# nuggy875/NeRF_pytorch_paeng

Measured on AMD Instinct MI355X. Metric: rays/sec (4096-ray batch, 64c+128f samples) + 800×800 frame render ms, higher is better.
Workload: dtype f32

## Files before the change

### nerf_pytorch_paeng_amd/csrc/api.hip

```cpp
#include <string>
#include "half_layout.h"

namespace minerf {

ABI_ERROR_STATE(, MI_NERF_EHIP)

int device_cus() {
    static std::atomic<int> cus[MN_MAX_DEVICES] = {};
    int dev = 0;
    if (hipGetDevice(&dev) != hipSuccess) return 256;
    std::atomic<int>& slot = cus[dev & (MN_MAX_DEVICES - 1)];
    int c = slot.load(std::memory_order_relaxed);
    if (c <= 0) {
        hipDeviceProp_t prop;
        c = (hipGetDeviceProperties(&prop, dev) == hipSuccess && prop.multiProcessorCount > 0) ? prop.multiProcessorCount : 256;
        slot.store(c, std::memory_order_relaxed);
    }
    return c;
}
int ensure_lds_opt_in(LdsOptIn& state, const void* kernel) {
    int dev = 0;
    MN_HIP(hipGetDevice(&dev));
    std::atomic<bool>& done = state.done[dev & (MN_MAX_DEVICES - 1)];
    if (!done.load(std::memory_order_acquire)) {
        MN_HIP(hipFuncSetAttribute(kernel, hipFuncAttributeMaxDynamicSharedMemorySize, 160 * 1024));
        done.store(true, std::memory_order_release);
    }
    return MI_NERF_OK;
}

int mlp_rays_fp32(const mi_nerf_net*, const void*, const float*, const float*, int64_t, int, float*, hipStream_t);
int mlp_embedded_fp32(const mi_nerf_net*, const void*, const float*, int64_t, float*, hipStream_t);
int mlp_rays_bf16(const mi_nerf_net*, const void*, const float*, const float*, int64_t, int, float*, hipStream_t, int points_per_wave, const StratDraw* strat,
                  FineDraw* fine = nullptr);
int mlp_rays_f16(const mi_nerf_net*, const void*, const float*, const float*, int64_t, int, float*, hipStream_t, int points_per_wave, const StratDraw* strat,
                 FineDraw* fine);
int mlp_rays_f16s(const mi_nerf_net*, const void*, const float*, const float*, int64_t, int, float*, hipStream_t);
int mlp_rays_f16s_stash(const mi_nerf_net*, const void*, const float*, const float*, int64_t, int, float*, float*, float*, float*, unsigned*, unsigned*,
                        hipStream_t);
int wgrad_products(int, const float* const*, const int*, const int*, const float* const*, const int*, const int*, int64_t, float* const*, const int*,
                   float* const*, void*, size_t, hipStream_t, bool);
int mlp_rays_fp32_stash(const mi_nerf_net*, const void*, const float*, const float*, int64_t, int, float*, float*, float*, float*, unsigned*,
                        unsigned*, hipStream_t);
int mlp_backward_fp32(const mi_nerf_net*, const void*, const void*, const float*, const float*, int64_t, int, const float*, const void*, void*,
                      size_t, float*, int, hipStream_t, const float*, int64_t, int);
int mlp_embedded_fp32_stash(const mi_nerf_net*, const void*, const float*, int64_t, float*, float*, float*, float*, unsigned*, unsigned*,
                            hipStream_t);
int train_layout(const mi_nerf_net*, int64_t, int, mi_nerf_train_layout*);
size_t wgrad_scratch_bytes();
int pack_apply(const int32_t*, const float*, size_t, void*, hipStream_t);
int frames_image_metrics(const float*, const float*, int64_t, float*, void*, size_t, hipStream_t);
int frames_nanmax(const float*, int64_t, float*, void*, size_t, hipStream_t);
int frames_to8b(const float*, int64_t, const float*, unsigned char*, hipStream_t);
int frames_rays_rgb(int, int, const float*, const float*, const float*, int64_t, float*, hipStream_t);
int frames_permute_rows(const float*, const int64_t*, int64_t, int, float*, hipStream_t);
int stage_make_o_d(int, int, const float*, const float*, int, int, float*, float*, hipStream_t);
int stage_make_o_d_pixels(int, int, const float*, const float*, const int64_t*, int64_t, float*, float*, hipStream_t);
int stage_ndc(int, int, float, float, const float*, int64_t, const float*, int64_t, int64_t, float*, float*, hipStream_t);
int stage_fill_uniform(uint32_t, uint32_t, int64_t, int64_t, int, float*, hipStream_t);
int stage_stratified(int64_t, int, float, float, const float*, uint32_t, int64_t, float*, hipStream_t);
int stage_embed(const float*, const float*, int64_t, int, int, int, float*, hipStream_t);
int stage_posenc(const float*, int64_t, int, float*, hipStream_t);
int stage_composite(const float*, const float*, const float*, int, int64_t, int, float*, float*, float*, float*, float*, hipStream_t);
int stage_composite_backward(const float*, const float*, const float*, int, int64_t, int, const float*, float*, hipStream_t);
int stage_sample_pdf(const float*, const float*, int64_t, int, int, int, const float*, float*, hipStream_t);
int stage_fine_z(const float*, const float*, int64_t, int, int, int, const float*, uint32_t, int64_t, float*, float*, hipStream_t);
int stage_composite_fine_z(const float*, const float*, const float*, int64_t, int, int, int, const float*, uint32_t, int64_t, float*, float*, float*,
                           float*, hipStream_t);

static int check_net_basic(const mi_nerf_net* net) {
    MN_CHECK_ARG(net != nullptr, "net is NULL");
    MN_CHECK_ARG(net->W >= 2 && net->W <= MAX_KERNEL_WIDTH, "unsupported width W=%d (the fp32 inference kernels run 2 <= W <= %d, padded to 128 / 256 / 384 / 512; "
                 "training, bf16 and split precision: 128 / 256 and 256)", net->W, MAX_KERNEL_WIDTH);
    MN_CHECK_ARG(net->D >= 2 && net->D <= 16, "unsupported depth D=%d", net->D);
    MN_CHECK_ARG(net->L_x >= 0 && net->L_x <= 10 && net->L_d >= 0 && net->L_d <= 4,
                 "unsupported encoding L_x=%d L_d=%d (the kernels evaluate up to 10 / 4 frequencies; fewer run with zero weights on the rest)", net->L_x, net->L_d);
    MN_CHECK_ARG(net->skip >= -1, "bad skip=%d", net->skip);
    return MI_NERF_OK;
}

enum class Family { FP32, F16S, BF16, F16 };
struct ModePlan { Family coarse, fine; int points_per_wave; };

static int mode_plan(int mode, ModePlan* p) {
    switch (mode) {
        case MI_NERF_MODE_F32:       *p = {Family::FP32, Family::FP32, 0}; return MI_NERF_OK;
        case MI_NERF_MODE_BF16:      *p = {Family::BF16, Family::BF16, 0}; return MI_NERF_OK;
        case MI_NERF_MODE_BF16_64:   *p = {Family::BF16, Family::BF16, 64}; return MI_NERF_OK;
        case MI_NERF_MODE_BF16_32:   *p = {Family::BF16, Family::BF16, 32}; return MI_NERF_OK;
        case MI_NERF_MODE_F16S:      *p = {Family::F16S, Family::F16S, 0}; return MI_NERF_OK;
        case MI_NERF_MODE_F16S_BF16: *p = {Family::F16S, Family::BF16, 0}; return MI_NERF_OK;
        case MI_NERF_MODE_F16:       *p = {Family::F16, Family::F16, 0}; return MI_NERF_OK;
        case MI_NERF_MODE_F16_BF16:  *p = {Family::F16, Family::BF16, 0}; return MI_NERF_OK;
    }
    set_error("mode must be one of MI_NERF_MODE_* (0..3, 5, 6, 8, 9; got %d)", mode);
    return MI_NERF_EINVAL;
}

static int mlp_rays_family(Family family, const mi_nerf_net* net, const void* packed, const float* rays, const float* z, int64_t n, int S, float* raw,
                           hipStream_t st, int points_per_wave, const StratDraw* strat = nullptr, FineDraw* fine = nullptr) {
    if (family == Family::FP32) return mlp_rays_fp32(net, packed, rays, z, n, S, raw, st);
    if (family == Family::F16S) return mlp_rays_f16s(net, packed, rays, z, n, S, raw, st);
    return (family == Family::F16 ? mlp_rays_f16 : mlp_rays_bf16)(net, packed, rays, z, n, S, raw, st, points_per_wave, strat, fine);
}

static int workspace_layout(const mi_nerf_render_cfg* cfg, int64_t n, mi_nerf_workspace_layout* L) {
    MN_CHECK_ARG(cfg && L, "NULL cfg/layout");
    MN_CHECK_ARG(n >= 0 && cfg->Sc >= 1 && cfg->Nf >= 0, "bad sizes n=%lld Sc=%d Nf=%d", (long long)n, cfg->Sc, cfg->Nf);
    MN_CHECK_ARG(cfg->Nf == 0 || cfg->Sc >= 3, "hierarchical sampling needs at least 3 coarse samples");
    size_t off = 0;
    const size_t nn = (size_t)n, Sc = (size_t)cfg->Sc, St = (size_t)(cfg->Sc + cfg->Nf);
    L->z_c = off;       off += align256(nn * Sc * 4);
    L->raw_c = off;     off += align256(nn * Sc * 16);
    L->weights_c = off; off += align256(nn * Sc * 4);
    L->z_f = off;       off += cfg->Nf > 0 ? align256(nn * St * 4) : 0;
    L->raw_f = off;     off += cfg->Nf > 0 ? align256(nn * St * 16) : 0;
    L->total = off;
    return MI_NERF_OK;
}

__global__ void mfma_selftest_kernel(const float* __restrict__ A, const float* __restrict__ B, float* __restrict__ D) {
    const int lane = threadIdx.x & 63;
    f32x16 acc;
#pragma unroll
    for (int r = 0; r < 16; ++r) acc[r] = 0.0f;
#pragma unroll
    for (int s = 0; s < 4; ++s) {
        const int k = 2 * s + (lane >> 5);
        const float a = A[(lane & 31) * 8 + k];
        const float b = B[k * 32 + (lane & 31)];
        acc = __builtin_amdgcn_mfma_f32_32x32x2f32(a, b, acc, 0, 0, 0);
    }
#pragma unroll
    for (int r = 0; r < 16; ++r) {
        const int i = (r & 3) + 8 * (r >> 2) + 4 * (lane >> 5);
        D[i * 32 + (lane & 31)] = acc[r];
    }
}

}

using namespace minerf;

extern "C" {

int mi_nerf_abi_version(void) { return MI_NERF_ABI_VERSION; }
const char* mi_nerf_last_error(void) { return g_err; }

size_t mi_nerf_packed_bytes(const mi_nerf_net* net) {
    if (check_net_basic(net)) return 0;
    return make_layout(net->D, net->W, net->skip, net->L_x, net->L_d).total_bytes;
}
int mi_nerf_pack_weights(const mi_nerf_net* net, const mi_nerf_params* params, void* blob, size_t bytes) {
    if (int rc = check_net_basic(net)) return rc;
    MN_CHECK_ARG(params && blob, "NULL params/blob");
    MN_CHECK_ARG(params->linear_x_w && params->linear_x_b && params->linear_density_w && params->linear_density_b &&
                 params->linear_feat_w && params->linear_feat_b && params->linear_d_w && params->linear_d_b &&
                 params->linear_color_w && params->linear_color_b, "NULL parameter pointer");
    for (int l = 0; l < net->D; ++l) MN_CHECK_ARG(params->linear_x_w[l] && params->linear_x_b[l], "NULL trunk layer %d", l);
    return pack_fp32(net, params, blob, bytes);
}
size_t mi_nerf_packed_bytes_bf16(const mi_nerf_net* net) {
    if (check_net_basic(net)) return 0;
    return packed_bytes_bf16(net);
}
size_t mi_nerf_packed_bytes_f16s(const mi_nerf_net* net) {
    return packed_bytes_f16s(net);
}
int mi_nerf_pack_weights_f16s(const mi_nerf_net* net, const mi_nerf_params* params, void* blob, size_t bytes) {
    MN_CHECK_ARG(net && params && blob, "NULL argument");
    return pack_f16s(net, params, blob, bytes);
}
int mi_nerf_pack_weights_bf16(const mi_nerf_net* net, const mi_nerf_params* params, void* blob, size_t bytes) {
    if (int rc = check_net_basic(net)) return rc;
    MN_CHECK_ARG(params && blob, "NULL params/blob");
    return pack_bf16(net, params, blob, bytes);
}

int mi_nerf_make_o_d(int W, int H, const float k4[4], const float pose12[12], int row0, int n_rows, float* o, float* d, void* st) {
    MN_CHECK_ARG(k4 && pose12, "NULL camera");
    return stage_make_o_d(W, H, k4, pose12, row0, n_rows, o, d, (hipStream_t)st);
}
int mi_nerf_make_o_d_pixels(int W, int H, const float k4[4], const float pose12[12], const int64_t* pix, int64_t n, float* o,
                            float* d, void* st) {
    MN_CHECK_ARG(k4 && pose12, "NULL camera");
    return stage_make_o_d_pixels(W, H, k4, pose12, pix, n, o, d, (hipStream_t)st);
}
int mi_nerf_ndc_rays(int H, int W, float focal, float near_, const float* o_in, int64_t os, const float* d_in, int64_t ds, int64_t n,
                     float* o_out, float* d_out, void* st) {
    return stage_ndc(H, W, focal, near_, o_in, os, d_in, ds, n, o_out, d_out, (hipStream_t)st);
}
int mi_nerf_fill_uniform(uint32_t seed, uint32_t stream_id, int64_t ray0, int64_t n_rays, int S, float* out, void* st) {
    return stage_fill_uniform(seed, stream_id, ray0, n_rays, S, out, (hipStream_t)st);
}
int mi_nerf_stratified_z(int64_t n_rays, int S, float near_, float far_, const float* t_rand, float* z, void* st) {
    MN_CHECK_ARG(t_rand != nullptr || n_rays == 0, "t_rand is NULL");
    return stage_stratified(n_rays, S, near_, far_, t_rand, 0, 0, z, (hipStream_t)st);
}
int mi_nerf_sample_pdf(const float* bins, const float* weights, int64_t n, int B, int N, int det, const float* u, float* out, void* st) {
    return stage_sample_pdf(bins, weights, n, B, N, det, u, out, (hipStream_t)st);
}
int mi_nerf_fine_z(const float* z_c, const float* w_c, int64_t n, int Sc, int Nf, int det, const float* u, float* z_f, float* z_s,
                   void* st) {
    MN_CHECK_ARG(det || u != nullptr || n == 0, "u is NULL (and det == 0)");
    return stage_fine_z(z_c, w_c, n, Sc, Nf, det, u, 0, 0, z_f, z_s, (hipStream_t)st);
}
int mi_nerf_embed(const float* rays, const float* z, int64_t n_rays, int S, int L_x, int L_d, float* out, void* st) {
    return stage_embed(rays, z, n_rays, S, L_x, L_d, out, (hipStream_t)st);
}
int mi_nerf_posenc(const float* x, int64_t n, int L, float* out, void* st) { return stage_posenc(x, n, L, out, (hipStream_t)st); }
int mi_nerf_mlp_embedded(const mi_nerf_net* net, const void* packed, const float* x, int64_t n, float* out, void* st) {
    return mlp_embedded_fp32(net, packed, x, n, out, (hipStream_t)st);
}
int mi_nerf_mlp_rays(const mi_nerf_net* net, const void* packed, const float* rays, const float* z, int64_t n_rays, int S, float* raw,
                     void* st) {
    return mlp_rays_fp32(net, packed, rays, z, n_rays, S, raw, (hipStream_t)st);
}
int mi_nerf_mlp_rays_bf16(const mi_nerf_net* net, const void* packed, const float* rays, const float* z, int64_t n_rays, int S,
                          float* raw, void* st) {
    MN_CHECK_ARG(z != nullptr || n_rays == 0, "z is NULL");
    return mlp_rays_bf16(net, packed, rays, z, n_rays, S, raw, (hipStream_t)st, 0, nullptr);
}
int mi_nerf_mlp_rays_f16s(const mi_nerf_net* net, const void* packed, const float* rays, const float* z, int64_t n_rays, int S, float* raw,
                          void* st) {
    return mlp_rays_f16s(net, packed, rays, z, n_rays, S, raw, (hipStream_t)st);
}
int mi_nerf_mlp_rays_bf16_shape(const mi_nerf_net* net, const void* packed, const float* rays, const float* z, int64_t n_rays, int S,
                                float* raw, int points_per_wave, void* st) {
    MN_CHECK_ARG(z != nullptr || n_rays == 0, "z is NULL");
    return mlp_rays_bf16(net, packed, rays, z, n_rays, S, raw, (hipStream_t)st, points_per_wave, nullptr);
}
int mi_nerf_composite(const float* raw, const float* z, const float* rays, int ray_stride, int64_t n, int S, float* rgb, float* disp,
                      float* acc, float* weights, float* depth, void* st) {
    return stage_composite(raw, z, rays, ray_stride, n, S, rgb, disp, acc, weights, depth, (hipStream_t)st);
}

int mi_nerf_composite_backward(const float* raw, const float* z, const float* rays, int ray_stride, int64_t n, int S,
                               const float* d_rgb, float* d_raw, void* st) {
    return stage_composite_backward(raw, z, rays, ray_stride, n, S, d_rgb, d_raw, (hipStream_t)st);
}

size_t mi_nerf_param_count(const mi_nerf_net* net) {
    if (check_net_basic(net)) return 0;
    return make_param_offsets(net->D, net->W, net->skip, net->L_x, net->L_d).total;
}
size_t mi_nerf_packed_bytes_bwd(const mi_nerf_net* net) {
    if (check_net_basic(net)) return 0;
    return packed_bytes_bwd(net);
}
int mi_nerf_pack_weights_bwd(const mi_nerf_net* net, const mi_nerf_params* params, void* host_blob, size_t blob_bytes) {
    if (int rc = check_net_basic(net)) return rc;
    MN_CHECK_ARG(params && host_blob, "NULL params/blob");
    return pack_bwd_fp32(net, params, host_blob, blob_bytes);
}
int mi_nerf_pack_map(const mi_nerf_net* net, int kind, int32_t* map_host, size_t map_len) {
    if (int rc = check_net_basic(net)) return rc;
    return pack_map(net, kind, map_host, map_len);
}
size_t mi_nerf_pack_map_bf16_len(const mi_nerf_net* net) {
    if (!net) return 0;
    return pack_map_bf16_len(net);
}
int mi_nerf_pack_map_bf16(const mi_nerf_net* net, int32_t* map_host, size_t map_len) {
    MN_CHECK_ARG(net && map_host, "NULL pointer");
    return pack_map_bf16(net, map_host, map_len);
}
int mi_nerf_pack_apply_bf16(const mi_nerf_net* net, const int32_t* map_dev, const float* flat_dev, void* blob_dev, size_t blob_bytes, void* st) {
    MN_CHECK_ARG(net, "net is NULL");
    return pack_apply_bf16(net, map_dev, flat_dev, blob_dev, blob_bytes, (hipStream_t)st);
}
int mi_nerf_pack_apply(const int32_t* map_dev, const float* flat_dev, size_t blob_bytes, void* blob_dev, void* st) {
    return pack_apply(map_dev, flat_dev, blob_bytes, blob_dev, (hipStream_t)st);
}
int mi_nerf_train_layout_query(const mi_nerf_net* net, int64_t n_rays, int S, mi_nerf_train_layout* out) {
    if (int rc = check_net_basic(net)) return rc;
    return train_layout(net, n_rays, S, out);
}
int mi_nerf_mlp_rays_train(const mi_nerf_net* net, const void* packed, const float* rays, const float* z, int64_t n_rays, int S,
                           float* raw, void* stash, size_t stash_bytes, void* st) {
    if (int rc = check_net_basic(net)) return rc;
    MN_CHECK_ARG(n_rays >= 0 && S >= 1, "bad sizes n_rays=%lld S=%d", (long long)n_rays, S);
    mi_nerf_train_layout L;
    if (int rc = train_layout(net, n_rays, S, &L)) return rc;
    if (n_rays == 0) return MI_NERF_OK;
    MN_CHECK_ARG(stash != nullptr && stash_bytes >= L.stash_bytes, "stash too small: %zu < %zu", stash_bytes, L.stash_bytes);
    return mlp_rays_fp32_stash(net, packed, rays, z, n_rays, S, raw, (float*)((char*)stash + L.stash_h), (float*)((char*)stash + L.stash_f),
                               (float*)((char*)stash + L.stash_g), (unsigned*)((char*)stash + L.mask_h), (unsigned*)((char*)stash + L.mask_g),
                               (hipStream_t)st);
}
int mi_nerf_mlp_rays_train_f16s(const mi_nerf_net* net, const void* packed_f16s, const float* rays, const float* z, int64_t n_rays, int S,
                                float* raw, void* stash, size_t stash_bytes, void* st) {
    if (int rc = check_net_basic(net)) return rc;
    MN_CHECK_ARG(n_rays >= 0 && S >= 1, "bad sizes n_rays=%lld S=%d", (long long)n_rays, S);
    mi_nerf_train_layout L;
    if (int rc = train_layout(net, n_rays, S, &L)) return rc;
    if (n_rays == 0) return MI_NERF_OK;
    MN_CHECK_ARG(stash != nullptr && stash_bytes >= L.stash_bytes, "stash too small: %zu < %zu", stash_bytes, L.stash_bytes);
    return mlp_rays_f16s_stash(net, packed_f16s, rays, z, n_rays, S, raw, (float*)((char*)stash + L.stash_h), (float*)((char*)stash + L.stash_f),
                               (float*)((char*)stash + L.stash_g), (unsigned*)((char*)stash + L.mask_h), (unsigned*)((char*)stash + L.mask_g),
                               (hipStream_t)st);
}
size_t mi_nerf_pack_map_f16s_len(const mi_nerf_net* net) {
    if (!net) return 0;
    return pack_map_f16s_len(net);
}
int mi_nerf_pack_map_f16s(const mi_nerf_net* net, int32_t* map_host, size_t map_len) {
    MN_CHECK_ARG(net && map_host, "NULL pointer");
    return pack_map_f16s(net, map_host, map_len);
}
size_t mi_nerf_packed_bytes_bwd_f16s(const mi_nerf_net* net) {
    if (!net) return 0;
    return packed_bytes_bwd_f16s(net);
}
int mi_nerf_pack_weights_bwd_f16s(const mi_nerf_net* net, const mi_nerf_params* params, void* host_blob, size_t blob_bytes) {
    MN_CHECK_ARG(net && params && host_blob, "NULL pointer");
    return pack_bwd_f16s(net, params, host_blob, blob_bytes);
}
size_t mi_nerf_pack_map_bwd_f16s_len(const mi_nerf_net* net) {
    if (!net) return 0;
    return pack_map_bwd_f16s_len(net);
}
int mi_nerf_pack_map_bwd_f16s(const mi_nerf_net* net, int32_t* map_host, size_t map_len) {
    MN_CHECK_ARG(net && map_host, "NULL pointer");
    return pack_map_bwd_f16s(net, map_host, map_len);
}
int mi_nerf_pack_apply_bwd_f16s(const mi_nerf_net* net, const int32_t* map_dev, const float* flat_dev, void* blob_dev, size_t blob_bytes,
                                uint32_t* out_of_range_dev, void* st) {
    MN_CHECK_ARG(net, "net is NULL");
    return pack_apply_bwd_f16s(net, map_dev, flat_dev, blob_dev, blob_bytes, out_of_range_dev, (hipStream_t)st);
}
int mi_nerf_pack_apply_f16s(const mi_nerf_net* net, const int32_t* map_dev, const float* flat_dev, void* blob_dev, size_t blob_bytes,
                            uint32_t* out_of_range_dev, void* st) {
    MN_CHECK_ARG(net, "net is NULL");
    return pack_apply_f16s(net, map_dev, flat_dev, blob_dev, blob_bytes, out_of_range_dev, (hipStream_t)st);
}
int mi_nerf_mlp_backward(const mi_nerf_net* net, const void* packed, const void* packed_bwd, const float* rays, const float* z,
                         int64_t n_rays, int S, const float* d_raw, const void* stash, void* work, size_t work_bytes, float* grads,
                         int stage, void* st) {
    if (int rc = check_net_basic(net)) return rc;
    return mlp_backward_fp32(net, packed, packed_bwd, rays, z, n_rays, S, d_raw, stash, work, work_bytes, grads, stage, (hipStream_t)st, nullptr, -1, 0);
}
int mi_nerf_mlp_backward_mode(const mi_nerf_net* net, const void* packed, const void* packed_bwd, const float* rays, const float* z,
                              int64_t n_rays, int S, const float* d_raw, const void* stash, void* work, size_t work_bytes, float* grads,
                              int stage, int mode, void* st) {
    if (int rc = check_net_basic(net)) return rc;
    MN_CHECK_ARG((mode & ~3) == 0, "unknown backward mode %d", mode);
    return mlp_backward_fp32(net, packed, packed_bwd, rays, z, n_rays, S, d_raw, stash, work, work_bytes, grads, stage, (hipStream_t)st, nullptr, -1, mode);
}
int mi_nerf_mlp_embedded_train(const mi_nerf_net* net, const void* packed, const float* x, int64_t n, float* out, void* stash, size_t stash_bytes,
                               void* st) {
    if (int rc = check_net_basic(net)) return rc;
    MN_CHECK_ARG(n >= 0, "bad n=%lld", (long long)n);
    mi_nerf_train_layout L;
    if (int rc = train_layout(net, (n + 31) / 32, 32, &L)) return rc;
    if (n == 0) return MI_NERF_OK;
    MN_CHECK_ARG(stash != nullptr && stash_bytes >= L.stash_bytes, "stash too small: %zu < %zu", stash_bytes, L.stash_bytes);
    return mlp_embedded_fp32_stash(net, packed, x, n, out, (float*)((char*)stash + L.stash_h), (float*)((char*)stash + L.stash_f),
                                   (float*)((char*)stash + L.stash_g), (unsigned*)((char*)stash + L.mask_h), (unsigned*)((char*)stash + L.mask_g),
                                   (hipStream_t)st);
}
int mi_nerf_mlp_embedded_backward(const mi_nerf_net* net, const void* packed, const void* packed_bwd, const float* x, int64_t n, const float* d_out,
                                  const void* stash, void* work, size_t work_bytes, float* grads, void* st) {
    if (int rc = check_net_basic(net)) return rc;
    MN_CHECK_ARG(n >= 0, "bad n=%lld", (long long)n);
    MN_CHECK_ARG(x != nullptr || n == 0, "NULL device pointer");
    static const float no_rows = 0.0f;
    return mlp_backward_fp32(net, packed, packed_bwd, nullptr, nullptr, (n + 31) / 32, 32, d_out, stash, work, work_bytes, grads, 0, (hipStream_t)st,
                             x ? x : &no_rows, n, 0);
}

int mi_nerf_image_metrics(const float* pred, const float* target, int64_t n, float* out2, void* scratch, size_t scratch_bytes, void* st) {
    return frames_image_metrics(pred, target, n, out2, scratch, scratch_bytes, (hipStream_t)st);
}
int mi_nerf_nanmax(const float* x, int64_t n, float* out, void* scratch, size_t scratch_bytes, void* st) {
    return frames_nanmax(x, n, out, scratch, scratch_bytes, (hipStream_t)st);
}
int mi_nerf_to8b(const float* x, int64_t n, const float* divisor, uint8_t* out, void* st) {
    return frames_to8b(x, n, divisor, out, (hipStream_t)st);
}
int mi_nerf_rays_rgb(int W, int H, const float k4[4], const float* poses, const float* images, int64_t n_img, float* out, void* st) {
    return frames_rays_rgb(W, H, k4, poses, images, n_img, out, (hipStream_t)st);
}
int mi_nerf_permute_rows(const float* src, const int64_t* perm, int64_t n, int row_floats, float* dst, void* st) {
    return frames_permute_rows(src, perm, n, row_floats, dst, (hipStream_t)st);
}

size_t mi_nerf_render_workspace_bytes(const mi_nerf_render_cfg* cfg, int64_t n_rays) {
    mi_nerf_workspace_layout L;
    if (workspace_layout(cfg, n_rays, &L)) return 0;
    return L.total;
}
int mi_nerf_render_workspace_layout(const mi_nerf_render_cfg* cfg, int64_t n_rays, mi_nerf_workspace_layout* out) {
    return workspace_layout(cfg, n_rays, out);
}

int mi_nerf_render_rays(const mi_nerf_net* net, const void* packed_c, const void* packed_f, const mi_nerf_render_cfg* cfg,
                        const float* rays, int64_t n, const float* t_rand, const float* u, void* ws, size_t ws_bytes,
                        float* rgb_c, float* disp_c, float* rgb_f, float* disp_f, void* stream) {
    hipStream_t st = (hipStream_t)stream;
    mi_nerf_workspace_layout L;
    if (int rc = workspace_layout(cfg, n, &L)) return rc;
    if (n == 0) return MI_NERF_OK;
    MN_CHECK_ARG(ws_bytes >= L.total, "workspace too small: %zu < %zu", ws_bytes, L.total);
    MN_CHECK_ARG(rays && rgb_c && disp_c && packed_c && (ws || L.total == 0), "NULL pointer");
    MN_CHECK_ARG(cfg->Nf == 0 || (packed_f && rgb_f && disp_f), "fine pass needs packed_fine and outputs");
    MN_CHECK_ARG(cfg->reserved == 0, "mi_nerf_render_cfg.reserved must be 0");
    char* w = (char*)ws;
    float* z_c = (float*)(w + L.z_c);
    float* raw_c = (float*)(w + L.raw_c);
    float* wts_c = (float*)(w + L.weights_c);
    const int Sc = cfg->Sc, St = cfg->Sc + cfg->Nf;
    ModePlan p;
    if (int rc = mode_plan(cfg->mode, &p)) return rc;
    if (p.coarse == Family::F16 || p.fine == Family::F16)
        if (int rc = check_net_half(net, "f16")) return rc;
    if (p.coarse == Family::F16S || p.fine == Family::F16S)
        if (int rc = check_net_f16s_forward(net)) return rc;
    FineDraw fd{};
    if (p.coarse == Family::BF16 || p.coarse == Family::F16) {
        const StratDraw sd{cfg->near_, cfg->far_, t_rand, cfg->seed, cfg->ray_offset, z_c};
        if (cfg->Nf > 0) fd = FineDraw{cfg->Nf, cfg->det, u, cfg->seed, cfg->ray_offset, rgb_c, disp_c, wts_c, (float*)(w + L.z_f), false};
        if (int rc = mlp_rays_family(p.coarse, net, packed_c, rays, nullptr, n, Sc, raw_c, st, p.points_per_wave, &sd,
                                     cfg->Nf > 0 && p.points_per_wave == 0 ? &fd : nullptr))
            return rc;
    } else {
        if (int rc = stage_stratified(n, Sc, cfg->near_, cfg->far_, t_rand, cfg->seed, cfg->ray_offset, z_c, st)) return rc;
        if (int rc = mlp_rays_family(p.coarse, net, packed_c, rays, z_c, n, Sc, raw_c, st, p.points_per_wave)) return rc;
    }
    if (cfg->Nf == 0) return stage_composite(raw_c, z_c, rays, 6, n, Sc, rgb_c, disp_c, nullptr, wts_c, nullptr, st);
    {
        float* z_f = (float*)(w + L.z_f);
        float* raw_f = (float*)(w + L.raw_f);
        if (!fd.taken)
            if (int rc = stage_composite_fine_z(raw_c, z_c, rays, n, Sc, cfg->Nf, cfg->det, u, cfg->seed, cfg->ray_offset, rgb_c, disp_c, wts_c, z_f, st))
                return rc;
        if (int rc = mlp_rays_family(p.fine, net, packed_f, rays, z_f, n, St, raw_f, st, p.points_per_wave)) return rc;
        if (int rc = stage_composite(raw_f, z_f, rays, 6, n, St, rgb_f, disp_f, nullptr, nullptr, nullptr, st)) return rc;
    }
    return MI_NERF_OK;
}

int mi_nerf_time_mlp_rays(const mi_nerf_net* net, const void* packed, const float* rays, const float* z, int64_t n_rays, int S,
                          float* raw, int iters, int mode, float* avg_ms, void* stream) {
    hipStream_t st = (hipStream_t)stream;
    MN_CHECK_ARG(iters >= 1 && avg_ms, "bad iters / NULL output");
    ModePlan p;
    if (int rc = mode_plan(mode, &p)) return rc;
    MN_CHECK_ARG(p.coarse == p.fine, "MI_NERF_MODE_* %d is two kernel families (mi_nerf_render_rays only): one network, one kernel family", mode);
    if (p.fine == Family::F16)
        if (int rc = check_net_half(net, "f16")) return rc;
    if (p.fine == Family::F16S)
        if (int rc = check_net_f16s_forward(net)) return rc;
    hipEvent_t e0, e1;
    MN_HIP(hipEventCreate(&e0));
    MN_HIP(hipEventCreate(&e1));
    int rc = MI_NERF_OK;
    MN_HIP(hipEventRecord(e0, st));
    for (int i = 0; i < iters && rc == MI_NERF_OK; ++i)
        rc = mlp_rays_family(p.fine, net, packed, rays, z, n_rays, S, raw, st, p.points_per_wave);
    MN_HIP(hipEventRecord(e1, st));
    MN_HIP(hipEventSynchronize(e1));
    float ms = 0.f;
    MN_HIP(hipEventElapsedTime(&ms, e0, e1));
    (void)hipEventDestroy(e0);
    (void)hipEventDestroy(e1);
    *avg_ms = ms / (float)iters;
    return rc;
}

size_t mi_nerf_wgrad_scratch_bytes(void) { return wgrad_scratch_bytes(); }
extern "C++" template <typename F>
static int timed_launches(int iters, float* avg_ms, hipStream_t st, F body) {
    MN_CHECK_ARG(iters >= 1, "bad iters");
    hipEvent_t e0 = nullptr, e1 = nullptr;
    if (avg_ms) {
        MN_HIP(hipEventCreate(&e0));
        MN_HIP(hipEventCreate(&e1));
        MN_HIP(hipEventRecord(e0, st));
    }
    int rc = MI_NERF_OK;
    for (int i = 0; i < iters && rc == MI_NERF_OK; ++i) rc = body();
    if (avg_ms) {
        MN_HIP(hipEventRecord(e1, st));
        MN_HIP(hipEventSynchronize(e1));
        float ms = 0.f;
        MN_HIP(hipEventElapsedTime(&ms, e0, e1));
        (void)hipEventDestroy(e0);
        (void)hipEventDestroy(e1);
        *avg_ms = ms / (float)iters;
    }
    return rc;
}
int mi_nerf_wgrad_products(int n, const float* const* delta, const int* ldd, const int* M, const float* const* x, const int* ldx, const int* N,
                           int64_t P, float* const* out, const int* ldo, float* const* bias, void* scratch, size_t scratch_bytes, int iters,
                           float* avg_ms, void* stream) {
    hipStream_t st = (hipStream_t)stream;
    return timed_launches(iters, avg_ms, st, [&] { return wgrad_products(n, delta, ldd, M, x, ldx, N, P, out, ldo, bias, scratch, scratch_bytes, st, false); });
}
int mi_nerf_wgrad_products_f16s(int n, const float* const* delta, const int* ldd, const int* M, const float* const* x, const int* ldx, const int* N,
                                int64_t P, float* const* out, const int* ldo, float* const* bias, void* scratch, size_t scratch_bytes, int iters,
                                float* avg_ms, void* stream) {
    hipStream_t st = (hipStream_t)stream;
    return timed_launches(iters, avg_ms, st, [&] { return wgrad_products(n, delta, ldd, M, x, ldx, N, P, out, ldo, bias, scratch, scratch_bytes, st, true); });
}

int mi_nerf_selftest_mfma(void* stream) {
    hipStream_t st = (hipStream_t)stream;
    float hA[32 * 8], hB[8 * 32], hD[32 * 32], ref[32 * 32];
    for (int i = 0; i < 32; ++i) for (int k = 0; k < 8; ++k) hA[i * 8 + k] = (float)((i * 3 + k * 7) % 11 - 5);
    for (int k = 0; k < 8; ++k) for (int j = 0; j < 32; ++j) hB[k * 32 + j] = (float)((k * 5 + j * 2 + (j > 9)) % 13 - 6);
    for (int i = 0; i < 32; ++i) for (int j = 0; j < 32; ++j) {
        float s = 0.f;
        for (int k = 0; k < 8; ++k) s += hA[i * 8 + k] * hB[k * 32 + j];
        ref[i * 32 + j] = s;
    }
    float *dA, *dB, *dD;
    MN_HIP(hipMalloc(&dA, sizeof(hA)));
    MN_HIP(hipMalloc(&dB, sizeof(hB)));
    MN_HIP(hipMalloc(&dD, sizeof(hD)));
    MN_HIP(hipMemcpyAsync(dA, hA, sizeof(hA), hipMemcpyHostToDevice, st));
    MN_HIP(hipMemcpyAsync(dB, hB, sizeof(hB), hipMemcpyHostToDevice, st));
    hipLaunchKernelGGL(mfma_selftest_kernel, dim3(1), dim3(64), 0, st, dA, dB, dD);
    MN_LAUNCH_CHECK("mfma_selftest_kernel");
    MN_HIP(hipMemcpyAsync(hD, dD, sizeof(hD), hipMemcpyDeviceToHost, st));
    MN_HIP(hipStreamSynchronize(st));
    (void)hipFree(dA); (void)hipFree(dB); (void)hipFree(dD);
    for (int i = 0; i < 32 * 32; ++i)
        if (hD[i] != ref[i]) {
            set_error("MFMA layout mismatch at D[%d][%d]: got %g want %g", i / 32, i % 32, hD[i], ref[i]);
            return MI_NERF_EINVAL;
        }
    return MI_NERF_OK;
}

}
```

### nerf_pytorch_paeng_amd/csrc/layout.h

```cpp
#pragma once
#include <stdint.h>
#include <stddef.h>

namespace minerf {

constexpr int QUAD_BYTES = 1024;
constexpr int SLOT_QUADS = 16;
constexpr int SLOT_BYTES = QUAD_BYTES * SLOT_QUADS;
constexpr int HEADER_BYTES = 1024;
constexpr uint32_t BLOB_MAGIC = 0x4D494E46u;

__host__ __device__ constexpr int pe_ksteps(int L) { return ((3 * L + 2 + 3) / 4) * 4; }

constexpr int KERNEL_LX = 10, KERNEL_LD = 4;

constexpr int MAX_KERNEL_WIDTH = 512;
__host__ __device__ constexpr int kernel_width(int W) { return W <= 128 ? 128 : (W <= 256 ? 256 : (W <= 384 ? 384 : 512)); }
__host__ __device__ constexpr bool wide_kernel_width(int Wk) { return Wk > 256; }
__host__ __device__ constexpr int pe_ksteps16(int L) { return (((3 * L + 1) / 2 + 1 + 3) / 4) * 4; }
__host__ __device__ constexpr bool native_width(int W) { return W == 128 || W == 256; }

struct BlobLayout {
    uint32_t stream_off;
    uint32_t stream_bytes_hoist;
    uint32_t stream_bytes_full;
    uint32_t side_off;
    uint32_t side_floats;
    uint32_t bias_trunk;
    uint32_t bias_feat;
    uint32_t bias_d;
    uint32_t dens_w;
    uint32_t dens_b;
    uint32_t color_w;
    uint32_t color_b;
    uint32_t wdir_t;
    uint32_t total_bytes;
};

__host__ __device__ inline uint32_t round_up_u32(uint32_t v, uint32_t m) { return (v + m - 1) / m * m; }

inline BlobLayout make_layout(int D, int W_net, int skip, int , int ) {
    constexpr int L_x = KERNEL_LX, L_d = KERNEL_LD;
    const int W = kernel_width(W_net);
    BlobLayout b{};
    const int NT = W / 32;
    const int in_d = 3 + 6 * L_d;
    const uint32_t pe_quads = (uint32_t)(pe_ksteps(L_x) / 4) * NT;
    const uint32_t h_quads = (uint32_t)(W / 2 / 4) * NT;
    uint32_t quads = pe_quads;
    for (int l = 1; l < D; ++l) quads += h_quads + ((skip >= 0 && l == skip + 1) ? pe_quads : 0);
    quads += h_quads;
    quads += (uint32_t)(W / 2 / 4) * (NT / 2);
    b.stream_off = HEADER_BYTES;
    b.stream_bytes_hoist = round_up_u32(quads, SLOT_QUADS) * QUAD_BYTES;
    uint32_t full = round_up_u32(quads, SLOT_QUADS) + round_up_u32((uint32_t)(pe_ksteps(L_d) / 4) * (NT / 2), SLOT_QUADS);
    b.stream_bytes_full = full * QUAD_BYTES;
    b.side_off = b.stream_off + b.stream_bytes_full;
    uint32_t f = 0;
    b.bias_trunk = f; f += (uint32_t)D * W;
    b.bias_feat = f;  f += W;
    b.bias_d = f;     f += W / 2;
    b.dens_w = f;     f += W;
    b.dens_b = f;     f += 4;
    b.color_w = f;    f += 3 * (W / 2);
    b.color_b = f;    f += 4;
    b.wdir_t = f;     f += (uint32_t)in_d * (W / 2);
    b.side_floats = round_up_u32(f, 4);
    b.total_bytes = b.side_off + b.side_floats * 4;
    return b;
}

struct SideTables {
    const char* stream;
    const float* side;
    int D;
    int skip_layer;
    unsigned stream_bytes;
    unsigned side_floats;
    unsigned o_bias_trunk, o_bias_feat, o_bias_d, o_wdir_t;
    unsigned o_dens_w, o_dens_b, o_color_w, o_color_b;
    unsigned o_head_b;
};
inline int skip_layer_of(int D, int skip) { return (skip >= 0 && skip + 1 < D) ? skip + 1 : -1; }

inline SideTables side_tables(const BlobLayout& L, const void* packed_dev, int D, int skip, bool full_stream) {
    SideTables t{};
    t.stream = (const char*)packed_dev + L.stream_off;
    t.side = (const float*)((const char*)packed_dev + L.side_off);
    t.D = D;
    t.skip_layer = skip_layer_of(D, skip);
    t.stream_bytes = full_stream ? L.stream_bytes_full : L.stream_bytes_hoist;
    t.side_floats = L.side_floats;
    t.o_bias_trunk = L.bias_trunk; t.o_bias_feat = L.bias_feat; t.o_bias_d = L.bias_d; t.o_wdir_t = L.wdir_t;
    t.o_dens_w = L.dens_w; t.o_dens_b = L.dens_b; t.o_color_w = L.color_w; t.o_color_b = L.color_b;
    return t;
}

struct ParamOffsets {
    uint32_t w_x[16], b_x[16];
    int in_l[16];
    uint32_t w_d, b_d, w_feat, b_feat, w_dens, b_dens, w_color, b_color;
    uint32_t total;
};

inline ParamOffsets make_param_offsets(int D, int W, int skip, int L_x, int L_d) {
    ParamOffsets p{};
    const int in_x = 3 + 6 * L_x, in_d = 3 + 6 * L_d;
    uint32_t f = 0;
    for (int l = 0; l < D; ++l) {
        p.in_l[l] = (l == 0) ? in_x : ((skip >= 0 && l == skip + 1) ? W + in_x : W);
        p.w_x[l] = f; f += (uint32_t)W * p.in_l[l];
        p.b_x[l] = f; f += W;
    }
    p.w_d = f;     f += (uint32_t)(W / 2) * (W + in_d);
    p.b_d = f;     f += W / 2;
    p.w_feat = f;  f += (uint32_t)W * W;
    p.b_feat = f;  f += W;
    p.w_dens = f;  f += W;
    p.b_dens = f;  f += 1;
    p.w_color = f; f += 3 * (W / 2);
    p.b_color = f; f += 3;
    p.total = f;
    return p;
}

inline uint32_t bwd_stream_bytes(int D, int W) {
    const uint32_t NT = W / 32;
    const uint32_t quads = (uint32_t)(W / 16) * NT + (uint32_t)D * (uint32_t)(W / 8) * NT;
    return round_up_u32(quads, SLOT_QUADS) * QUAD_BYTES;
}

}
```

### nerf_pytorch_paeng_amd/csrc/mlp_fp32.hip

```cpp
#include <stdlib.h>
#include <vector>
#include "common.h"
#include "layout.h"
#include "mlp_core.h"


namespace minerf {


template <int L, bool SLOW, int NPE>
__device__ __forceinline__ void encode_regs(float (&pe)[NPE], const float (&p)[3], int hh) {
#pragma unroll
    for (int s = 0; s < 3 * L; ++s) {
        const float y = p[s % 3] * (float)(1 << (s / 3));
        pe[s] = SLOW ? sin_cos_slow(y, hh) : sin_cos_fast(y, hh);
    }
    pe[3 * L] = hh ? p[1] : p[0];
    pe[3 * L + 1] = hh ? 0.0f : p[2];
#pragma unroll
    for (int s = 3 * L + 2; s < NPE; ++s) pe[s] = 0.0f;
}

template <int L, int NPE>
__device__ __forceinline__ void gather_regs(float (&pe)[NPE], const float* row, int hh, bool valid, int L_net) {
#pragma unroll
    for (int s = 0; s < 3 * L; ++s) {
        const int ch = 3 + 6 * (s / 3) + (s % 3) + 3 * hh;
        const bool have = valid && (s / 3) < L_net;
        pe[s] = have ? row[have ? ch : 0] : 0.0f;
    }
    pe[3 * L] = valid ? row[hh] : 0.0f;
    pe[3 * L + 1] = (valid && !hh) ? row[2] : 0.0f;
#pragma unroll
    for (int s = 3 * L + 2; s < NPE; ++s) pe[s] = 0.0f;
}

template <int W, bool STASH, int NEXT, int AL, int HN>
__device__ __forceinline__ void hidden_gemm(const MlpArgs& a, int layer, long long out_idx, long long wt, bool wave_active, f32x16 (&acc)[8],
                                            const float (&h)[HN], f32x4 (&aq)[8], const char* smem, WRing& ring, int lane, int hh) {
    constexpr int NT = W / 32;
    constexpr int HK_B = NT - 3, HK_M = NT - 2, HK_S = NT - 1;
    if constexpr (STASH) {
        float* row = a.stash_h + ((long long)layer * a.stash_rows + out_idx) * W + 4 * hh;
        unsigned mw[4] = {0u, 0u, 0u, 0u};
        unsigned mb[4];
        auto hook = [&](int kq, int t) __attribute__((always_inline)) {
            if (t == HK_B) mask_bits_chunk(h, kq, mb);
            if (t == HK_M) mask_merge_chunk(mb, kq, mw);
            if (t == HK_S) store_chunk(h, kq, row);
        };
        gemm_part<NT, HN, NEXT, AL>(acc, h, aq, smem, ring, lane, hook);
        if (wave_active) {
            u32x4 m; m[0] = mw[0]; m[1] = mw[1]; m[2] = mw[2]; m[3] = mw[3];
            *(u32x4*)(a.mask_h + (((long long)layer * a.n_wtiles + wt) * 64 + lane) * 4) = m;
        }
    } else {
        gemm_part<NT, HN, NEXT, AL>(acc, h, aq, smem, ring, lane);
    }
}

template <int W, int MODE, int LX, int LD, bool STASH>
__global__ __launch_bounds__(256) __attribute__((amdgpu_waves_per_eu(1, 1)))
void mlp_fp32_kernel(const MlpArgs a) {
    constexpr int NT = W / 32;
    constexpr int HN = W / 2;
    constexpr int KPE = pe_ksteps(LX);
    constexpr int KDE = pe_ksteps(LD);
    constexpr int AL = STASH ? 8 : 4;
    extern __shared__ __attribute__((aligned(16))) char smem[];
    float* side = (float*)(smem + RING_BYTES);
    const int tid = threadIdx.x;
    const int lane = tid & 63;
    const int wave = __builtin_amdgcn_readfirstlane(tid >> 6);
    const int col = lane & 31, hh = lane >> 5;
    float* scratch = side + a.side_floats + wave * (W / 2);

    for (unsigned i = tid * 4; i < a.side_floats; i += 256 * 4) *(f32x4*)(side + i) = *(const f32x4*)(a.side + i);

    const long long n_wg_tiles = (a.n_wtiles + 3) >> 2;
    if ((long long)blockIdx.x >= n_wg_tiles) return;

    WRing ring = ring_start(a.stream, a.stream_bytes, smem, wave, lane);

    f32x16 acc[8];
    f32x4 aq[8];
    float h[HN];
    float pe[KPE];
    ring_advance(ring);
#pragma unroll
    for (int t = 0; t < NT; ++t) aq[t] = ring_read(smem, ring, lane, t);

#ifdef MN_DIAG
    unsigned long long seg[8] = {0, 0, 0, 0, 0, 0, 0, 0};
    unsigned long long tprev = mn_stamp();
#endif
    RayTileWalk<32> walk = {};
    long long bias_ray = -1;
    const long long wid = (long long)blockIdx.x * 4 + wave;
    if constexpr (MODE == 0) walk.start(a, wid, col);
    for (long long it = 0; it < a.n_iter; ++it) {
#ifdef MN_DIAG
        ring.dlog = (a.diag && it == 2 && blockIdx.x < 4) ? a.diag + (size_t)gridDim.x * 32 + ((size_t)blockIdx.x * 4 + wave) * 512 : nullptr;
        ring.dcnt = 0;
#endif
        bool wave_active;
        long long wt;
        bool valid;
        long long out_idx;
        float de[KDE];
        if constexpr (MODE == 0) {
            wave_active = walk.active(a);
            const long long ray = walk.ray(a);
            const int chunk = walk.chunk(a);
            wt = ray * a.tpr + chunk;
            const int sample = chunk * 32 + col;
            valid = wave_active && sample < a.S;
            const int sc = sample < a.S ? sample : a.S - 1;
            out_idx = ray * a.S + sc;
            const float o[3] = {walk.o[0], walk.o[1], walk.o[2]}, d[3] = {walk.d[0], walk.d[1], walk.d[2]};
            const float zv = walk.z;
            walk.advance(a, col);
            float p[3];
            sample_point(p, o, d, zv);
            if (__builtin_expect(point_is_fast<LX>(p), 1)) encode_regs<LX, false>(pe, p, hh);
            else encode_regs<LX, true>(pe, p, hh);
            if (ray != bias_ray) {
                bias_ray = ray;
                hoisted_dir_bias<W, LD>(scratch, d[0], d[1], d[2], side + a.o_wdir_t, side + a.o_bias_d, lane);
            }
        } else {
            wt = it * ((long long)gridDim.x * 4) + wid;
            wave_active = wt < a.n_wtiles;
            if (!wave_active) wt = a.n_wtiles - 1;
            const long long p0 = wt * 32 + col;
            valid = wave_active && p0 < a.n_pts;
            out_idx = p0 < a.n_pts ? p0 : a.n_pts - 1;
            const int in_x_net = 3 + 6 * a.Lx_net;
            const float* row = a.x + out_idx * (in_x_net + 3 + 6 * a.Ld_net);
            gather_regs<LX>(pe, row, hh, true, a.Lx_net);
            gather_regs<LD>(de, row + in_x_net, hh, true, a.Ld_net);
        }

        MN_STAMP(0);
        acc_init<NT>(acc, side + a.o_bias_trunk, hh);
        gemm_part<NT, KPE, NT, AL>(acc, pe, aq, smem, ring, lane);
        MN_STAMP(1);
#pragma unroll 1
        for (int l = 1; l < a.D; ++l) {
            acc_to_b<NT, true>(acc, h);
            acc_init<NT>(acc, side + a.o_bias_trunk + l * W, hh);
            if (l == a.skip_layer) gemm_part<NT, KPE, NT, AL>(acc, pe, aq, smem, ring, lane);
            hidden_gemm<W, STASH, NT, AL>(a, l - 1, out_idx, wt, wave_active, acc, h, aq, smem, ring, lane, hh);
        }
        acc_to_b<NT, true>(acc, h);
        MN_STAMP(2);
        const float dens = xhalf_sum(dot_half<HN>(h, side + a.o_dens_w, hh)) + side[a.o_dens_b];
        acc_init<NT>(acc, side + a.o_bias_feat, hh);
        hidden_gemm<W, STASH, NT / 2, AL>(a, a.D - 1, out_idx, wt, wave_active, acc, h, aq, smem, ring, lane, hh);
        acc_to_b<NT, false>(acc, h);
        MN_STAMP(3);
        float* const row_f = STASH ? a.stash_f + out_idx * W + 4 * hh : nullptr;
        auto feat_hook = [&](int kq, int t) __attribute__((always_inline)) {
            if (STASH && t == NT / 2 - 1) store_chunk(h, kq, row_f);
        };
        if constexpr (MODE == 0) {
            acc_init<NT / 2>(acc, scratch, hh);
            gemm_part<NT / 2, HN, NT, AL>(acc, h, aq, smem, ring, lane, feat_hook);
        } else {
            acc_init<NT / 2>(acc, side + a.o_bias_d, hh);
            gemm_part<NT / 2, HN, NT / 2, AL>(acc, h, aq, smem, ring, lane, feat_hook);
            gemm_part<NT / 2, KDE, NT, AL>(acc, de, aq, smem, ring, lane);
        }
        float h2[HN / 2];
        acc_to_b<NT / 2, true>(acc, h2);
        if constexpr (STASH) {
            store_rows<NT / 2>(h2, a.stash_g + out_idx * (W / 2) + 4 * hh, valid);
            unsigned mg[2] = {0u, 0u};
#pragma unroll
            for (int q = 0; q < HN / 8; ++q) mask_pack_chunk(h2, q, mg);
            if (wave_active) {
                u32x2 m; m[0] = mg[0]; m[1] = mg[1];
                *(u32x2*)(a.mask_g + (wt * 64 + lane) * 2) = m;
            }
        }
        MN_STAMP(4);
        const float* cw = side + a.o_color_w;
        const float r0 = xhalf_sum(dot_half<HN / 2>(h2, cw, hh)) + side[a.o_color_b + 0];
        const float r1 = xhalf_sum(dot_half<HN / 2>(h2, cw + W / 2, hh)) + side[a.o_color_b + 1];
        const float r2 = xhalf_sum(dot_half<HN / 2>(h2, cw + W, hh)) + side[a.o_color_b + 2];
        if (valid && hh == 0) {
            f32x4 o; o[0] = r0; o[1] = r1; o[2] = r2; o[3] = dens;
            *(f32x4*)(a.out + out_idx * 4) = o;
        }
        MN_STAMP(5);
    }
#ifdef MN_DIAG
    if (a.diag && lane == 0) {
        unsigned long long* d = a.diag + ((size_t)blockIdx.x * 4 + wave) * 8;
        for (int i = 0; i < 8; ++i) d[i] = seg[i];
    }
#endif
    asm volatile("s_waitcnt vmcnt(0)" ::: "memory");
    __syncthreads();
}

static int check_net(const mi_nerf_net* net) {
    MN_CHECK_ARG(net != nullptr, "net is NULL");
    MN_CHECK_ARG(net->W >= 2 && net->W <= MAX_KERNEL_WIDTH, "unsupported width W=%d (the fp32 inference kernels run 2 <= W <= %d, padded to 128 / 256 / 384 / 512)", net->W, MAX_KERNEL_WIDTH);
    MN_CHECK_ARG(net->D >= 2 && net->D <= 16, "unsupported depth D=%d", net->D);
    MN_CHECK_ARG(net->L_x >= 0 && net->L_x <= KERNEL_LX && net->L_d >= 0 && net->L_d <= KERNEL_LD,
                 "unsupported encoding L_x=%d L_d=%d (the kernels evaluate up to %d / %d frequencies)", net->L_x, net->L_d, KERNEL_LX, KERNEL_LD);
    MN_CHECK_ARG(net->skip >= -1, "bad skip=%d", net->skip);
    return MI_NERF_OK;
}

int mlp_rays_fp32_wide(const mi_nerf_net*, const void*, const float*, const float*, int64_t, int, float*, hipStream_t);
int mlp_embedded_fp32_wide(const mi_nerf_net*, const void*, const float*, int64_t, float*, hipStream_t);

template <int W, int MODE, bool STASH = false>
static int launch(const MlpArgs& args_in, hipStream_t st) {
    MlpArgs args = args_in;
    auto kern = mlp_fp32_kernel<W, MODE, 10, 4, STASH>;
    static LdsOptIn opt_in = {};
    size_t lds;
    int grid;
    if (int rc = plan_launch<W, MODE>(args, (const void*)kern, opt_in, lds, grid)) return rc;
#ifdef MN_DIAG
    {
        MlpArgs da = args;
        unsigned long long* dbuf = nullptr;
        const size_t n = (size_t)grid * 4 * 8 + 16 * 512;
        MN_HIP(hipMalloc(&dbuf, n * 8));
        MN_HIP(hipMemsetAsync(dbuf, 0, n * 8, st));
        da.diag = dbuf;
        hipLaunchKernelGGL(kern, dim3(grid), dim3(256), lds, st, da);
        MN_HIP(hipStreamSynchronize(st));
        std::vector<unsigned long long> hbuf(n);
        MN_HIP(hipMemcpy(hbuf.data(), dbuf, n * 8, hipMemcpyDeviceToHost));
        (void)hipFree(dbuf);
        const double tiles = (double)((args.n_wtiles + 4 * grid - 1) / (4 * grid));
        static const char* names[6] = {"prologue", "layer0", "trunk", "dens+feature", "viewdir", "colour+store"};
        double tot = 0;
        fprintf(stderr, "[mn_diag] W=%d MODE=%d grid=%d tiles/wg=%.1f  cycles per tile (mean over waves):\n", W, MODE, grid, tiles);
        for (int sgi = 0; sgi < 6; ++sgi) {
            double sum = 0;
            for (size_t w = 0; w < (size_t)grid * 4; ++w) sum += (double)hbuf[w * 8 + sgi];
            const double per = sum / ((double)grid * 4) / tiles;
            tot += per;
            fprintf(stderr, "[mn_diag]   %-14s %10.0f\n", names[sgi], per);
        }
        fprintf(stderr, "[mn_diag]   %-14s %10.0f\n", "total", tot);
        if (const char* e = getenv("MN_DIAG_KQ")) {
            const int wsel = atoi(e);
            const unsigned long long* lg = hbuf.data() + (size_t)grid * 32 + (size_t)wsel * 512;
            fprintf(stderr, "[mn_diag] k-quad deltas (cycles; ideal %d) of wave %d, tile 2:", 4 * 64 * (W / 32), wsel);
            for (int i = 1; i < 500 && lg[i]; ++i) fprintf(stderr, "%s%llu", (i % 16 == 1) ? "\n[mn_diag]   " : " ", lg[i] - lg[i - 1]);
            fprintf(stderr, "\n");
        }
        return MI_NERF_OK;
    }
#endif
    hipLaunchKernelGGL(kern, dim3(grid), dim3(256), lds, st, args);
    MN_LAUNCH_CHECK("mlp_fp32_kernel");
    return MI_NERF_OK;
}

int mlp_rays_fp32(const mi_nerf_net* net, const void* packed_dev, const float* rays_dev, const float* z_dev,
                  int64_t n_rays, int S, float* raw_dev, hipStream_t st) {
    if (int rc = check_net(net)) return rc;
    MN_CHECK_ARG(n_rays >= 0 && S >= 1, "bad sizes n_rays=%lld S=%d", (long long)n_rays, S);
    if (n_rays == 0) return MI_NERF_OK;
    MN_CHECK_ARG(packed_dev && rays_dev && z_dev && raw_dev, "NULL device pointer");
    if (wide_kernel_width(kernel_width(net->W))) return mlp_rays_fp32_wide(net, packed_dev, rays_dev, z_dev, n_rays, S, raw_dev, st);
    MlpArgs a{};
    fill_common(a, net, packed_dev, false);
    fill_rays<32>(a, rays_dev, z_dev, n_rays, S, raw_dev);
    return kernel_width(net->W) == 256 ? launch<256, 0>(a, st) : launch<128, 0>(a, st);
}

int mlp_rays_fp32_stash(const mi_nerf_net* net, const void* packed_dev, const float* rays_dev, const float* z_dev,
                        int64_t n_rays, int S, float* raw_dev, float* stash_h, float* stash_f, float* stash_g, unsigned* mask_h,
                        unsigned* mask_g, hipStream_t st) {
    if (int rc = check_net(net)) return rc;
    MN_CHECK_ARG(native_width(net->W), "the training kernels exist for W = 128 and 256 (got %d)", net->W);
    MN_CHECK_ARG(n_rays >= 0 && S >= 1, "bad sizes n_rays=%lld S=%d", (long long)n_rays, S);
    if (n_rays == 0) return MI_NERF_OK;
    MN_CHECK_ARG(packed_dev && rays_dev && z_dev && raw_dev && stash_h && stash_f && stash_g && mask_h && mask_g, "NULL device pointer");
    MlpArgs a{};
    fill_common(a, net, packed_dev, false);
    fill_rays<32>(a, rays_dev, z_dev, n_rays, S, raw_dev);
    a.stash_h = stash_h; a.stash_f = stash_f; a.stash_g = stash_g; a.stash_rows = (long long)n_rays * S;
    a.mask_h = mask_h; a.mask_g = mask_g;
    return net->W == 256 ? launch<256, 0, true>(a, st) : launch<128, 0, true>(a, st);
}

int mlp_embedded_fp32_stash(const mi_nerf_net* net, const void* packed_dev, const float* x_dev, int64_t n, float* out_dev, float* stash_h,
                            float* stash_f, float* stash_g, unsigned* mask_h, unsigned* mask_g, hipStream_t st) {
    if (int rc = check_net(net)) return rc;
    MN_CHECK_ARG(native_width(net->W), "the training kernels exist for W = 128 and 256 (got %d)", net->W);
    MN_CHECK_ARG(n >= 0, "bad n=%lld", (long long)n);
    if (n == 0) return MI_NERF_OK;
    MN_CHECK_ARG(packed_dev && x_dev && out_dev && stash_h && stash_f && stash_g && mask_h && mask_g, "NULL device pointer");
    MlpArgs a{};
    fill_common(a, net, packed_dev, true);
    a.x = x_dev; a.out = out_dev; a.n_pts = n;
    a.n_wtiles = (n + 31) / 32;
    a.stash_h = stash_h; a.stash_f = stash_f; a.stash_g = stash_g; a.stash_rows = a.n_wtiles * 32;
    a.mask_h = mask_h; a.mask_g = mask_g;
    return net->W == 256 ? launch<256, 1, true>(a, st) : launch<128, 1, true>(a, st);
}

int mlp_embedded_fp32(const mi_nerf_net* net, const void* packed_dev, const float* x_dev, int64_t n, float* out_dev,
                      hipStream_t st) {
    if (int rc = check_net(net)) return rc;
    MN_CHECK_ARG(n >= 0, "bad n=%lld", (long long)n);
    if (n == 0) return MI_NERF_OK;
    MN_CHECK_ARG(packed_dev && x_dev && out_dev, "NULL device pointer");
    if (wide_kernel_width(kernel_width(net->W))) return mlp_embedded_fp32_wide(net, packed_dev, x_dev, n, out_dev, st);
    MlpArgs a{};
    fill_common(a, net, packed_dev, true);
    a.x = x_dev; a.out = out_dev; a.n_pts = n;
    a.n_wtiles = (n + 31) / 32;
    return kernel_width(net->W) == 256 ? launch<256, 1>(a, st) : launch<128, 1>(a, st);
}

}
```

### nerf_pytorch_paeng_amd/csrc/stage_dev.h

```cpp
#pragma once
#include "common.h"

namespace minerf {

__device__ __forceinline__ float wave_sum(float v) {
#pragma unroll
    for (int m = 32; m >= 1; m >>= 1) v += __shfl_xor(v, m, 64);
    return v;
}
__device__ __forceinline__ float wave_excl_prod(float v, int lane) {
    float inc = v;
#pragma unroll
    for (int d = 1; d < 64; d <<= 1) {
        const float o = __shfl_up(inc, d, 64);
        if (lane >= d) inc *= o;
    }
    const float e = __shfl_up(inc, 1, 64);
    return lane == 0 ? 1.0f : e;
}
__device__ __forceinline__ float wave_excl_sum(float v, int lane) {
    float inc = v;
#pragma unroll
    for (int d = 1; d < 64; d <<= 1) {
        const float o = __shfl_up(inc, d, 64);
        if (lane >= d) inc += o;
    }
    const float e = __shfl_up(inc, 1, 64);
    return lane == 0 ? 0.0f : e;
}
__device__ __forceinline__ float wave_excl_suffix_sum(float v, int lane) {
    float inc = v;
#pragma unroll
    for (int d = 1; d < 64; d <<= 1) {
        const float o = __shfl_down(inc, d, 64);
        if (lane + d < 64) inc += o;
    }
    const float e = __shfl_down(inc, 1, 64);
    return lane == 63 ? 0.0f : e;
}

template <int C>
__device__ __forceinline__ void composite_ray(const float* __restrict__ raw, const float* __restrict__ z, const float* __restrict__ rays,
                                              int ray_stride, long long ray, int S, int lane, float* __restrict__ rgb_o,
                                              float* __restrict__ disp_o, float* __restrict__ acc_o, float* __restrict__ w_o,
                                              float* __restrict__ depth_o, float* w_lds) {
    const float* dp = rays + ray * ray_stride + (ray_stride == 6 ? 3 : 0);
    const float dx = dp[0], dy = dp[1], dz = dp[2];
    const float dnorm = __builtin_sqrtf(dx * dx + dy * dy + dz * dz);
    const float* zr = z + ray * S;
    const f32x4* rr = (const f32x4*)(raw + ray * S * 4);

    float alpha[C], zv[C], cr[C], cg[C], cb[C];
    float local = 1.0f;
#pragma unroll
    for (int c = 0; c < C; ++c) {
        const int s = lane * C + c;
        const bool in = s < S;
        const int sc = in ? s : S - 1;
        const f32x4 v = rr[sc];
        zv[c] = zr[sc];
        float dist = (s + 1 < S) ? (zr[s + 1] - zv[c]) : 1e10f;
        dist = dist * dnorm;
        const float sig = __builtin_fmaxf(v[3], 0.0f);
        float a = 1.0f - expf(-sig * dist);
        if (!in || S == 1) a = 0.0f;
        alpha[c] = a;
        cr[c] = 1.0f / (1.0f + expf(-v[0]));
        cg[c] = 1.0f / (1.0f + expf(-v[1]));
        cb[c] = 1.0f / (1.0f + expf(-v[2]));
        local *= in ? (1.0f - a + 1e-10f) : 1.0f;
    }
    float T = wave_excl_prod(local, lane);
    float sw = 0.f, sr = 0.f, sg = 0.f, sb = 0.f, sd = 0.f;
#pragma unroll
    for (int c = 0; c < C; ++c) {
        const int s = lane * C + c;
        const float w = alpha[c] * T;
        if (s < S) {
            if (w_o) w_o[ray * S + s] = w;
            if (w_lds) w_lds[s] = w;
            sw += w; sr += w * cr[c]; sg += w * cg[c]; sb += w * cb[c]; sd += w * zv[c];
        }
        T *= (1.0f - alpha[c] + 1e-10f);
    }
    sw = wave_sum(sw); sr = wave_sum(sr); sg = wave_sum(sg); sb = wave_sum(sb); sd = wave_sum(sd);
    if (lane == 0) {
        const float q = sd / sw;
        const float m = (q != q) ? q : __builtin_fmaxf(1e-10f, q);
        float disp = 1.0f / m;
        if (disp != disp) disp = 0.0f;
        if (disp > 5.0f) disp = 5.0f;
        const float bg = 1.0f - sw;
        rgb_o[ray * 3 + 0] = sr + bg; rgb_o[ray * 3 + 1] = sg + bg; rgb_o[ray * 3 + 2] = sb + bg;
        disp_o[ray] = disp;
        if (acc_o) acc_o[ray] = sw;
        if (depth_o) depth_o[ray] = sd;
    }
}

__device__ __forceinline__ void build_cdf(const float* __restrict__ w, int nw, float* cdf, int lane) {
    const int C = (nw + 63) / 64;
    float part = 0.f;
    for (int c = 0; c < C; ++c) {
        const int k = lane * C + c;
        if (k < nw) part += w[k] + 1e-5f;
    }
    const float total = wave_sum(part);
    float run = 0.f, lsum = 0.f;
    for (int c = 0; c < C; ++c) {
        const int k = lane * C + c;
        if (k < nw) lsum += (w[k] + 1e-5f) / total;
    }
    run = wave_excl_sum(lsum, lane);
    if (lane == 0) cdf[0] = 0.0f;
    for (int c = 0; c < C; ++c) {
        const int k = lane * C + c;
        if (k < nw) { run += (w[k] + 1e-5f) / total; cdf[k + 1] = run; }
    }
}

__device__ __forceinline__ float invert_cdf(const float* cdf, const float* bins, int B, float u) {
    int lo = 0, len = B;
    while (len > 0) {
        const int half = len >> 1;
        const bool go = cdf[lo + half] <= u;
        lo = go ? lo + half + 1 : lo;
        len = go ? len - half - 1 : half;
    }
    const int below = lo - 1 > 0 ? lo - 1 : 0;
    const int above = lo < B - 1 ? lo : B - 1;
    const float c0 = cdf[below], c1 = cdf[above];
    float denom = c1 - c0;
    if (denom < 1e-5f) denom = 1.0f;
    const float t = (u - c0) / denom;
    const float b0 = bins[below], b1 = bins[above];
    return b0 + t * (b1 - b0);
}

__device__ __forceinline__ float det_u(int j, int N) {
    if (N == 1) return 0.0f;
    const float step = 1.0f / (float)(N - 1);
    return (j < N / 2) ? step * (float)j : 1.0f - step * (float)(N - 1 - j);
}

template <int R>
__device__ __forceinline__ void bitonic_sort_regs(float (&v)[R], int lane) {
    constexpr int n2 = 64 * R;
#pragma unroll
    for (int k = 2; k <= n2; k <<= 1) {
#pragma unroll
        for (int j = k >> 1; j > 0; j >>= 1) {
            if (j >= R) {
                const int m = j / R;
                const bool lower = (lane & m) == 0;
#pragma unroll
                for (int r = 0; r < R; ++r) {
                    const bool up = (((R * lane + r) & k) == 0);
                    const float x = v[r], y = __shfl_xor(x, m, 64);
                    const bool lt = x < y;
                    const float lo = lt ? x : y, hi = lt ? y : x;
                    v[r] = (lower == up) ? lo : hi;
                }
            } else {
#pragma unroll
                for (int r = 0; r < R; ++r)
                    if ((r & j) == 0) {
                        const bool up = (((R * lane + r) & k) == 0);
                        const float x = v[r], y = v[r | j];
                        const bool lt = x < y;
                        const float lo = lt ? x : y, hi = lt ? y : x;
                        v[r] = up ? lo : hi;
                        v[r | j] = up ? hi : lo;
                    }
            }
        }
    }
}
template <int R>
__device__ __forceinline__ void sort_row_regs(const float* all, int St, float* __restrict__ zrow, int lane) {
    float v[R];
    int nan_here = 0;
#pragma unroll
    for (int r = 0; r < R; ++r) {
        const int e = R * lane + r;
        const float x = e < St ? all[e] : __builtin_inff();
        const bool isn = x != x;
        nan_here += isn ? 1 : 0;
        v[r] = isn ? __builtin_inff() : x;
    }
    int n_nan = nan_here;
#pragma unroll
    for (int o = 32; o > 0; o >>= 1) n_nan += __shfl_xor(n_nan, o, 64);
    bitonic_sort_regs<R>(v, lane);
#pragma unroll
    for (int r = 0; r < R; ++r) {
        const int e = R * lane + r;
        if (e < St) zrow[e] = e < St - n_nan ? v[r] : __builtin_nanf("");
    }
}

__device__ __forceinline__ void fine_z_ray(const float* __restrict__ z_c, const float* wr, long long ray, int Sc, int Nf, int n2, int det,
                                           const Jitter& u, float* __restrict__ z_f, float* __restrict__ z_samp, float* lds,
                                           int lane) {
    const int B = Sc - 1, St = Sc + Nf;
    float* cdf = lds;
    float* bn = cdf + B;
    float* all = bn + B;
    const float* zr = z_c + ray * Sc;
    for (int k = lane; k < Sc; k += 64) all[k] = zr[k];
    for (int k = lane; k < B; k += 64) bn[k] = 0.5f * (zr[k + 1] + zr[k]);
    build_cdf(wr + 1, Sc - 2, cdf, lane);
    __builtin_amdgcn_wave_barrier();
    __builtin_amdgcn_fence(__ATOMIC_ACQ_REL, "wavefront");
    for (int j = lane; j < Nf; j += 64) {
        const float uu = det ? det_u(j, Nf) : jitter_at(u, ray, j, Nf);
        const float s = invert_cdf(cdf, bn, B, uu);
        all[Sc + j] = s;
        if (z_samp) z_samp[ray * Nf + j] = s;
    }
    __builtin_amdgcn_wave_barrier();
    __builtin_amdgcn_fence(__ATOMIC_ACQ_REL, "wavefront");
    if (n2 == 256) return sort_row_regs<4>(all, St, z_f + ray * St, lane);
    if (n2 == 128) return sort_row_regs<2>(all, St, z_f + ray * St, lane);
    if (n2 == 64) return sort_row_regs<1>(all, St, z_f + ray * St, lane);
    if (n2 == 512) return sort_row_regs<8>(all, St, z_f + ray * St, lane);
    int nan_here = 0;
    for (int e = lane; e < n2; e += 64) {
        const float v = e < St ? all[e] : __builtin_inff();
        const bool isn = v != v;
        nan_here += isn ? 1 : 0;
        if (isn || e >= St) all[e] = __builtin_inff();
    }
    int n_nan = nan_here;
#pragma unroll
    for (int o = 32; o > 0; o >>= 1) n_nan += __shfl_xor(n_nan, o, 64);
    __builtin_amdgcn_wave_barrier();
    __builtin_amdgcn_fence(__ATOMIC_ACQ_REL, "wavefront");
    for (int k = 2; k <= n2; k <<= 1)
        for (int j = k >> 1; j > 0; j >>= 1) {
            for (int t = lane; t < (n2 >> 1); t += 64) {
                const int i = ((t & ~(j - 1)) << 1) | (t & (j - 1));
                const int l = i | j;
                const float x = all[i], y = all[l];
                const bool lt = x < y;
                const float lo = lt ? x : y, hi = lt ? y : x;
                const bool up = (i & k) == 0;
                all[i] = up ? lo : hi;
                all[l] = up ? hi : lo;
            }
            __builtin_amdgcn_wave_barrier();
            __builtin_amdgcn_fence(__ATOMIC_ACQ_REL, "wavefront");
        }
    for (int e = lane; e < St; e += 64) z_f[ray * St + e] = e < St - n_nan ? all[e] : __builtin_nanf("");
}

}
```

### nerf_pytorch_paeng_amd/csrc/stages.hip

```cpp
#include "common.h"
#include "stage_dev.h"

namespace minerf {

struct CamArgs {
    float fx, fy, cx, cy;
    float r[9];
    float t[3];
};

__device__ __forceinline__ void pixel_ray(const CamArgs& c, int x, int y, float (&d)[3]) {
    const float dx = ((float)x - c.cx) / c.fx;
    const float dy = -((float)y - c.cy) / c.fy;
    const float dz = -1.0f;
#pragma unroll
    for (int i = 0; i < 3; ++i)
        d[i] = __builtin_fmaf(dz, c.r[3 * i + 2], __builtin_fmaf(dy, c.r[3 * i + 1], dx * c.r[3 * i + 0]));
}

__global__ __launch_bounds__(256) void make_o_d_kernel(CamArgs c, int W, int row0, long long n, float* __restrict__ o,
                                                        float* __restrict__ dout) {
    const long long i = (long long)blockIdx.x * 256 + threadIdx.x;
    if (i >= n) return;
    const int y = (int)(i / W) + row0, x = (int)(i % W);
    float d[3];
    pixel_ray(c, x, y, d);
    dout[3 * i + 0] = d[0]; dout[3 * i + 1] = d[1]; dout[3 * i + 2] = d[2];
    if (o) { o[3 * i + 0] = c.t[0]; o[3 * i + 1] = c.t[1]; o[3 * i + 2] = c.t[2]; }
}

__global__ __launch_bounds__(256) void make_o_d_pixels_kernel(CamArgs c, int W, const long long* __restrict__ pix,
                                                               long long n, float* __restrict__ o, float* __restrict__ dout) {
    const long long i = (long long)blockIdx.x * 256 + threadIdx.x;
    if (i >= n) return;
    const long long p = pix[i];
    float d[3];
    pixel_ray(c, (int)(p % W), (int)(p / W), d);
    dout[3 * i + 0] = d[0]; dout[3 * i + 1] = d[1]; dout[3 * i + 2] = d[2];
    if (o) { o[3 * i + 0] = c.t[0]; o[3 * i + 1] = c.t[1]; o[3 * i + 2] = c.t[2]; }
}

static CamArgs cam_args(const float k4[4], const float pose12[12]) {
    CamArgs c;
    c.fx = k4[0]; c.fy = k4[1]; c.cx = k4[2]; c.cy = k4[3];
    for (int i = 0; i < 3; ++i) {
        for (int j = 0; j < 3; ++j) c.r[3 * i + j] = pose12[4 * i + j];
        c.t[i] = pose12[4 * i + 3];
    }
    return c;
}

__global__ __launch_bounds__(256) void ndc_kernel(float sx, float sy, float near_, float two_near, const float* __restrict__ oin,
                                                   long long os, const float* __restrict__ din, long long ds, long long n,
                                                   float* __restrict__ oo, float* __restrict__ dd) {
    const long long i = (long long)blockIdx.x * 256 + threadIdx.x;
    if (i >= n) return;
    float ox = oin[i * os + 0], oy = oin[i * os + 1], oz = oin[i * os + 2];
    const float dx = din[i * ds + 0], dy = din[i * ds + 1], dz = din[i * ds + 2];
    const float t = -(near_ + oz) / dz;
    ox = ox + t * dx; oy = oy + t * dy; oz = oz + t * dz;
    const float ox_oz = ox / oz, oy_oz = oy / oz;
    oo[3 * i + 0] = sx * ox / oz;
    oo[3 * i + 1] = sy * oy / oz;
    oo[3 * i + 2] = 1.0f + two_near / oz;
    dd[3 * i + 0] = sx * (dx / dz - ox_oz);
    dd[3 * i + 1] = sy * (dy / dz - oy_oz);
    dd[3 * i + 2] = -two_near / oz;
}

__global__ __launch_bounds__(256) void fill_uniform_kernel(uint32_t seed, uint32_t stream_id, long long ray0, long long total,
                                                            int S, float* __restrict__ out) {
    const long long i = (long long)blockIdx.x * 256 + threadIdx.x;
    if (i >= total) return;
    const long long r = i / S;
    out[i] = counter_uniform(seed, stream_id, (uint32_t)(ray0 + r), (uint32_t)(i - r * S));
}

__global__ __launch_bounds__(256) void stratified_kernel(long long total, int S, float near_, float far_, float step,
                                                          Jitter t_rand, float* __restrict__ z) {
    const long long idx = (long long)blockIdx.x * 256 + threadIdx.x;
    if (idx >= total) return;
    const long long ray = idx / S;
    const int i = (int)(idx - ray * S);
    z[idx] = stratified_depth(ray, i, S, step, near_, far_, t_rand);
}

constexpr int EMB_PTS = 64;
__global__ __launch_bounds__(256) void embed_kernel(const float* __restrict__ rays, const float* __restrict__ z, long long n_pts,
                                                     int S, int L_x, int L_d, float* __restrict__ out) {
    extern __shared__ __attribute__((aligned(16))) float emb_tile[];
    const int in_x = 3 + 6 * L_x, ch_total = in_x + 3 + 6 * L_d;
    const int items = L_x + L_d + 2;
    const long long p0 = (long long)blockIdx.x * EMB_PTS;
    const int npt = (int)((n_pts - p0 < EMB_PTS) ? n_pts - p0 : EMB_PTS);
    for (int w = threadIdx.x; w < npt * items; w += 256) {
        const int lp = w / items, it = w - lp * items;
        const long long pt = p0 + lp;
        const float* rp = rays + (pt / S) * 6;
        const bool is_d = it > L_x;
        float b[3];
        if (!is_d) {
            const float zz = z[pt];
#pragma unroll
            for (int c = 0; c < 3; ++c) b[c] = rp[c] + rp[3 + c] * zz;
        } else {
            const float dx = rp[3], dy = rp[4], dz = rp[5];
            const float nrm = __builtin_sqrtf(dx * dx + dy * dy + dz * dz);
#pragma unroll
            for (int c = 0; c < 3; ++c) b[c] = rp[3 + c] / nrm;
        }
        float* row = emb_tile + lp * ch_total + (is_d ? in_x : 0);
        const int k = (is_d ? it - L_x - 1 : it) - 1;
        if (k < 0) {
#pragma unroll
            for (int c = 0; c < 3; ++c) row[c] = b[c];
        } else {
#pragma unroll
            for (int c = 0; c < 3; ++c) {
                const float y = b[c] * (float)(1 << k);
                const bool fast = __builtin_fabsf(y) < SINCOS_FAST_LIMIT;
                row[3 + 6 * k + c] = sin_cos_any(y, fast, 0);
                row[3 + 6 * k + 3 + c] = sin_cos_any(y, fast, 1);
            }
        }
    }
    __syncthreads();
    float* o = out + p0 * ch_total;
    const int n = npt * ch_total;
    if (((uintptr_t)o & 15) == 0) {
        const int n4 = n >> 2;
        for (int i = threadIdx.x; i < n4; i += 256) ((f32x4*)o)[i] = ((const f32x4*)emb_tile)[i];
        for (int i = 4 * n4 + threadIdx.x; i < n; i += 256) o[i] = emb_tile[i];
    } else {
        for (int i = threadIdx.x; i < n; i += 256) o[i] = emb_tile[i];
    }
}

__global__ __launch_bounds__(256) void posenc_kernel(const float* __restrict__ x, long long n, int L, float* __restrict__ out) {
    const int ch_total = 3 + 6 * L;
    const long long idx = (long long)blockIdx.x * 256 + threadIdx.x;
    if (idx >= n * ch_total) return;
    const long long pt = idx / ch_total;
    const int ch = (int)(idx - pt * ch_total);
    const int c = (ch < 3) ? ch : (ch - 3) % 3;
    const float base = x[pt * 3 + c];
    float v = base;
    if (ch >= 3) {
        const int k = (ch - 3) / 6, is_cos = ((ch - 3) % 6) >= 3;
        const float y = base * (float)(1 << k);
        v = sin_cos_any(y, __builtin_fabsf(y) < SINCOS_FAST_LIMIT, is_cos);
    }
    out[idx] = v;
}

template <int C>
__global__ __launch_bounds__(256) void composite_kernel(const float* __restrict__ raw, const float* __restrict__ z,
                                                         const float* __restrict__ rays, int ray_stride, long long n, int S,
                                                         float* __restrict__ rgb_o, float* __restrict__ disp_o,
                                                         float* __restrict__ acc_o, float* __restrict__ w_o,
                                                         float* __restrict__ depth_o) {
    const int lane = threadIdx.x & 63;
    const long long ray = (long long)blockIdx.x * 4 + (threadIdx.x >> 6);
    if (ray >= n) return;
    composite_ray<C>(raw, z, rays, ray_stride, ray, S, lane, rgb_o, disp_o, acc_o, w_o, depth_o, nullptr);
}

template <int C>
__global__ __launch_bounds__(256) void composite_bwd_kernel(const float* __restrict__ raw, const float* __restrict__ z,
                                                             const float* __restrict__ rays, int ray_stride, long long n, int S,
                                                             const float* __restrict__ d_rgb, float* __restrict__ d_raw) {
    const int lane = threadIdx.x & 63;
    const long long ray = (long long)blockIdx.x * 4 + (threadIdx.x >> 6);
    if (ray >= n) return;
    const float* dp = rays + ray * ray_stride + (ray_stride == 6 ? 3 : 0);
    const float dx = dp[0], dy = dp[1], dz = dp[2];
    const float dnorm = __builtin_sqrtf(dx * dx + dy * dy + dz * dz);
    const float* zr = z + ray * S;
    const f32x4* rr = (const f32x4*)(raw + ray * S * 4);
    f32x4* out = (f32x4*)(d_raw + ray * S * 4);
    const float Gr = d_rgb[ray * 3 + 0], Gg = d_rgb[ray * 3 + 1], Gb = d_rgb[ray * 3 + 2];

    float alpha[C], dads[C], cr[C], cg[C], cb[C];
    float local = 1.0f;
#pragma unroll
    for (int c = 0; c < C; ++c) {
        const int s = lane * C + c;
        const bool in = s < S;
        const int sc = in ? s : S - 1;
        const f32x4 v = rr[sc];
        float dist = (s + 1 < S) ? (zr[s + 1] - zr[sc]) : 1e10f;
        dist = dist * dnorm;
        const float sig = __builtin_fmaxf(v[3], 0.0f);
        const float e = expf(-sig * dist);
        float a = 1.0f - e;
        float ds = (v[3] > 0.0f) ? dist * e : 0.0f;
        if (!in || S == 1) { a = 0.0f; ds = 0.0f; }
        alpha[c] = a;
        dads[c] = ds;
        cr[c] = 1.0f / (1.0f + expf(-v[0]));
        cg[c] = 1.0f / (1.0f + expf(-v[1]));
        cb[c] = 1.0f / (1.0f + expf(-v[2]));
        local *= in ? (1.0f - a + 1e-10f) : 1.0f;
    }
    float T = wave_excl_prod(local, lane);
    float Tc[C], q[C], w[C];
    float lsum = 0.0f;
#pragma unroll
    for (int c = 0; c < C; ++c) {
        Tc[c] = T;
        w[c] = alpha[c] * T;
        q[c] = Gr * (cr[c] - 1.0f) + Gg * (cg[c] - 1.0f) + Gb * (cb[c] - 1.0f);
        lsum += q[c] * w[c];
        T *= (1.0f - alpha[c] + 1e-10f);
    }
    float R = wave_excl_suffix_sum(lsum, lane);
#pragma unroll
    for (int c = C - 1; c >= 0; --c) {
        const int s = lane * C + c;
        const float u = 1.0f - alpha[c] + 1e-10f;
        const float dLda = q[c] * Tc[c] - R / u;
        R += q[c] * w[c];
        if (s < S) {
            f32x4 o;
            o[0] = Gr * w[c] * cr[c] * (1.0f - cr[c]);
            o[1] = Gg * w[c] * cg[c] * (1.0f - cg[c]);
            o[2] = Gb * w[c] * cb[c] * (1.0f - cb[c]);
            o[3] = dLda * dads[c];
            out[s] = o;
        }
    }
}

__global__ __launch_bounds__(256) void sample_pdf_kernel(const float* __restrict__ bins, const float* __restrict__ weights,
                                                          long long n, int B, int N, int det, const float* __restrict__ u,
                                                          float* __restrict__ out) {
    extern __shared__ __attribute__((aligned(16))) float lds[];
    const int lane = threadIdx.x & 63, wv = threadIdx.x >> 6;
    const long long ray = (long long)blockIdx.x * 4 + wv;
    if (ray >= n) return;
    float* cdf = lds + wv * 2 * B;
    float* bn = cdf + B;
    for (int k = lane; k < B; k += 64) bn[k] = bins[ray * B + k];
    build_cdf(weights + ray * (B - 1), B - 1, cdf, lane);
    __builtin_amdgcn_wave_barrier();
    __builtin_amdgcn_fence(__ATOMIC_ACQ_REL, "wavefront");
    for (int j = lane; j < N; j += 64) {
        const float uu = det ? det_u(j, N) : u[ray * N + j];
        out[ray * N + j] = invert_cdf(cdf, bn, B, uu);
    }
}

__global__ __launch_bounds__(256) void fine_z_kernel(const float* __restrict__ z_c, const float* __restrict__ w_c, long long n,
                                                      int Sc, int Nf, int n2, int det, Jitter u,
                                                      float* __restrict__ z_f, float* __restrict__ z_samp) {
    extern __shared__ __attribute__((aligned(16))) float lds[];
    const int lane = threadIdx.x & 63, wv = threadIdx.x >> 6;
    const long long ray = (long long)blockIdx.x * 4 + wv;
    if (ray >= n) return;
    fine_z_ray(z_c, w_c + ray * Sc, ray, Sc, Nf, n2, det, u, z_f, z_samp, lds + wv * (2 * (Sc - 1) + n2), lane);
}

template <int C>
__global__ __launch_bounds__(256) void composite_fine_z_kernel(const float* __restrict__ raw, const float* __restrict__ z_c,
                                                                const float* __restrict__ rays, long long n, int Sc, int Nf, int n2, int det,
                                                                Jitter u, float* __restrict__ rgb_o, float* __restrict__ disp_o,
                                                                float* __restrict__ w_o, float* __restrict__ z_f) {
    extern __shared__ __attribute__((aligned(16))) float lds[];
    const int lane = threadIdx.x & 63, wv = threadIdx.x >> 6;
    const long long ray = (long long)blockIdx.x * 4 + wv;
    if (ray >= n) return;
    float* mine = lds + wv * (Sc + 2 * (Sc - 1) + n2);
    composite_ray<C>(raw, z_c, rays, 6, ray, Sc, lane, rgb_o, disp_o, nullptr, w_o, nullptr, mine);
    __builtin_amdgcn_wave_barrier();
    __builtin_amdgcn_fence(__ATOMIC_ACQ_REL, "wavefront");
    fine_z_ray(z_c, mine, ray, Sc, Nf, n2, det, u, z_f, nullptr, mine + Sc, lane);
}

constexpr int MAX_LDS_FLOATS_PER_RAY = 64 * 1024 / 4 / 4;

int stage_make_o_d(int W, int H, const float k4[4], const float pose12[12], int row0, int n_rows, float* o, float* d,
                   hipStream_t st) {
    MN_CHECK_ARG(W > 0 && H > 0 && row0 >= 0 && n_rows >= 0 && row0 + n_rows <= H, "bad image window W=%d H=%d rows [%d,+%d)", W, H, row0, n_rows);
    MN_CHECK_ARG(d != nullptr, "rays_d output is NULL");
    const long long n = (long long)n_rows * W;
    if (n == 0) return MI_NERF_OK;
    hipLaunchKernelGGL(make_o_d_kernel, dim3(blocks_for(n, 256)), dim3(256), 0, st, cam_args(k4, pose12), W, row0, n, o, d);
    MN_LAUNCH_CHECK("make_o_d_kernel");
    return MI_NERF_OK;
}

int stage_make_o_d_pixels(int W, int H, const float k4[4], const float pose12[12], const int64_t* pix, int64_t n, float* o,
                          float* d, hipStream_t st) {
    MN_CHECK_ARG(W > 0 && H > 0 && n >= 0 && d != nullptr && (pix != nullptr || n == 0), "bad arguments");
    if (n == 0) return MI_NERF_OK;
    hipLaunchKernelGGL(make_o_d_pixels_kernel, dim3(blocks_for(n, 256)), dim3(256), 0, st, cam_args(k4, pose12), W,
                       (const long long*)pix, (long long)n, o, d);
    MN_LAUNCH_CHECK("make_o_d_pixels_kernel");
    return MI_NERF_OK;
}

int stage_ndc(int H, int W, float focal, float near_, const float* o_in, int64_t os, const float* d_in, int64_t ds, int64_t n,
              float* o_out, float* d_out, hipStream_t st) {
    MN_CHECK_ARG(H > 0 && W > 0 && n >= 0, "bad sizes");
    if (n == 0) return MI_NERF_OK;
    MN_CHECK_ARG(o_in && d_in && o_out && d_out, "NULL pointer");
    const float sx = (float)(-1.0 / ((double)W / (2.0 * (double)focal)));
    const float sy = (float)(-1.0 / ((double)H / (2.0 * (double)focal)));
    const float two_near = (float)(2.0 * (double)near_);
    hipLaunchKernelGGL(ndc_kernel, dim3(blocks_for(n, 256)), dim3(256), 0, st, sx, sy, near_, two_near, o_in, (long long)os, d_in,
                       (long long)ds, (long long)n, o_out, d_out);
    MN_LAUNCH_CHECK("ndc_kernel");
    return MI_NERF_OK;
}

int stage_fill_uniform(uint32_t seed, uint32_t stream_id, int64_t ray0, int64_t n_rays, int S, float* out, hipStream_t st) {
    MN_CHECK_ARG(n_rays >= 0 && S >= 0 && (out || n_rays * S == 0), "bad arguments");
    const long long total = (long long)n_rays * S;
    if (total == 0) return MI_NERF_OK;
    hipLaunchKernelGGL(fill_uniform_kernel, dim3(blocks_for(total, 256)), dim3(256), 0, st, seed, stream_id, (long long)ray0, total, S, out);
    MN_LAUNCH_CHECK("fill_uniform_kernel");
    return MI_NERF_OK;
}

int stage_stratified(int64_t n_rays, int S, float near_, float far_, const float* t_rand, uint32_t seed, int64_t ray0, float* z, hipStream_t st) {
    MN_CHECK_ARG(n_rays >= 0 && S >= 1, "bad sizes");
    const long long total = (long long)n_rays * S;
    if (total == 0) return MI_NERF_OK;
    MN_CHECK_ARG(z, "NULL pointer");
    const float step = S > 1 ? 1.0f / (float)(S - 1) : 0.0f;
    hipLaunchKernelGGL(stratified_kernel, dim3(blocks_for(total, 256)), dim3(256), 0, st, total, S, near_, far_, step,
                       Jitter{t_rand, seed, 0u, (long long)ray0}, z);
    MN_LAUNCH_CHECK("stratified_kernel");
    return MI_NERF_OK;
}

int stage_embed(const float* rays, const float* z, int64_t n_rays, int S, int L_x, int L_d, float* out, hipStream_t st) {
    MN_CHECK_ARG(n_rays >= 0 && S >= 1 && L_x >= 0 && L_x <= 20 && L_d >= 0 && L_d <= 20, "bad sizes");
    const long long n_pts = (long long)n_rays * S;
    const long long total = n_pts * (6 + 6 * L_x + 6 * L_d);
    if (total == 0) return MI_NERF_OK;
    MN_CHECK_ARG(rays && z && out, "NULL pointer");
    hipLaunchKernelGGL(embed_kernel, dim3(blocks_for(n_pts, EMB_PTS)), dim3(256), (size_t)EMB_PTS * (6 + 6 * L_x + 6 * L_d) * sizeof(float), st,
                       rays, z, n_pts, S, L_x, L_d, out);
    MN_LAUNCH_CHECK("embed_kernel");
    return MI_NERF_OK;
}

int stage_posenc(const float* x, int64_t n, int L, float* out, hipStream_t st) {
    MN_CHECK_ARG(n >= 0 && L >= 0 && L <= 20, "bad sizes");
    const long long total = (long long)n * (3 + 6 * L);
    if (total == 0) return MI_NERF_OK;
    MN_CHECK_ARG(x && out, "NULL pointer");
    hipLaunchKernelGGL(posenc_kernel, dim3(blocks_for(total, 256)), dim3(256), 0, st, x, (long long)n, L, out);
    MN_LAUNCH_CHECK("posenc_kernel");
    return MI_NERF_OK;
}

int stage_composite(const float* raw, const float* z, const float* rays, int ray_stride, int64_t n, int S, float* rgb, float* disp,
                    float* acc, float* weights, float* depth, hipStream_t st) {
    MN_CHECK_ARG(n >= 0 && S >= 1 && S <= 1024, "bad sizes (n=%lld S=%d)", (long long)n, S);
    MN_CHECK_ARG(ray_stride == 3 || ray_stride == 6, "ray_stride must be 3 or 6");
    if (n == 0) return MI_NERF_OK;
    MN_CHECK_ARG(raw && z && rays && rgb && disp, "NULL pointer");
    const dim3 grid(blocks_for(n, 4)), block(256);
    const int C = (S + 63) / 64;
#define MN_COMP(CC) hipLaunchKernelGGL(composite_kernel<CC>, grid, block, 0, st, raw, z, rays, ray_stride, (long long)n, S, rgb, disp, acc, weights, depth)
    if (C == 1) MN_COMP(1); else if (C == 2) MN_COMP(2); else if (C == 3) MN_COMP(3); else if (C == 4) MN_COMP(4);
    else if (C <= 8) MN_COMP(8); else MN_COMP(16);
#undef MN_COMP
    MN_LAUNCH_CHECK("composite_kernel");
    return MI_NERF_OK;
}

int stage_composite_backward(const float* raw, const float* z, const float* rays, int ray_stride, int64_t n, int S,
                             const float* d_rgb, float* d_raw, hipStream_t st) {
    MN_CHECK_ARG(n >= 0 && S >= 1 && S <= 1024, "bad sizes (n=%lld S=%d)", (long long)n, S);
    MN_CHECK_ARG(ray_stride == 3 || ray_stride == 6, "ray_stride must be 3 or 6");
    if (n == 0) return MI_NERF_OK;
    MN_CHECK_ARG(raw && z && rays && d_rgb && d_raw, "NULL pointer");
    const dim3 grid(blocks_for(n, 4)), block(256);
    const int C = (S + 63) / 64;
#define MN_COMPB(CC) hipLaunchKernelGGL(composite_bwd_kernel<CC>, grid, block, 0, st, raw, z, rays, ray_stride, (long long)n, S, d_rgb, d_raw)
    if (C == 1) MN_COMPB(1); else if (C == 2) MN_COMPB(2); else if (C == 3) MN_COMPB(3); else if (C == 4) MN_COMPB(4);
    else if (C <= 8) MN_COMPB(8); else MN_COMPB(16);
#undef MN_COMPB
    MN_LAUNCH_CHECK("composite_bwd_kernel");
    return MI_NERF_OK;
}

int stage_sample_pdf(const float* bins, const float* weights, int64_t n, int B, int N, int det, const float* u, float* out,
                     hipStream_t st) {
    MN_CHECK_ARG(n >= 0 && B >= 2 && B <= MAX_LDS_FLOATS_PER_RAY / 2 && N >= 1, "bad sizes (B=%d N=%d; at most %d bins)", B, N, MAX_LDS_FLOATS_PER_RAY / 2);
    if (n == 0) return MI_NERF_OK;
    MN_CHECK_ARG(bins && weights && out && (det || u), "NULL pointer");
    hipLaunchKernelGGL(sample_pdf_kernel, dim3(blocks_for(n, 4)), dim3(256), (size_t)4 * 2 * B * sizeof(float), st, bins, weights,
                       (long long)n, B, N, det, u, out);
    MN_LAUNCH_CHECK("sample_pdf_kernel");
    return MI_NERF_OK;
}

int stage_fine_z(const float* z_c, const float* w_c, int64_t n, int Sc, int Nf, int det, const float* u, uint32_t seed, int64_t ray0,
                 float* z_f, float* z_samp, hipStream_t st) {
    MN_CHECK_ARG(n >= 0 && Sc >= 3 && Nf >= 1 && Sc + Nf <= MAX_LDS_FLOATS_PER_RAY, "bad sizes (Sc=%d Nf=%d)", Sc, Nf);
    int n2 = 2;
    while (n2 < Sc + Nf) n2 <<= 1;
    MN_CHECK_ARG(2 * (Sc - 1) + n2 <= MAX_LDS_FLOATS_PER_RAY, "bad sizes (Sc=%d Nf=%d: 2*(Sc-1) + %d (Sc+Nf rounded up to a power of two) must not exceed %d)",
                 Sc, Nf, n2, MAX_LDS_FLOATS_PER_RAY);
    if (n == 0) return MI_NERF_OK;
    MN_CHECK_ARG(z_c && w_c && z_f, "NULL pointer");
    const size_t lds = (size_t)4 * (2 * (Sc - 1) + n2) * sizeof(float);
    hipLaunchKernelGGL(fine_z_kernel, dim3(blocks_for(n, 4)), dim3(256), lds, st, z_c, w_c, (long long)n, Sc, Nf, n2, det,
                       Jitter{u, seed, 1u, (long long)ray0}, z_f, z_samp);
    MN_LAUNCH_CHECK("fine_z_kernel");
    return MI_NERF_OK;
}

int stage_composite_fine_z(const float* raw_c, const float* z_c, const float* rays, int64_t n, int Sc, int Nf, int det, const float* u,
                           uint32_t seed, int64_t ray0, float* rgb_c, float* disp_c, float* w_c, float* z_f, hipStream_t st) {
    MN_CHECK_ARG(n >= 0 && Sc >= 3 && Sc <= 1024 && Nf >= 1 && Sc + Nf <= MAX_LDS_FLOATS_PER_RAY, "bad sizes (Sc=%d Nf=%d)", Sc, Nf);
    int n2 = 2;
    while (n2 < Sc + Nf) n2 <<= 1;
    MN_CHECK_ARG(Sc + 2 * (Sc - 1) + n2 <= MAX_LDS_FLOATS_PER_RAY, "bad sizes (Sc=%d Nf=%d: 3 Sc - 2 + %d must not exceed %d)", Sc, Nf, n2,
                 MAX_LDS_FLOATS_PER_RAY);
    if (n == 0) return MI_NERF_OK;
    MN_CHECK_ARG(raw_c && z_c && rays && rgb_c && disp_c && w_c && z_f, "NULL pointer");
    const size_t lds = (size_t)4 * (Sc + 2 * (Sc - 1) + n2) * sizeof(float);
    const dim3 grid(blocks_for(n, 4)), block(256);
    const Jitter j{u, seed, 1u, (long long)ray0};
    const int C = (Sc + 63) / 64;
#define MN_CFZ(CC) hipLaunchKernelGGL(composite_fine_z_kernel<CC>, grid, block, lds, st, raw_c, z_c, rays, (long long)n, Sc, Nf, n2, det, j, rgb_c, disp_c, w_c, z_f)
    if (C == 1) MN_CFZ(1); else if (C == 2) MN_CFZ(2); else if (C == 3) MN_CFZ(3); else if (C == 4) MN_CFZ(4);
    else if (C <= 8) MN_CFZ(8); else MN_CFZ(16);
#undef MN_CFZ
    MN_LAUNCH_CHECK("composite_fine_z_kernel");
    return MI_NERF_OK;
}

}
```

### nerf_pytorch_paeng_amd/dist.py

```python
from __future__ import annotations

import ctypes as C
from typing import Callable, Dict, Optional, Sequence, Tuple

import torch
import torch.distributed as dist

from ._lib import MiNerfError, check, dev_ptr, lib, stream_ptr

COMM_ID_BYTES = 128


def shard_rows(H: int, world: int, rank: int) -> Tuple[int, int]:
    base, extra = divmod(H, world)
    n = base + (1 if rank < extra else 0)
    row0 = rank * base + min(rank, extra)
    return row0, n


def shard_range(n: int, world: int, rank: int) -> Tuple[int, int]:
    return shard_rows(n, world, rank)


class TileComm:

    def __init__(self, id_bytes: bytes, world: int, rank: int, device):
        self.device = torch.device(device)
        if self.device.type != "cuda":
            raise MiNerfError(f"TileComm lives on a HIP device, got {self.device}")
        if len(id_bytes) != COMM_ID_BYTES:
            raise MiNerfError(f"the unique id has {COMM_ID_BYTES} bytes, got {len(id_bytes)}")
        self.world, self.rank = int(world), int(rank)
        self._staging: Optional[torch.Tensor] = None
        handle = C.c_void_p()
        with torch.cuda.device(self.device):
            check(lib().mi_nerf_comm_init_rank(C.c_char_p(bytes(id_bytes)), self.world, self.rank, C.byref(handle)), "mi_nerf_comm_init_rank")
        self._handle = handle

    @staticmethod
    def available() -> None:
        check(lib().mi_nerf_rccl_available(), "mi_nerf_rccl_available")

    @staticmethod
    def unique_id() -> bytes:
        buf = C.create_string_buffer(COMM_ID_BYTES)
        check(lib().mi_nerf_comm_unique_id(buf), "mi_nerf_comm_unique_id")
        return buf.raw

    @classmethod
    def from_group(cls, device, group=None) -> "TileComm":
        device = torch.device(device)
        world, rank = dist.get_world_size(group), dist.get_rank(group)
        carrier = device if dist.get_backend(group) == "nccl" else torch.device("cpu")
        ident, why = bytes(COMM_ID_BYTES), None
        try:
            cls.available()
            if rank == 0:
                ident = cls.unique_id()
        except MiNerfError as e:
            why = e
        ok = torch.tensor([0 if why is not None else 1], dtype=torch.int32, device=carrier)
        dist.all_reduce(ok, op=dist.ReduceOp.MIN, group=group)
        if int(ok.item()) == 0:
            raise MiNerfError(f"TileComm.from_group: RCCL is not usable on every rank of the group (rank {rank}: {why if why is not None else 'ok here'})")
        t = torch.frombuffer(bytearray(ident), dtype=torch.uint8).to(carrier)
        dist.broadcast(t, src=dist.get_global_rank(group, 0) if group is not None else 0, group=group)
        return cls(bytes(t.cpu().numpy().tobytes()), world, rank, device)

    def all_gather_tiles(self, local: torch.Tensor, H: int, W: int, out: Optional[torch.Tensor] = None) -> torch.Tensor:
        if self._handle is None:
            raise MiNerfError("the communicator is closed")
        if local.dim() != 2 or local.shape[0] % W:
            raise MiNerfError(f"tile must be [rows_local * {W}, C], got {tuple(local.shape)}")
        Cc = int(local.shape[1])
        rows = local.shape[0] // W
        frame = torch.empty(H * W, Cc, dtype=torch.float32, device=local.device) if out is None else out
        if tuple(frame.shape) != (H * W, Cc) or frame.device != local.device:
            raise MiNerfError(f"out must be [{H * W}, {Cc}] on {local.device}, got {tuple(frame.shape)} on {frame.device}")
        need = int(lib().mi_nerf_all_gather_staging_bytes(self.world, H, W, Cc))
        if need and (self._staging is None or self._staging.numel() < need):
            self._staging = torch.empty(need, dtype=torch.uint8, device=local.device)
        with torch.cuda.device(local.device):
            check(lib().mi_nerf_all_gather_tiles(self._handle, dev_ptr(local, "tile"), rows, H, W, Cc, dev_ptr(frame, "frame"),
                                                 dev_ptr(self._staging, "staging", torch.uint8, 16) if need else None, need,
                                                 stream_ptr(local.device)), "mi_nerf_all_gather_tiles")
        return frame

    def close(self) -> None:
        if self._handle is not None:
            h, self._handle = self._handle, None
            with torch.cuda.device(self.device):
                check(lib().mi_nerf_comm_destroy(h), "mi_nerf_comm_destroy")


def unpad_tiles(staging: torch.Tensor, world: int, H: int, W: int, C_: int) -> torch.Tensor:
    frame = torch.empty(H * W, C_, dtype=torch.float32, device=staging.device)
    with torch.cuda.device(staging.device):
        check(lib().mi_nerf_unpad_tiles(dev_ptr(staging, "staging"), int(world), int(H), int(W), int(C_), dev_ptr(frame), stream_ptr(staging.device)),
              "mi_nerf_unpad_tiles")
    return frame


_tile_comms: Dict[Tuple[int, int], TileComm] = {}


def tile_comm(device, group=None) -> TileComm:
    device = torch.device(device)
    key = (id(group) if group is not None else 0, device.index if device.index is not None else torch.cuda.current_device())
    if key not in _tile_comms:
        _tile_comms[key] = TileComm.from_group(device, group)
    return _tile_comms[key]


def close_tile_comms() -> None:
    while _tile_comms:
        _tile_comms.popitem()[1].close()


def gather_tiles(local: torch.Tensor, H: int, W: int, group=None, force_collective: bool = False, via: str = "torch") -> torch.Tensor:
    if via not in ("torch", "c_abi"):
        raise ValueError(f"via must be 'torch' or 'c_abi', got {via!r}")
    if not (dist.is_available() and dist.is_initialized()) or (dist.get_world_size(group) == 1 and not force_collective):
        return local
    world, rank = dist.get_world_size(group), dist.get_rank(group)
    if via == "c_abi":
        if not local.is_cuda:
            raise MiNerfError(f"via='c_abi' gathers through the library's RCCL communicator and needs tiles on a HIP device (got {local.device}); there is no host fallback")
        _, n_rows = shard_rows(H, world, rank)
        if local.shape[0] != n_rows * W:
            raise ValueError(f"rank {rank}: tile has {local.shape[0]} rays, expected {n_rows * W}")
        return tile_comm(local.device, group).all_gather_tiles(local.contiguous(), H, W)
    C = local.shape[1]
    max_rows = (H + world - 1) // world
    _, n_rows = shard_rows(H, world, rank)
    if local.shape[0] != n_rows * W:
        raise ValueError(f"rank {rank}: tile has {local.shape[0]} rays, expected {n_rows * W}")
    padded = local
    if n_rows < max_rows:
        padded = torch.zeros(max_rows * W, C, dtype=local.dtype, device=local.device)
        padded[:n_rows * W] = local
    dev = local.device
    if dev.type == "cuda" and dist.get_backend(group) == "gloo":
        padded = padded.cpu()
    out = torch.empty(world * max_rows * W, C, dtype=local.dtype, device=padded.device)
    dist.all_gather_into_tensor(out, padded.contiguous(), group=group)
    out = out.to(dev)
    if H % world == 0:
        return out
    parts = []
    for r in range(world):
        _, nr = shard_rows(H, world, r)
        parts.append(out[r * max_rows * W:r * max_rows * W + nr * W])
    return torch.cat(parts, 0)


def assemble_tiles(tiles: Sequence[torch.Tensor], H: int, W: int) -> torch.Tensor:
    world = len(tiles)
    for r, t in enumerate(tiles):
        _, nr = shard_rows(H, world, r)
        if t.shape[0] != nr * W:
            raise ValueError(f"tile {r} of {world} has {t.shape[0]} rays, expected {nr * W}")
    return tiles[0] if world == 1 else torch.cat(list(tiles), 0)


def render_shard(H: int, W: int, K, pose, model, opts, world: int, rank: int, *, seed: int = 0, bf16: bool = False,
                 f16s: bool = False, coarse_f16s: bool = False) -> torch.Tensor:
    from . import nerf_process as NP
    from . import ops
    from .weights import packed_for
    packed = packed_for(model)
    r0, nr = shard_rows(H, world, rank)
    _, d = ops.make_o_d(W, H, K, pose, packed.device, row0=r0, n_rows=nr, want_origins=False)
    p = pose if isinstance(pose, torch.Tensor) else torch.as_tensor(pose)
    o = p[:3, -1].to(packed.device, torch.float32).expand(d.shape)
    rc, dc, rf, df = NP.batchify_rays_and_render_by_chunk(o, d, packed, None, H, W, K, opts, seed=seed, ray_offset=r0 * W, bf16=bf16, f16s=f16s,
                                                          coarse_f16s=coarse_f16s)
    rgb, disp = (rc, dc) if int(opts.N_samples_f) == 0 else (rf, df)
    return torch.cat([rgb, disp[:, None]], -1)


def render_frame(H: int, W: int, K, pose, model, opts, *, seed: int = 0, group=None, bf16: bool = False, f16s: bool = False,
                 render_rows_fn: Optional[Callable[[int, int], torch.Tensor]] = None, via: str = "torch",
                 force_collective: bool = False, coarse_f16s: bool = False) -> Tuple[torch.Tensor, torch.Tensor]:
    if dist.is_available() and dist.is_initialized():
        world, rank = dist.get_world_size(group), dist.get_rank(group)
    else:
        world, rank = 1, 0
    if render_rows_fn is None:
        local = render_shard(H, W, K, pose, model, opts, world, rank, seed=seed, bf16=bf16, f16s=f16s, coarse_f16s=coarse_f16s)
    else:
        local = render_rows_fn(*shard_rows(H, world, rank))
    full = gather_tiles(local, H, W, group, force_collective=force_collective, via=via)
    return full[:, :3].reshape(H, W, 3), full[:, 3].reshape(H, W)
```

### nerf_pytorch_paeng_amd/harness.py

```python
from __future__ import annotations

import os
import struct
import zlib
from typing import Dict, List, Optional, Sequence

import numpy as np
import torch

from . import nerf_process as NP
from . import ops
from ._lib import MiNerfError, as_f32_dev
from .rays import make_o_d


def write_png(path: str, img: np.ndarray) -> None:
    a = np.ascontiguousarray(img)
    if a.dtype != np.uint8:
        raise MiNerfError(f"write_png wants uint8, got {a.dtype}")
    if a.ndim == 3 and a.shape[2] == 1:
        a = a[:, :, 0]
    if a.ndim == 2:
        color, raw = 0, a
    elif a.ndim == 3 and a.shape[2] == 3:
        color, raw = 2, a.reshape(a.shape[0], -1)
    else:
        raise MiNerfError(f"write_png: unsupported shape {a.shape}")
    h, w = a.shape[0], a.shape[1]
    rows = np.concatenate([np.zeros((h, 1), np.uint8), raw], axis=1).tobytes()

    def chunk(tag: bytes, data: bytes) -> bytes:
        return struct.pack(">I", len(data)) + tag + data + struct.pack(">I", zlib.crc32(tag + data) & 0xFFFFFFFF)

    with open(path, "wb") as f:
        f.write(b"\x89PNG\r\n\x1a\n" + chunk(b"IHDR", struct.pack(">IIBBBBB", w, h, 8, color, 0, 0, 0))
                + chunk(b"IDAT", zlib.compress(rows, 6)) + chunk(b"IEND", b""))


def load_checkpoint(path: str, model: Optional[torch.nn.Module] = None, *, allow_pickle: bool = False) -> Dict:
    ck = torch.load(path, map_location="cpu", weights_only=not allow_pickle)
    if "model_state_dict" not in ck:
        raise MiNerfError(f"{path}: no 'model_state_dict' (keys: {sorted(ck)[:8]})")
    if model is not None:
        model.load_state_dict(ck["model_state_dict"])
    return ck


def _ckpt_path(log_dir: str, exp_name: str, idx) -> str:
    return os.path.join(log_dir, exp_name, f"{exp_name}_{idx}.pth.tar")


def spherical_poses(theta_deg, phi_deg: float, radius: float) -> np.ndarray:
    th = np.atleast_1d(np.asarray(theta_deg, dtype=np.float64)) / 180.0 * np.pi
    ph = float(phi_deg) / 180.0 * np.pi
    ct, st = np.cos(th).astype(np.float32), np.sin(th).astype(np.float32)
    cp, sp, r = np.float32(np.cos(ph)), np.float32(np.sin(ph)), np.float32(radius)
    zero, one = np.zeros_like(ct), np.ones_like(ct)
    fwd = np.stack([st * cp, ct * cp, -sp * one], -1)
    rows = np.stack([np.stack([-ct, st * sp, fwd[:, 0], fwd[:, 0] * r], -1),
                     np.stack([st, ct * sp, fwd[:, 1], fwd[:, 1] * r], -1),
                     np.stack([zero, cp * one, fwd[:, 2], fwd[:, 2] * r], -1),
                     np.stack([zero, zero, zero, one], -1)], 1)
    return rows.astype(np.float32)


def pose_spherical(theta: float, phi: float, radius: float) -> torch.Tensor:
    return torch.from_numpy(spherical_poses([theta], phi, radius)[0])


def get_render_pose(n_angle: int = 1, single_angle: float = -1, phi: float = -30.0, nf: float = 4.0, device=None) -> torch.Tensor:
    circle = n_angle != 1 and single_angle == -1
    azimuths = np.linspace(-180, 180, n_angle + 1)[:-1] if circle else [single_angle]
    poses = torch.from_numpy(spherical_poses(azimuths, phi, nf))
    return poses.to(device) if device is not None else poses


def _unit(v: np.ndarray) -> np.ndarray:
    if v.ndim == 1:
        return v / np.linalg.norm(v)
    return v / np.sqrt(np.square(v).sum(-1, keepdims=True))


def look_frames(back: np.ndarray, up: np.ndarray, eye: np.ndarray) -> np.ndarray:
    z = _unit(np.asarray(back))
    x = _unit(np.cross(np.broadcast_to(up, z.shape), z))
    y = _unit(np.cross(z, x))
    return np.stack([x, y, z, np.broadcast_to(eye, z.shape)], -1)


def rig_average(poses: np.ndarray) -> np.ndarray:
    frame = look_frames(_unit(poses[:, :3, 2].sum(0)), poses[:, :3, 1].sum(0), poses[:, :3, 3].mean(0))
    return np.concatenate([frame, poses[0, :3, -1:]], 1)


def spiral_path(c2w: np.ndarray, up: np.ndarray, radii, focus: float, zrate: float, rots: float, n: int) -> np.ndarray:
    t = np.linspace(0.0, 2.0 * np.pi * rots, int(n) + 1)[:-1]
    frame = c2w[:3, :4]
    local = np.stack([np.cos(t), -np.sin(t), -np.sin(t * zrate), np.ones_like(t)], -1) * np.append(np.asarray(radii, dtype=np.float64), 1.0)
    eyes = (local[:, None, :] * frame[None]).sum(-1)
    target = (frame * np.array([0.0, 0.0, -focus, 1.0])).sum(-1)
    cams = look_frames(eyes - target, up, eyes)
    return np.concatenate([cams, np.broadcast_to(c2w[:, 4:5], (len(t), 3, 1))], -1)


def recenter_rig(poses: np.ndarray) -> np.ndarray:
    last_row = np.array([0.0, 0.0, 0.0, 1.0])
    world_from_avg = np.vstack([rig_average(poses)[:3, :4], last_row])
    homog = np.concatenate([poses[:, :3, :4], np.broadcast_to(last_row, (poses.shape[0], 1, 4))], 1)
    out = poses + 0
    out[:, :3, :4] = (np.linalg.inv(world_from_avg) @ homog)[:, :3, :4]
    return out


def llff_render_poses(poses, bds, path_zflat: bool = False, n_views: int = 120, n_rots: int = 2) -> np.ndarray:
    centre = rig_average(poses)
    up = _unit(poses[:, :3, 1].sum(0))
    nearest, farthest = bds.min() * .9, bds.max() * 5.
    focus = 1. / (.25 / nearest + .75 / farthest)
    radii = np.percentile(np.abs(poses[:, :3, 3]), 90, 0)
    if path_zflat:
        centre[:3, 3] = centre[:3, 3] - nearest * .1 * centre[:3, 2]
        radii[2] = 0.
        n_rots, n_views = 1, n_views // 2
    return spiral_path(centre, up, radii, focus, zrate=.5, rots=n_rots, n=n_views).astype(np.float32)


def llff_cameras(raw_poses, raw_bds, bd_factor=.75, path_zflat: bool = False) -> Dict:
    poses = np.moveaxis(np.concatenate([raw_poses[:, 1:2, :], -raw_poses[:, 0:1, :], raw_poses[:, 2:, :]], 1), -1, 0).astype(np.float32)
    bds = np.moveaxis(raw_bds, -1, 0).astype(np.float32)
    scale = 1. if bd_factor is None else 1. / (bds.min() * bd_factor)
    poses[:, :3, 3] *= scale
    bds *= scale
    poses = recenter_rig(poses)
    render_poses = llff_render_poses(poses, bds, path_zflat)
    poses = poses.astype(np.float32)
    H, W, focal = poses[0, :3, -1]
    H, W = int(H), int(W)
    K = np.array([[focal, 0, 0.5 * W], [0, focal, 0.5 * H], [0, 0, 1]])
    return {"poses": poses, "bds": bds, "render_poses": render_poses, "gt_extrinsic": poses[:, :3, :4], "gt_intrinsic": K, "hw": [H, W]}


_PRECISIONS = {"fp32": (), "f16s": ("f16s",), "bf16": ("bf16",), "f16s+bf16": ("bf16", "coarse_f16s"), "f16": ("f16",), "f16+bf16": ("bf16", "coarse_f16")}


def _precision(opts) -> Dict[str, bool]:
    mode = str(getattr(opts, "precision", "fp32")).lower()
    if mode not in _PRECISIONS:
        raise ValueError(f"opts.precision must be one of {', '.join(repr(k) for k in _PRECISIONS)}, got {mode!r}")
    return {k: k in _PRECISIONS[mode] for k in ops.PRECISION_FLAGS}


def _frozen(model, opts):
    from .weights import packed_for
    if getattr(opts, "baked", None) is not None and getattr(opts, "mesh_view", None) is not None:
        raise MiNerfError("opts.baked and opts.mesh_view are both set: each renders every frame without the network; set one")
    if getattr(opts, "baked", None) is not None or getattr(opts, "mesh_view", None) is not None:
        return None
    packed = packed_for(model)
    if ops.precision(**_precision(opts)).reads_f16s:
        packed.f16s()
        packed.check_f16s_range()
    return packed


def _device_of(model, opts):
    grid = getattr(opts, "baked", None)
    if grid is not None:
        return grid.device
    view = getattr(opts, "mesh_view", None)
    if view is not None:
        return view.verts.device
    return next(model.parameters()).device if isinstance(model, torch.nn.Module) else model.device


def _render_pose(model, posenc, K, pose, hw, opts):
    img_h, img_w = hw
    view = getattr(opts, "mesh_view", None)
    if view is not None:
        from .mesh import Camera
        frame = view.render(Camera(img_h, img_w, K, pose[:3, :4]), near=float(getattr(opts, "mesh_view_near", 1e-3)),
                            cull=int(getattr(opts, "mesh_view_cull", 0)), bg=getattr(opts, "mesh_view_bg", (1.0, 1.0, 1.0)))
        return frame.rgb.reshape(-1, 3), frame.disp.reshape(-1)
    rays_o, rays_d = make_o_d(img_w, img_h, K, pose[:3, :4])
    grid = getattr(opts, "baked", None)
    if grid is not None:
        rays = torch.cat([rays_o.reshape(-1, 3), rays_d.reshape(-1, 3)], -1)
        rgb, disp, _, _ = grid.render(rays, step=getattr(opts, "baked_step", None), T_min=float(getattr(opts, "baked_T_min", 0.0) or 0.0))
        return rgb, disp
    rgb_c, disp_c, rgb_f, disp_f = NP.batchify_rays_and_render_by_chunk(rays_o, rays_d, model, posenc, img_h, img_w, K, opts, **_precision(opts),
                                                                        occupancy=getattr(opts, "occupancy", None))
    return (rgb_c, disp_c) if int(opts.N_samples_f) == 0 else (rgb_f, disp_f)


def test(idx, i_test, posenc, model, test_imgs, gt_intrinsic, gt_extrinsic, hw, opts, *, log_dir: Optional[str] = None,
         save_dir: Optional[str] = None, keep_frames: bool = False, ssim: bool = False, lpips=None) -> Dict:
    want_ssim = bool(ssim) or bool(getattr(opts, "ssim", False))
    lpips_model = lpips if lpips is not None else getattr(opts, "lpips", None)
    want_lpips = lpips_model is not None
    col_lpips = 3 if want_ssim else 2
    if isinstance(model, torch.nn.Module):
        model.eval()
        if log_dir is not None:
            load_checkpoint(_ckpt_path(log_dir, opts.exp_name, idx), model)
    if save_dir is not None:
        os.makedirs(save_dir, exist_ok=True)
    img_h, img_w = hw
    dev = _device_of(model, opts)
    n_pose = len(gt_extrinsic)
    want_frames = save_dir is not None or keep_frames
    metrics = torch.empty(n_pose, col_lpips + int(want_lpips), dtype=torch.float32, device=dev)
    rgbs8 = torch.empty(n_pose, img_h, img_w, 3, dtype=torch.uint8, device=dev) if want_frames else None
    disps8 = torch.empty(n_pose, img_h, img_w, 1, dtype=torch.uint8, device=dev) if want_frames else None
    with torch.no_grad():
        frozen = _frozen(model, opts)
        for i, pose in enumerate(gt_extrinsic):
            pose = as_f32_dev(pose, dev)
            pred_rgb, pred_disp = _render_pose(frozen, posenc, gt_intrinsic, pose, hw, opts)
            target = as_f32_dev(test_imgs[i], pred_rgb.device).reshape(-1, 3)
            metrics[i, :2] = ops.image_metrics(pred_rgb, target)
            if want_ssim:
                metrics[i, 2:3] = ops.ssim(pred_rgb.reshape(-1, 3), target, hw=(img_h, img_w))
            if want_lpips:
                metrics[i, col_lpips:] = ops.lpips(pred_rgb.reshape(-1, 3), target, hw=(img_h, img_w), model=lpips_model)
            if want_frames:
                rgbs8[i] = ops.to8b(pred_rgb).reshape(img_h, img_w, 3)
                disps8[i] = ops.to8b(pred_disp, ops.nanmax(pred_disp)).reshape(img_h, img_w, 1)
    m_host = metrics.cpu().numpy()
    losses: List[float] = [float(v) for v in m_host[:, 0]]
    psnrs: List[float] = [float(v) for v in m_host[:, 1]]
    frames = []
    if want_frames:
        rgbs_np, disps_np = rgbs8.cpu().numpy(), disps8.cpu().numpy()
        for i in range(n_pose):
            if save_dir is not None:
                write_png(os.path.join(save_dir, f"{i:03d}.png"), rgbs_np[i])
                write_png(os.path.join(save_dir, f"{i:03d}_disp.png"), disps_np[i])
            if keep_frames:
                frames.append((rgbs_np[i], disps_np[i]))
    ssims: Optional[List[float]] = [float(v) for v in m_host[:, 2]] if want_ssim else None
    lpipss: Optional[List[float]] = [float(v) for v in m_host[:, col_lpips]] if want_lpips else None
    best = int(np.argmax(psnrs)) if psnrs else -1
    res = {"loss": losses, "psnr": psnrs, "ssim": ssims, "lpips": lpipss, "best_idx": best,
           "best_psnr": psnrs[best] if psnrs else None, "mean_psnr": float(np.mean(psnrs)) if psnrs else None}
    if want_ssim:
        res["best_ssim"] = max(ssims) if ssims else None
        res["mean_ssim"] = float(np.mean(ssims)) if ssims else None
    if want_lpips:
        res["best_lpips"] = min(lpipss) if lpipss else None
        res["mean_lpips"] = float(np.mean(lpipss)) if lpipss else None
    if keep_frames:
        res["frames"] = frames
    if save_dir is not None:
        with open(os.path.join(save_dir, "_result.txt"), "w") as f:
            for i in range(len(losses)):
                f.write(f"idx:{i}\tloss:{losses[i]}\tpsnr:{psnrs[i]}\tssim:{ssims[i] if want_ssim else 'n/a'}\tlpips:{lpipss[i] if want_lpips else 'n/a'}\n")
            f.write(f"\nBest Value ) PSNR : {res['best_psnr']}\tSSIM : {res['best_ssim'] if want_ssim else 'n/a'}\tLPIPS : {res['best_lpips'] if want_lpips else 'n/a'}\n")
            f.write(f"Mean Value ) PSNR : {res['mean_psnr']}\tSSIM : {res['mean_ssim'] if want_ssim else 'n/a'}\tLPIPS : {res['mean_lpips'] if want_lpips else 'n/a'}")
    return res


def render(idx, posenc, model, gt_intrinsic, render_pose, hw, opts, *, log_dir: Optional[str] = None, save_dir: Optional[str] = None):
    dev = _device_of(model, opts)
    if getattr(opts, "data_type", None) in ("blender", "custom"):
        render_pose = get_render_pose(n_angle=opts.n_angle, single_angle=opts.single_angle, phi=opts.phi, nf=opts.nf)
    elif render_pose is None:
        raise MiNerfError("render(): llff data needs the loader's render poses (harness.llff_render_poses); got None")
    poses = torch.as_tensor(np.asarray(render_pose) if not isinstance(render_pose, torch.Tensor) else render_pose, dtype=torch.float32).to(dev)
    if isinstance(model, torch.nn.Module):
        model.eval()
        if log_dir is not None:
            load_checkpoint(_ckpt_path(log_dir, opts.exp_name, idx), model)
    if save_dir is not None:
        os.makedirs(save_dir, exist_ok=True)
    img_h, img_w = hw
    n = poses.shape[0]
    rgbs = torch.empty(n, img_h, img_w, 3, dtype=torch.uint8, device=dev)
    disps = torch.empty(n, img_h, img_w, dtype=torch.uint8, device=dev)
    with torch.no_grad():
        frozen = _frozen(model, opts)
        for i in range(n):
            rgb, disp = _render_pose(frozen, posenc, gt_intrinsic, poses[i], hw, opts)
            rgbs[i] = ops.to8b(rgb).reshape(img_h, img_w, 3)
            disps[i] = ops.to8b(disp, ops.nanmax(disp)).reshape(img_h, img_w)
    rgbs_np, disps_np = rgbs.cpu().numpy(), disps.cpu().numpy()
    if save_dir is not None:
        for i in range(n):
            write_png(os.path.join(save_dir, f"{i}_rgb.png"), rgbs_np[i])
            write_png(os.path.join(save_dir, f"{i}_disp.png"), disps_np[i])
    return rgbs_np, disps_np


class ShuffledRows:

    def __init__(self, table: torch.Tensor, perm: torch.Tensor):
        self.table, self.perm = table, perm

    @property
    def shape(self):
        return self.table.shape

    @property
    def device(self):
        return self.table.device

    def __len__(self) -> int:
        return int(self.table.shape[0])

    def __getitem__(self, key) -> torch.Tensor:
        if not isinstance(key, slice):
            raise MiNerfError("a shuffled global batch is read in slices of consecutive rows (train.py:29); materialize() gives the whole array")
        return ops.gather_rows(self.table, self.perm[key].contiguous())

    def materialize(self) -> torch.Tensor:
        return ops.permute_rows(self.table, self.perm)


class GetterRayBatchIdx:

    def __init__(self, rays_rgb: torch.Tensor, generator: Optional[torch.Generator] = None, shuffle: bool = False):
        self.table = rays_rgb
        self.perm: Optional[torch.Tensor] = None
        self.epoch = 0
        self.i_batch = 0
        self._gen = generator
        if shuffle:
            self._draw()

    def _draw(self) -> None:
        self.perm = torch.randperm(self.table.shape[0], device=self.table.device, generator=self._gen)

    @property
    def rays_rgb(self):
        return self.table if self.perm is None else ShuffledRows(self.table, self.perm)

    def shuffle_ray_idx(self, batch_size: int) -> None:
        self._draw()
        self.i_batch = batch_size
        self.epoch += 1

    def __call__(self, batch_size: int):
        self.i_batch += batch_size
        if self.i_batch >= self.table.shape[0]:
            self.shuffle_ray_idx(batch_size)
        return self.i_batch, self.rays_rgb, self.epoch


def global_batch(images, gt_intrinsic, gt_extrinsic, i_train: Sequence[int], hw, device, generator: Optional[torch.Generator] = None,
                 shuffle: bool = True) -> GetterRayBatchIdx:
    img_h, img_w = hw
    idx = torch.as_tensor(np.asarray(list(i_train)), dtype=torch.long)
    imgs = torch.as_tensor(np.asarray(images) if not isinstance(images, torch.Tensor) else images)
    poses = torch.as_tensor(np.asarray(gt_extrinsic) if not isinstance(gt_extrinsic, torch.Tensor) else gt_extrinsic)
    imgs = imgs[idx.to(imgs.device)].to(device=device, dtype=torch.float32).contiguous()
    poses = poses[idx.to(poses.device)][:, :3, :4].to(device=device, dtype=torch.float32).contiguous()
    rr = ops.rays_rgb(img_w, img_h, gt_intrinsic, poses, imgs)
    return GetterRayBatchIdx(rr, generator, shuffle=shuffle)


def sample_rays_and_pixel(i, img_w, img_h, K, pose, target_img, opts, generator: Optional[torch.Generator] = None, *, pose_grad: bool = False):
    target_img = as_f32_dev(target_img)
    dev = target_img.device
    if i < int(getattr(opts, "precrop_iters", 0)):
        dH = int(img_h // 2 * opts.precrop_frac)
        dW = int(img_w // 2 * opts.precrop_frac)
        ys = torch.arange(img_h // 2 - dH, img_h // 2 + dH, device=dev)
        xs = torch.arange(img_w // 2 - dW, img_w // 2 + dW, device=dev)
    else:
        ys = torch.arange(img_h, device=dev)
        xs = torch.arange(img_w, device=dev)
    n_coords = ys.numel() * xs.numel()
    n = int(opts.N_rays)
    if n > n_coords:
        raise MiNerfError(f"cannot draw {n} pixels without replacement from {n_coords}")
    sel = torch.randperm(n_coords, device=dev, generator=generator)[:n]
    py, px = ys[sel // xs.numel()], xs[sel % xs.numel()]
    pix = (py * img_w + px).contiguous()
    if pose_grad:
        from . import pose as pose_mod
        rays_o, rays_d = pose_mod.make_o_d(int(img_w), int(img_h), K, pose, pixels=pix)
    else:
        rays_o, rays_d = ops.make_o_d_pixels(int(img_w), int(img_h), K, pose, pix)
    target = target_img.reshape(-1, 3)[pix]
    return rays_o, rays_d, target


def train(idx, i_train, images, gt_cam_param, hw, model, criterion, posenc, optimizer, global_batch_idx, vis, opts, *,
          log_dir: Optional[str] = None, generator: Optional[torch.Generator] = None) -> Dict:
    from . import geometry as geo
    geom = geo.parse_options(getattr(opts, "geometry", None), float(opts.near), float(opts.far))
    refiner = getattr(opts, "pose_refine", None)
    if refiner is not None:
        from .pose import CameraRefiner
        if not isinstance(refiner, CameraRefiner):
            raise MiNerfError(f"opts.pose_refine must be a pose.CameraRefiner, got {type(refiner).__name__}")
        if global_batch_idx is not None and getattr(opts, "global_batch", True):
            raise MiNerfError("opts.pose_refine needs the per-image branch: the global batch holds rays precomputed from fixed poses "
                              "(pass global_batch_idx=None or opts.global_batch=False)")
    model.train()
    img_h, img_w = hw
    gt_intrinsic, gt_extrinsic = gt_cam_param
    dev = next(model.parameters()).device
    if global_batch_idx is not None and getattr(opts, "global_batch", True):
        i_batch, rays_rgb, _ = global_batch_idx(int(opts.N_rays))
        batch = rays_rgb[i_batch - int(opts.N_rays):i_batch]
        rays_o, rays_d, target_img = batch[:, 0], batch[:, 1], batch[:, 2]
    else:
        i_img = int(np.random.choice(i_train))
        target_full = as_f32_dev(torch.as_tensor(images[i_img]), dev)
        pose = torch.as_tensor(np.asarray(gt_extrinsic[i_img]) if not isinstance(gt_extrinsic, torch.Tensor) else gt_extrinsic[i_img])
        if refiner is not None:
            rays_o, rays_d, target_img = sample_rays_and_pixel(idx, img_w, img_h, gt_intrinsic, refiner(i_img, pose[:3, :4]), target_full, opts,
                                                               generator, pose_grad=True)
        else:
            rays_o, rays_d, target_img = sample_rays_and_pixel(idx, img_w, img_h, gt_intrinsic, pose[:3, :4], target_full, opts, generator)
    train_grid = getattr(opts, "train_occupancy", None)
    rebake = int(getattr(opts, "occupancy_rebake_every", 0) or 0)
    if train_grid is not None and rebake > 0 and idx % rebake == 0:
        with torch.no_grad():
            train_grid.bake(model, **getattr(opts, "occupancy_bake_args", {}))
    rgb_c, _, rgb_f, _, *extras = NP.batchify_rays_and_render_by_chunk(rays_o.contiguous(), rays_d.contiguous(), model, posenc, img_h, img_w,
                                                                       gt_intrinsic, opts, **_precision(opts), train_occupancy=train_grid,
                                                                       **({} if geom is None else {"geometry": True}),
                                                                       **({} if refiner is None else {"ray_grad": True}))
    optimizer.zero_grad()
    target_img = target_img.contiguous()
    loss = criterion(rgb_c, target_img)
    out = {"loss_c": loss.detach(), "psnr_c": -10.0 * torch.log10(loss.detach())}
    if int(opts.N_samples_f) > 0:
        loss_f = criterion(rgb_f, target_img)
        out.update(loss_f=loss_f.detach(), psnr_f=-10.0 * torch.log10(loss_f.detach()))
        loss = loss + loss_f
    if geom is not None:
        acc_t = depth_t = None
        if geom["targets"] is not None:
            with torch.no_grad():
                acc_t, depth_t = geom["targets"](torch.cat([rays_o, rays_d], -1).detach().contiguous())
        for key in ("c", "f") if int(opts.N_samples_f) > 0 else ("c",):
            for name, term in geo.loss_terms(geom, extras[0], key, acc_t, depth_t).items():
                loss = loss + geom[name + "_weight"] * term
                out["loss_" + name] = out.get("loss_" + name, 0.0) + term.detach()
    out["loss"] = loss.detach()
    loss.backward()
    optimizer.step()
    if _precision(opts)["f16s"] and idx % int(getattr(opts, "idx_print", 0) or 100) == 0:
        from . import train_path
        out["f16s"] = train_path.f16s_status(model, reset=False)
    if log_dir is not None and idx % int(getattr(opts, "idx_save", 0) or (1 << 62)) == 0 and idx > 0:
        save_path = os.path.join(log_dir, opts.exp_name)
        os.makedirs(save_path, exist_ok=True)
        torch.save({"idx": idx, "model_state_dict": model.state_dict(), "optimizer_state_dict": optimizer.state_dict()},
                   _ckpt_path(log_dir, opts.exp_name, idx))
    return out
```

### nerf_pytorch_paeng_amd/nerf_process.py

```python
from __future__ import annotations

from typing import Dict, Optional

import torch

from . import ops
from ._lib import MiNerfError, as_f32_dev
from .weights import PackedNeRF, packed_for
from . import train_path
from . import occupancy as occ
from . import occupancy_train
from . import geometry as geo

MAX_RAYS_PER_LAUNCH = 1 << 20

_rng = {"seed": 0, "calls": 0}


def manual_seed(seed: int) -> None:
    _rng["seed"], _rng["calls"] = int(seed), 0


def _next_seed(seed: Optional[int]) -> int:
    if seed is not None:
        return int(seed)
    s = (_rng["seed"] * 0x9E3779B1 + _rng["calls"]) & 0xFFFFFFFF
    _rng["calls"] += 1
    return s


_det = ops.deterministic


def ndc_rays(H, W, focal, near, rays_o, rays_d):
    lead = rays_d.shape[:-1]
    d = as_f32_dev(rays_d).reshape(-1, 3)
    o = rays_o.to(torch.float32) if rays_o.dtype != torch.float32 else rays_o
    o = o.expand(rays_d.shape).reshape(-1, 3) if o.shape != rays_d.shape else o.reshape(-1, 3)
    if isinstance(focal, torch.Tensor):
        focal = float(focal.item())
    oo, dd = ops.ndc_rays(int(H), int(W), float(focal), float(near), o, d)
    return oo.reshape(*lead, 3), dd.reshape(*lead, 3)


def sample_pdf(bins, weights, N_samples, det=False, opts=None, *, u=None):
    assert opts is not None
    bins, weights = as_f32_dev(bins), as_f32_dev(weights, bins.device)
    lead = bins.shape[:-1]
    b2, w2 = bins.reshape(-1, bins.shape[-1]), weights.reshape(-1, weights.shape[-1])
    if not det:
        u = (ops.fill_uniform(_next_seed(None), 1, 0, b2.shape[0], int(N_samples), bins.device) if u is None
             else as_f32_dev(u, bins.device).reshape(-1, int(N_samples)))
    out = ops.sample_pdf(b2, w2, int(N_samples), bool(det), u)
    return out.reshape(*lead, int(N_samples))


def pre_process(rays, posenc, opts, z_vals=None, weights=None, isFine=False, *, t_rand=None, u=None):
    rays = as_f32_dev(rays)
    n = rays.shape[0]
    L_x, L_d = int(getattr(posenc[0], "L", 10)), int(getattr(posenc[1], "L", 4))
    if not isFine:
        if t_rand is None:
            t_rand = ops.fill_uniform(_next_seed(None), 0, 0, n, int(opts.N_samples_c), rays.device)
        z = ops.stratified_z(float(opts.near), float(opts.far), as_f32_dev(t_rand, rays.device))
    else:
        det = _det(opts)
        if not det and u is None:
            u = ops.fill_uniform(_next_seed(None), 1, 0, n, int(opts.N_samples_f), rays.device)
        z = ops.fine_z(as_f32_dev(z_vals, rays.device), as_f32_dev(weights, rays.device), int(opts.N_samples_f), det,
                       None if det else as_f32_dev(u, rays.device))
    embedded = ops.embed(rays, z, L_x, L_d)
    return embedded, z, rays[:, 3:]


class _Composite(torch.autograd.Function):

    @staticmethod
    def forward(ctx, raw, z, d, weights_grad=False):
        rgb, disp, acc, wts, depth = ops.composite(raw, z, d, want_all=True)
        ctx.save_for_backward(raw, z, d)
        ctx.mark_non_differentiable(*((disp,) if weights_grad else (disp, wts)))
        ctx.set_materialize_grads(False)
        return rgb, disp, acc, wts, depth

    @staticmethod
    def backward(ctx, g_rgb, g_disp, g_acc, g_wts, g_depth):
        if g_rgb is None and g_acc is None and g_wts is None and g_depth is None:
            return None, None, None, None
        raw, z, d = ctx.saved_tensors
        if g_acc is None and g_wts is None and g_depth is None:
            return ops.composite_backward(raw, z, d, g_rgb.contiguous().float()), None, None, None
        g_rgb, g_acc, g_wts, g_depth = (None if g is None else g.contiguous().float() for g in (g_rgb, g_acc, g_wts, g_depth))
        return geo.composite_geo_backward(raw, z, d, 0.0, 1.0, g_rgb, g_acc, g_depth, None, g_wts), None, None, None


def post_process(outputs, z_vals, rays_d, *, weights_grad: bool = False):
    z = as_f32_dev(z_vals)
    raw = as_f32_dev(outputs, z.device)
    d = as_f32_dev(rays_d, z.device)
    if torch.is_grad_enabled() and raw.requires_grad:
        return _Composite.apply(raw, z.detach(), d.detach(), bool(weights_grad))
    return ops.composite(raw, z, d, want_all=True)


raw2outputs = post_process


def run_network(model, embedded, is_fine: bool = False):
    if train_path.wants_grad(model):
        return model(embedded, is_fine)
    packed = packed_for(model)
    return ops.mlp_embedded(packed.net, packed.blob(is_fine), as_f32_dev(embedded, packed.device))


def _render(rays: torch.Tensor, packed: PackedNeRF, opts, t_rand, u, seed: int, ray_offset: int, prec: ops.Precision,
            intermediates: bool, occupancy=None, geometry: bool = False) -> Dict[str, torch.Tensor]:
    n = rays.shape[0]
    dev = rays.device
    Sc, Nf = int(opts.N_samples_c), int(opts.N_samples_f)
    det = _det(opts)
    cfg = ops.render_cfg(float(opts.near), float(opts.far), Sc, Nf, det, seed=seed, ray_offset=ray_offset)
    cfg.mode = prec.mode
    if t_rand is not None:
        t_rand = as_f32_dev(t_rand, dev)
    elif intermediates:
        t_rand = ops.fill_uniform(seed, 0, ray_offset, n, Sc, dev)
    if Nf > 0 and not det:
        if u is not None:
            u = as_f32_dev(u, dev)
        elif intermediates:
            u = ops.fill_uniform(seed, 1, ray_offset, n, Nf, dev)
    else:
        u = None
    net, blob_c, blob_f = packed.kernel_blobs(prec)
    stats = None
    if occupancy is None:
        rgb_c, disp_c, rgb_f, disp_f, ws = ops.render_rays(net, blob_c, blob_f if Nf > 0 else None, cfg, rays, t_rand, u)
        views = ops.workspace_views
    else:
        rgb_c, disp_c, rgb_f, disp_f, ws, stats = occ.render_rays(net, blob_c, blob_f if Nf > 0 else None, cfg, occupancy, rays, t_rand, u)
        occupancy.last_stats = occ.add_stats(occupancy.last_stats, stats)
        views = occ.workspace_views
    out = {"rgb_c": rgb_c, "disp_c": disp_c}
    if Nf > 0:
        out["rgb_f"], out["disp_f"] = rgb_f, disp_f
    if geometry:
        v = views(cfg, n, ws)
        for key in ("c", "f") if Nf > 0 else ("c",):
            extra = geo.composite_geo(v["raw_" + key], v["z_" + key], rays, float(opts.near), float(opts.far))
            out.update({name + "_" + key: t for name, t in zip(geo.EXTRA_KEYS, (extra[2], extra[4], extra[5]))})
    if intermediates:
        for k, v in views(cfg, n, ws).items():
            out["_" + k] = v
        out["_t_rand"], out["_u"] = t_rand, u
        if stats is not None:
            out["_occ_stats"] = stats
    return out


def _occupancy_arg(occupancy, training: bool, prec: ops.Precision):
    if occupancy is None:
        return None
    if training:
        raise MiNerfError("occupancy= is an inference feature (call under torch.no_grad(), or freeze the model); to train with a grid pass it as "
                          "train_occupancy=")
    if not isinstance(occupancy, occ.OccupancyGrid):
        raise MiNerfError(f"occupancy must be an occupancy.OccupancyGrid, got {type(occupancy).__name__}")
    occ.check_precision(prec)
    occupancy.last_stats = None
    return occupancy


def _train_occupancy_arg(grid, training: bool, prec: ops.Precision):
    if grid is None:
        return None
    occupancy_train.check_grid(grid)
    if not training:
        raise MiNerfError("train_occupancy= is a training feature: gradients are disabled or no parameter of the model requires them "
                          "(under torch.no_grad() render with occupancy=)")
    if prec.coarse != prec.fine or prec.fine not in ("fp32", "f16s"):
        raise MiNerfError(f"training with a grid runs fp32 or f16s for both networks (got coarse {prec.coarse}, fine {prec.fine})")
    grid.last_stats = None
    return grid


def _train_f16s(prec: ops.Precision, intermediates: bool = False) -> bool:
    if prec.fine not in ("fp32", "f16s") or intermediates:
        raise MiNerfError("the training path has no bf16 / f16 mode (fp32, or f16s=True: split-precision forward, fp32 backward) and returns no intermediates")
    return prec.fine == "f16s"


def _geometry_kw(geometry, ray_grad=False) -> Dict[str, bool]:
    return {**({"geometry": True} if geometry else {}), **({"ray_grad": True} if ray_grad else {})}


def _render_train(rays, model, opts, train_occupancy, t_rand, u, seed: int, ray_offset: int, f16s: bool, geometry, ray_grad):
    grid = {} if train_occupancy is None else {"grid": train_occupancy}
    return train_path.render_train(rays, model, opts, t_rand=t_rand, u=u, seed=seed, ray_offset=ray_offset, f16s=f16s,
                                   **_geometry_kw(geometry, ray_grad), **grid)


def _ray_grad_arg(ray_grad, train_occupancy) -> bool:
    if ray_grad and train_occupancy is not None:
        raise MiNerfError(train_path.RAY_GRAD_WITH_GRID)
    return bool(ray_grad)


def render_rays(rays, model, posenc, opts, *, t_rand=None, u=None, seed=None, ray_offset: int = 0, bf16: bool = False,
                return_intermediates: bool = False, f16s: bool = False, coarse_f16s: bool = False, f16: bool = False, coarse_f16: bool = False,
                occupancy=None, train_occupancy=None, geometry: bool = False, ray_grad: bool = False):
    prec = ops.precision(bf16, f16s, coarse_f16s, f16, coarse_f16)
    ray_grad = _ray_grad_arg(ray_grad, train_occupancy)
    training = train_path.wants_grad(model) or train_path.wants_ray_grad(model, ray_grad, rays)
    occupancy = _occupancy_arg(occupancy, training, prec)
    train_occupancy = _train_occupancy_arg(train_occupancy, training, prec)
    if training:
        train_f16s = _train_f16s(prec, return_intermediates)
        if rays.dim() != 2 or rays.shape[1] != 6:
            raise MiNerfError(f"rays must be [n, 6] (o, d), got {tuple(rays.shape)}")
        return _render_train(rays, model, opts, train_occupancy, t_rand, u, _next_seed(seed), int(ray_offset), train_f16s, geometry, ray_grad)
    packed = packed_for(model)
    rays = as_f32_dev(rays, packed.device)
    if rays.dim() != 2 or rays.shape[1] != 6:
        raise MiNerfError(f"rays must be [n, 6] (o, d), got {tuple(rays.shape)}")
    if occupancy is not None and rays.shape[0] > occ.MAX_RAYS_PER_LAUNCH:
        raise MiNerfError(f"render_rays with a grid takes at most {occ.MAX_RAYS_PER_LAUNCH} rays per call (batchify_rays_and_render_by_chunk slabs them)")
    return _render(rays, packed, opts, t_rand, u, _next_seed(seed), int(ray_offset), prec, return_intermediates, occupancy, **_geometry_kw(geometry))


def batchify_rays_and_render_by_chunk(ray_o, ray_d, model, posenc, H, W, K, opts, *, t_rand=None, u=None, seed=None,
                                      ray_offset: int = 0, bf16: bool = False, f16s: bool = False, coarse_f16s: bool = False, f16: bool = False,
                                      coarse_f16: bool = False, occupancy=None, train_occupancy=None, geometry: bool = False,
                                      ray_grad: bool = False):
    prec = ops.precision(bf16, f16s, coarse_f16s, f16, coarse_f16)
    ray_grad = _ray_grad_arg(ray_grad, train_occupancy)
    training = train_path.wants_grad(model) or train_path.wants_ray_grad(model, ray_grad, ray_o, ray_d)
    occupancy = _occupancy_arg(occupancy, training, prec)
    train_occupancy = _train_occupancy_arg(train_occupancy, training, prec)
    train_f16s = _train_f16s(prec) if training else False
    packed = None if training else packed_for(model)
    dev = next(model.parameters()).device if training else packed.device
    ray_d = as_f32_dev(ray_d, dev)
    flat_d = ray_d.reshape(-1, 3)
    ray_o = ray_o.to(dev) if ray_o.device != dev else ray_o
    flat_o = ray_o.to(torch.float32).expand(ray_d.shape).reshape(-1, 3)
    if getattr(opts, "data_type", None) == "llff":
        k00 = K[0][0]
        focal = float(k00.item()) if isinstance(k00, torch.Tensor) else float(k00)
        if ray_grad:
            from . import pose
            flat_o, flat_d = pose.ndc_rays(H, W, focal, 1.0, flat_o, flat_d)
        else:
            flat_o, flat_d = ndc_rays(H, W, focal, 1.0, flat_o, flat_d)
    rays = torch.cat((flat_o, flat_d), dim=-1)
    N = rays.shape[0]
    seed = _next_seed(seed)
    Nf = int(opts.N_samples_f)
    parts = []
    train_stats = None
    slab = train_path.MAX_TRAIN_RAYS if training else (MAX_RAYS_PER_LAUNCH if occupancy is None else occ.MAX_RAYS_PER_LAUNCH)
    for i in range(0, N, slab):
        j = min(N, i + slab)
        tr, uu = (None if t_rand is None else t_rand[i:j]), (None if u is None else u[i:j])
        if training:
            parts.append(_render_train(rays[i:j].contiguous(), model, opts, train_occupancy, tr, uu, seed, int(ray_offset) + i, train_f16s, geometry,
                                       ray_grad))
            if train_occupancy is not None:
                train_stats = occ.add_stats(train_stats, train_occupancy.last_stats)
        else:
            parts.append(_render(rays[i:j], packed, opts, tr, uu, seed, int(ray_offset) + i, prec, False, occupancy, **_geometry_kw(geometry)))
    if train_occupancy is not None:
        train_occupancy.last_stats = train_stats
    def cat(key):
        return parts[0][key] if len(parts) == 1 else torch.cat([p[key] for p in parts], dim=0)
    res = (cat("rgb_c"), cat("disp_c"), cat("rgb_f"), cat("disp_f")) if Nf > 0 else (cat("rgb_c"), cat("disp_c"), None, None)
    if geometry:
        return (*res, {name + "_" + key: cat(name + "_" + key) for key in (("c", "f") if Nf > 0 else ("c",)) for name in geo.EXTRA_KEYS})
    return res
```

### nerf_pytorch_paeng_amd/ops.py

```python
from __future__ import annotations

import ctypes as C
from typing import Dict, NamedTuple, Optional, Sequence, Tuple

import numpy as np
import torch

from . import _lib as L
from ._lib import MiNerfError, Net, RenderCfg, TrainLayout, WorkspaceLayout, check, dev_ptr, lib, stream_ptr


def _guard(device):
    device = torch.device(device)
    if device.type != "cuda":
        raise MiNerfError(f"tensors must live on a HIP device (got {device}); this path has no CPU fallback")
    return torch.cuda.device(device)


def make_net(D: int, W: int, skip: int = 4, L_x: int = 10, L_d: int = 4) -> Net:
    return Net(D, W, skip, L_x, L_d)


F16S_FWD_MAX_D = 14
F16S_DGRAD_MAX_D = 15
HALF_64PT_MAX_D = 12


def check_f16s_forward_depth(net: Net) -> None:
    if net.D > F16S_FWD_MAX_D:
        raise MiNerfError(f"the split-precision forward kernel keeps every layer's biases and its waves' encoding buffers beside the weight ring in LDS: "
                          f"D = {net.D} does not fit (D <= {F16S_FWD_MAX_D}); a deeper network runs in fp32, bf16 or f16")


def f16s_dgrad_fits(net: Net) -> bool:
    return net.D <= F16S_DGRAD_MAX_D


def pack_module(sd: Dict[str, "np.ndarray | torch.Tensor"], prefix: str, net: Net, bf16: bool = False, backward: bool = False,
                f16s: bool = False) -> torch.Tensor:
    def arr(key):
        v = sd[prefix + key]
        if isinstance(v, torch.Tensor):
            v = v.detach().cpu().numpy()
        return np.ascontiguousarray(v, dtype=np.float32)

    in_x, in_d, W, D = 3 + 6 * net.L_x, 3 + 6 * net.L_d, net.W, net.D
    keep = []
    def ptr(a, shape):
        if tuple(a.shape) != tuple(shape):
            raise MiNerfError(f"parameter shape {a.shape} != expected {shape}")
        keep.append(a)
        return a.ctypes.data_as(C.c_void_p)

    wx = (C.c_void_p * D)()
    bx = (C.c_void_p * D)()
    for l in range(D):
        fan_in = in_x if l == 0 else (W + in_x if (net.skip >= 0 and l == net.skip + 1) else W)
        wx[l] = ptr(arr(f"linear_x.{l}.weight"), (W, fan_in))
        bx[l] = ptr(arr(f"linear_x.{l}.bias"), (W,))
    p = L.Params(wx, bx,
                 ptr(arr("linear_density.weight"), (1, W)), ptr(arr("linear_density.bias"), (1,)),
                 ptr(arr("linear_feat.weight"), (W, W)), ptr(arr("linear_feat.bias"), (W,)),
                 ptr(arr("linear_d.weight"), (W // 2, W + in_d)), ptr(arr("linear_d.bias"), (W // 2,)),
                 ptr(arr("linear_color.weight"), (3, W // 2)), ptr(arr("linear_color.bias"), (3,)))
    if backward and f16s:
        size_fn, pack_fn = lib().mi_nerf_packed_bytes_bwd_f16s, lib().mi_nerf_pack_weights_bwd_f16s
    elif backward:
        size_fn, pack_fn = lib().mi_nerf_packed_bytes_bwd, lib().mi_nerf_pack_weights_bwd
    elif f16s:
        size_fn, pack_fn = lib().mi_nerf_packed_bytes_f16s, lib().mi_nerf_pack_weights_f16s
    elif bf16:
        size_fn, pack_fn = lib().mi_nerf_packed_bytes_bf16, lib().mi_nerf_pack_weights_bf16
    else:
        size_fn, pack_fn = lib().mi_nerf_packed_bytes, lib().mi_nerf_pack_weights
    nbytes = size_fn(C.byref(net))
    if nbytes == 0:
        check(1, "mi_nerf_packed_bytes")
    blob = torch.empty(nbytes, dtype=torch.uint8)
    check(pack_fn(C.byref(net), C.byref(p), blob.data_ptr(), nbytes), "mi_nerf_pack_weights")
    return blob


def _cam(K, pose) -> Tuple[C.Array, C.Array]:
    k = K.detach().cpu().numpy() if isinstance(K, torch.Tensor) else np.asarray(K)
    k4 = (C.c_float * 4)(float(np.float32(k[0][0])), float(np.float32(k[1][1])), float(np.float32(k[0][2])), float(np.float32(k[1][2])))
    p = pose.detach().cpu().numpy() if isinstance(pose, torch.Tensor) else np.asarray(pose)
    p = np.asarray(p, dtype=np.float32)[:3, :4]
    return k4, (C.c_float * 12)(*p.reshape(-1).tolist())


def make_o_d(W: int, H: int, K, pose, device, row0: int = 0, n_rows: Optional[int] = None, want_origins: bool = True):
    n_rows = H - row0 if n_rows is None else n_rows
    device = torch.device(device)
    k4, p12 = _cam(K, pose)
    d = torch.empty(n_rows, W, 3, dtype=torch.float32, device=device)
    o = torch.empty(n_rows, W, 3, dtype=torch.float32, device=device) if want_origins else None
    with _guard(device):
        check(lib().mi_nerf_make_o_d(W, H, k4, p12, row0, n_rows, dev_ptr(o), dev_ptr(d), stream_ptr(device)), "mi_nerf_make_o_d")
    return o, d


def make_o_d_pixels(W: int, H: int, K, pose, pix: torch.Tensor):
    device = pix.device
    k4, p12 = _cam(K, pose)
    n = pix.numel()
    o = torch.empty(n, 3, dtype=torch.float32, device=device)
    d = torch.empty(n, 3, dtype=torch.float32, device=device)
    with _guard(device):
        check(lib().mi_nerf_make_o_d_pixels(W, H, k4, p12, dev_ptr(pix, "pix", torch.int64, 8), n, dev_ptr(o), dev_ptr(d),
                                            stream_ptr(device)), "mi_nerf_make_o_d_pixels")
    return o, d


def ndc_rays(H: int, W: int, focal: float, near: float, rays_o: torch.Tensor, rays_d: torch.Tensor):
    device = rays_d.device
    n = rays_d.shape[0]
    def strided(t, name):
        if t.dim() != 2 or t.shape[1] != 3 or t.dtype != torch.float32 or not t.is_cuda:
            raise MiNerfError(f"{name} must be a [n,3] fp32 device tensor")
        if t.stride(1) != 1 or (t.stride(0) not in (0, 3) and n > 1):
            t = t.contiguous()
        return t, (t.stride(0) if n > 1 else 3)
    o, os_ = strided(rays_o, "rays_o")
    d, ds_ = strided(rays_d, "rays_d")
    oo = torch.empty(n, 3, dtype=torch.float32, device=device)
    dd = torch.empty(n, 3, dtype=torch.float32, device=device)
    with _guard(device):
        check(lib().mi_nerf_ndc_rays(H, W, float(focal), float(near), o.data_ptr(), os_, d.data_ptr(), ds_, n, dev_ptr(oo),
                                     dev_ptr(dd), stream_ptr(device)), "mi_nerf_ndc_rays")
    return oo, dd


def deterministic(opts) -> bool:
    p = getattr(opts, "perturb", 1.0)
    return isinstance(p, (int, float)) and p == 0.0


def fill_uniform(seed: int, stream_id: int, ray0: int, n_rays: int, n_samples: int, device, out: Optional[torch.Tensor] = None) -> torch.Tensor:
    device = torch.device(device)
    if out is None:
        out = torch.empty(n_rays, n_samples, dtype=torch.float32, device=device)
    else:
        if tuple(out.shape) != (n_rays, n_samples):
            raise MiNerfError(f"out must be [{n_rays}, {n_samples}], got {tuple(out.shape)}")
        device = out.device
    with _guard(device):
        check(lib().mi_nerf_fill_uniform(seed & 0xFFFFFFFF, stream_id, ray0, n_rays, n_samples, dev_ptr(out), stream_ptr(device)),
              "mi_nerf_fill_uniform")
    return out


def stratified_z(near: float, far: float, t_rand: torch.Tensor) -> torch.Tensor:
    n, S = t_rand.shape
    z = torch.empty_like(t_rand)
    with _guard(t_rand.device):
        check(lib().mi_nerf_stratified_z(n, S, float(near), float(far), dev_ptr(t_rand, "t_rand"), dev_ptr(z),
                                         stream_ptr(t_rand.device)), "mi_nerf_stratified_z")
    return z


def sample_pdf(bins: torch.Tensor, weights: torch.Tensor, N: int, det: bool, u: Optional[torch.Tensor]) -> torch.Tensor:
    n, B = bins.shape
    if tuple(weights.shape) != (n, B - 1):
        raise MiNerfError(f"weights must be [n, B-1] = {(n, B - 1)}, got {tuple(weights.shape)}")
    if not det and (u is None or tuple(u.shape) != (n, N)):
        raise MiNerfError("u [n, N] is required unless det")
    out = torch.empty(n, N, dtype=torch.float32, device=bins.device)
    with _guard(bins.device):
        check(lib().mi_nerf_sample_pdf(dev_ptr(bins, "bins"), dev_ptr(weights, "weights"), n, B, N, int(det),
                                       None if det else dev_ptr(u, "u"), dev_ptr(out), stream_ptr(bins.device)), "mi_nerf_sample_pdf")
    return out


def fine_z(z_c: torch.Tensor, weights_c: torch.Tensor, Nf: int, det: bool, u: Optional[torch.Tensor], want_samples: bool = False):
    n, Sc = z_c.shape
    if tuple(weights_c.shape) != (n, Sc):
        raise MiNerfError("weights_c must match z_c")
    if not det and (u is None or tuple(u.shape) != (n, Nf)):
        raise MiNerfError("u [n, Nf] is required unless det")
    z_f = torch.empty(n, Sc + Nf, dtype=torch.float32, device=z_c.device)
    zs = torch.empty(n, Nf, dtype=torch.float32, device=z_c.device) if want_samples else None
    with _guard(z_c.device):
        check(lib().mi_nerf_fine_z(dev_ptr(z_c, "z_c"), dev_ptr(weights_c, "weights_c"), n, Sc, Nf, int(det),
                                   None if det else dev_ptr(u, "u"), dev_ptr(z_f), dev_ptr(zs), stream_ptr(z_c.device)), "mi_nerf_fine_z")
    return (z_f, zs) if want_samples else z_f


def embed(rays: torch.Tensor, z: torch.Tensor, L_x: int, L_d: int) -> torch.Tensor:
    n, S = z.shape
    out = torch.empty(n * S, 6 + 6 * L_x + 6 * L_d, dtype=torch.float32, device=z.device)
    with _guard(z.device):
        check(lib().mi_nerf_embed(dev_ptr(rays, "rays"), dev_ptr(z, "z"), n, S, L_x, L_d, dev_ptr(out), stream_ptr(z.device)), "mi_nerf_embed")
    return out


def posenc(x: torch.Tensor, Lf: int) -> torch.Tensor:
    n = x.shape[0]
    out = torch.empty(n, 3 + 6 * Lf, dtype=torch.float32, device=x.device)
    with _guard(x.device):
        check(lib().mi_nerf_posenc(dev_ptr(x, "x"), n, Lf, dev_ptr(out), stream_ptr(x.device)), "mi_nerf_posenc")
    return out


def mlp_embedded(net: Net, packed: torch.Tensor, x: torch.Tensor) -> torch.Tensor:
    n = x.shape[0]
    if x.dim() != 2 or x.shape[1] != 6 + 6 * net.L_x + 6 * net.L_d:
        raise MiNerfError(f"x must be [n, {6 + 6 * net.L_x + 6 * net.L_d}], got {tuple(x.shape)}")
    out = torch.empty(n, 4, dtype=torch.float32, device=x.device)
    with _guard(x.device):
        check(lib().mi_nerf_mlp_embedded(C.byref(net), dev_ptr(packed, "packed", torch.uint8, 16), dev_ptr(x, "x"), n, dev_ptr(out, "out", align=16),
                                         stream_ptr(x.device)), "mi_nerf_mlp_embedded")
    return out


def mlp_rays(net: Net, packed: torch.Tensor, rays: torch.Tensor, z: torch.Tensor, bf16: bool = False, points_per_wave: int = 0,
             f16s: bool = False) -> torch.Tensor:
    n, S = z.shape
    if tuple(rays.shape) != (n, 6):
        raise MiNerfError(f"rays must be [n,6], got {tuple(rays.shape)}")
    raw = torch.empty(n, S, 4, dtype=torch.float32, device=z.device)
    args = (C.byref(net), dev_ptr(packed, "packed", torch.uint8, 16), dev_ptr(rays, "rays"), dev_ptr(z, "z"), n, S, dev_ptr(raw, "raw", align=16))
    with _guard(z.device):
        if f16s:
            check(lib().mi_nerf_mlp_rays_f16s(*args, stream_ptr(z.device)), "mi_nerf_mlp_rays_f16s")
        elif bf16:
            check(lib().mi_nerf_mlp_rays_bf16_shape(*args, int(points_per_wave), stream_ptr(z.device)), "mi_nerf_mlp_rays_bf16_shape")
        else:
            check(lib().mi_nerf_mlp_rays(*args, stream_ptr(z.device)), "mi_nerf_mlp_rays")
    return raw


def composite(raw: torch.Tensor, z: torch.Tensor, rays_or_d: torch.Tensor, want_all: bool = True):
    n, S = z.shape
    if tuple(raw.shape) != (n, S, 4):
        raise MiNerfError(f"raw must be [n,S,4] = {(n, S, 4)}, got {tuple(raw.shape)}")
    stride = rays_or_d.shape[-1]
    if tuple(rays_or_d.shape) != (n, stride) or stride not in (3, 6):
        raise MiNerfError("rays must be [n,6] or rays_d [n,3]")
    dev = z.device
    rgb = torch.empty(n, 3, dtype=torch.float32, device=dev)
    disp = torch.empty(n, dtype=torch.float32, device=dev)
    acc = torch.empty(n, dtype=torch.float32, device=dev) if want_all else None
    wts = torch.empty(n, S, dtype=torch.float32, device=dev) if want_all else None
    depth = torch.empty(n, dtype=torch.float32, device=dev) if want_all else None
    with _guard(dev):
        check(lib().mi_nerf_composite(dev_ptr(raw, "raw", align=16), dev_ptr(z, "z"), dev_ptr(rays_or_d, "rays"), stride, n, S, dev_ptr(rgb),
                                      dev_ptr(disp), dev_ptr(acc), dev_ptr(wts), dev_ptr(depth), stream_ptr(dev)), "mi_nerf_composite")
    return rgb, disp, acc, wts, depth


def composite_backward(raw: torch.Tensor, z: torch.Tensor, rays_or_d: torch.Tensor, d_rgb: torch.Tensor) -> torch.Tensor:
    n, S = z.shape
    if tuple(raw.shape) != (n, S, 4) or tuple(d_rgb.shape) != (n, 3):
        raise MiNerfError(f"raw must be {(n, S, 4)} and d_rgb {(n, 3)}, got {tuple(raw.shape)} / {tuple(d_rgb.shape)}")
    stride = rays_or_d.shape[-1]
    if tuple(rays_or_d.shape) != (n, stride) or stride not in (3, 6):
        raise MiNerfError("rays must be [n,6] or rays_d [n,3]")
    d_raw = torch.empty(n, S, 4, dtype=torch.float32, device=z.device)
    with _guard(z.device):
        check(lib().mi_nerf_composite_backward(dev_ptr(raw, "raw", align=16), dev_ptr(z, "z"), dev_ptr(rays_or_d, "rays"), stride, n, S,
                                               dev_ptr(d_rgb, "d_rgb"), dev_ptr(d_raw, "d_raw", align=16), stream_ptr(z.device)),
              "mi_nerf_composite_backward")
    return d_raw


PARAM_ORDER = ("linear_x", "linear_d", "linear_feat", "linear_density", "linear_color")


def param_count(net: Net) -> int:
    n = lib().mi_nerf_param_count(C.byref(net))
    if n == 0:
        check(1, "mi_nerf_param_count")
    return int(n)


def param_names(net: Net):
    names = []
    for l in range(net.D):
        names += [f"linear_x.{l}.weight", f"linear_x.{l}.bias"]
    for head in PARAM_ORDER[1:]:
        names += [f"{head}.weight", f"{head}.bias"]
    return names


def flatten_params(sd, prefix: str, net: Net, device=None) -> torch.Tensor:
    flat = torch.cat([torch.as_tensor(sd[prefix + k]).detach().reshape(-1).float() for k in param_names(net)])
    if flat.numel() != param_count(net):
        raise MiNerfError(f"flat parameter vector has {flat.numel()} entries, expected {param_count(net)}")
    return flat.to(device) if device is not None else flat


def train_layout(net: Net, n_rays: int, S: int) -> TrainLayout:
    lay = TrainLayout()
    check(lib().mi_nerf_train_layout_query(C.byref(net), int(n_rays), int(S), C.byref(lay)), "mi_nerf_train_layout_query")
    return lay


def pack_map(net: Net, backward: bool = False) -> torch.Tensor:
    nbytes = (lib().mi_nerf_packed_bytes_bwd if backward else lib().mi_nerf_packed_bytes)(C.byref(net))
    if nbytes == 0:
        check(1, "mi_nerf_packed_bytes")
    m = torch.empty(nbytes // 4, dtype=torch.int32)
    check(lib().mi_nerf_pack_map(C.byref(net), int(backward), m.data_ptr(), m.numel()), "mi_nerf_pack_map")
    return m


def pack_apply(map_dev: torch.Tensor, flat: torch.Tensor, out: Optional[torch.Tensor] = None) -> torch.Tensor:
    dev = flat.device
    nbytes = map_dev.numel() * 4
    if out is None:
        out = torch.empty(nbytes, dtype=torch.uint8, device=dev)
    if out.numel() != nbytes:
        raise MiNerfError(f"blob must have {nbytes} bytes, got {out.numel()}")
    with _guard(dev):
        check(lib().mi_nerf_pack_apply(dev_ptr(map_dev, "map", torch.int32), dev_ptr(flat, "flat"), nbytes, dev_ptr(out, "blob", torch.uint8, 16),
                                       stream_ptr(dev)), "mi_nerf_pack_apply")
    return out


def pack_map_bf16(net: Net) -> torch.Tensor:
    n = lib().mi_nerf_pack_map_bf16_len(C.byref(net))
    if n == 0:
        check(1, "mi_nerf_pack_map_bf16_len")
    m = torch.empty(n, dtype=torch.int32)
    check(lib().mi_nerf_pack_map_bf16(C.byref(net), m.data_ptr(), m.numel()), "mi_nerf_pack_map_bf16")
    return m


def pack_apply_bf16(net: Net, map_dev: torch.Tensor, flat: torch.Tensor) -> torch.Tensor:
    dev = flat.device
    nbytes = lib().mi_nerf_packed_bytes_bf16(C.byref(net))
    out = torch.empty(nbytes, dtype=torch.uint8, device=dev)
    with _guard(dev):
        check(lib().mi_nerf_pack_apply_bf16(C.byref(net), dev_ptr(map_dev, "map", torch.int32), dev_ptr(flat, "flat"), dev_ptr(out, "blob", torch.uint8, 16),
                                            nbytes, stream_ptr(dev)), "mi_nerf_pack_apply_bf16")
    return out


def pack_map_f16s(net: Net, backward: bool = False) -> torch.Tensor:
    n = (lib().mi_nerf_pack_map_bwd_f16s_len if backward else lib().mi_nerf_pack_map_f16s_len)(C.byref(net))
    if n == 0:
        check(1, "mi_nerf_pack_map_f16s_len")
    m = torch.empty(n, dtype=torch.int32)
    check((lib().mi_nerf_pack_map_bwd_f16s if backward else lib().mi_nerf_pack_map_f16s)(C.byref(net), m.data_ptr(), m.numel()), "mi_nerf_pack_map_f16s")
    return m


def pack_apply_f16s(net: Net, map_dev: torch.Tensor, flat: torch.Tensor, out_of_range: Optional[torch.Tensor] = None, backward: bool = False) -> torch.Tensor:
    dev = flat.device
    nbytes = (lib().mi_nerf_packed_bytes_bwd_f16s if backward else lib().mi_nerf_packed_bytes_f16s)(C.byref(net))
    if nbytes == 0:
        check(1, "mi_nerf_packed_bytes_f16s")
    out = torch.empty(nbytes, dtype=torch.uint8, device=dev)
    fn = lib().mi_nerf_pack_apply_bwd_f16s if backward else lib().mi_nerf_pack_apply_f16s
    with _guard(dev):
        check(fn(C.byref(net), dev_ptr(map_dev, "map", torch.int32), dev_ptr(flat, "flat"), dev_ptr(out, "blob", torch.uint8, 16),
                 nbytes, None if out_of_range is None else dev_ptr(out_of_range, "out_of_range", torch.int32), stream_ptr(dev)),
              "mi_nerf_pack_apply_f16s")
    return out


def mlp_rays_train(net: Net, packed: torch.Tensor, rays: torch.Tensor, z: torch.Tensor, stash: Optional[torch.Tensor] = None, f16s: bool = False):
    n, S = z.shape
    if tuple(rays.shape) != (n, 6):
        raise MiNerfError(f"rays must be [n,6], got {tuple(rays.shape)}")
    lay = train_layout(net, n, S)
    if stash is None:
        stash = torch.empty(lay.stash_bytes, dtype=torch.uint8, device=z.device)
    raw = torch.empty(n, S, 4, dtype=torch.float32, device=z.device)
    with _guard(z.device):
        fn = lib().mi_nerf_mlp_rays_train_f16s if f16s else lib().mi_nerf_mlp_rays_train
        check(fn(C.byref(net), dev_ptr(packed, "packed", torch.uint8, 16), dev_ptr(rays, "rays"), dev_ptr(z, "z"), n, S,
                 dev_ptr(raw, "raw", align=16), dev_ptr(stash, "stash", torch.uint8, 16), stash.numel(),
                 stream_ptr(z.device)), "mi_nerf_mlp_rays_train_f16s" if f16s else "mi_nerf_mlp_rays_train")
    return raw, stash


def mlp_backward(net: Net, packed: torch.Tensor, packed_bwd: torch.Tensor, rays: torch.Tensor, z: torch.Tensor, d_raw: torch.Tensor,
                 stash: torch.Tensor, work: Optional[torch.Tensor] = None, stage: int = 0, grads: Optional[torch.Tensor] = None,
                 f16s_wgrad: bool = False, f16s_dgrad: bool = False):
    n, S = z.shape
    if tuple(d_raw.shape) != (n, S, 4) or tuple(rays.shape) != (n, 6):
        raise MiNerfError(f"d_raw must be {(n, S, 4)} and rays {(n, 6)}, got {tuple(d_raw.shape)} / {tuple(rays.shape)}")
    lay = train_layout(net, n, S)
    dev = z.device
    if work is None:
        work = torch.empty(lay.work_bytes, dtype=torch.uint8, device=dev)
    if grads is None:
        grads = torch.empty(param_count(net), dtype=torch.float32, device=dev)
    elif grads.numel() != param_count(net):
        raise MiNerfError(f"grads must have {param_count(net)} elements, got {grads.numel()}")
    with _guard(dev):
        check(lib().mi_nerf_mlp_backward_mode(C.byref(net), dev_ptr(packed, "packed", torch.uint8, 16), dev_ptr(packed_bwd, "packed_bwd", torch.uint8, 16),
                                              dev_ptr(rays, "rays"), dev_ptr(z, "z"), n, S, dev_ptr(d_raw, "d_raw", align=16),
                                              dev_ptr(stash, "stash", torch.uint8, 16), dev_ptr(work, "work", torch.uint8, 16), work.numel(),
                                              dev_ptr(grads, "grads"), int(stage), (1 if f16s_wgrad else 0) | (2 if f16s_dgrad else 0), stream_ptr(dev)), "mi_nerf_mlp_backward_mode")
    return (None if stage == 1 else grads), work


def mlp_embedded_train(net: Net, packed: torch.Tensor, x: torch.Tensor):
    n = x.shape[0]
    if x.dim() != 2 or x.shape[1] != 6 + 6 * net.L_x + 6 * net.L_d:
        raise MiNerfError(f"x must be [n, {6 + 6 * net.L_x + 6 * net.L_d}], got {tuple(x.shape)}")
    lay = train_layout(net, (n + 31) // 32, 32)
    stash = torch.empty(lay.stash_bytes, dtype=torch.uint8, device=x.device)
    out = torch.empty(n, 4, dtype=torch.float32, device=x.device)
    with _guard(x.device):
        check(lib().mi_nerf_mlp_embedded_train(C.byref(net), dev_ptr(packed, "packed", torch.uint8, 16), dev_ptr(x, "x"), n, dev_ptr(out, "out", align=16),
                                               dev_ptr(stash, "stash", torch.uint8, 16), stash.numel(), stream_ptr(x.device)), "mi_nerf_mlp_embedded_train")
    return out, stash


def mlp_embedded_backward(net: Net, packed: torch.Tensor, packed_bwd: torch.Tensor, x: torch.Tensor, d_out: torch.Tensor, stash: torch.Tensor,
                          grads: Optional[torch.Tensor] = None) -> torch.Tensor:
    n = x.shape[0]
    if tuple(d_out.shape) != (n, 4):
        raise MiNerfError(f"d_out must be {(n, 4)}, got {tuple(d_out.shape)}")
    lay = train_layout(net, (n + 31) // 32, 32)
    dev = x.device
    work = torch.empty(lay.work_bytes, dtype=torch.uint8, device=dev)
    if grads is None:
        grads = torch.empty(param_count(net), dtype=torch.float32, device=dev)
    with _guard(dev):
        check(lib().mi_nerf_mlp_embedded_backward(C.byref(net), dev_ptr(packed, "packed", torch.uint8, 16), dev_ptr(packed_bwd, "packed_bwd", torch.uint8, 16),
                                                  dev_ptr(x, "x"), n, dev_ptr(d_out, "d_out", align=16), dev_ptr(stash, "stash", torch.uint8, 16),
                                                  dev_ptr(work, "work", torch.uint8, 16), work.numel(), dev_ptr(grads, "grads"), stream_ptr(dev)),
              "mi_nerf_mlp_embedded_backward")
    return grads


def wgrad_product(delta: torch.Tensor, M: int, x: torch.Tensor, N: int, P: int, want_bias: bool = True, iters: int = 1, timed: bool = False):
    outs, biases, ms = wgrad_products([delta], [x], P, [int(M)], [int(N)], want_bias, iters, timed)
    return outs[0], (biases[0] if want_bias else None), ms


def wgrad_products(deltas: Sequence[torch.Tensor], xs: Sequence[torch.Tensor], P: int, Ms: Optional[Sequence[int]] = None,
                   Ns: Optional[Sequence[int]] = None, want_bias: bool = True, iters: int = 1, timed: bool = False, f16s: bool = False):
    n = len(deltas)
    if n == 0 or len(xs) != n:
        raise MiNerfError("deltas / xs must be non-empty lists of equal length")
    dev = deltas[0].device
    Ms = [d.shape[1] for d in deltas] if Ms is None else list(Ms)
    Ns = [x.shape[1] for x in xs] if Ns is None else list(Ns)
    for d, x, M, N in zip(deltas, xs, Ms, Ns):
        if d.dim() != 2 or x.dim() != 2 or d.shape[0] < P or x.shape[0] < P or d.shape[1] < M or x.shape[1] < N:
            raise MiNerfError(f"operands {tuple(d.shape)} / {tuple(x.shape)} too small for P={P}, M={M}, N={N}")
    outs = [torch.empty(M, N, dtype=torch.float32, device=dev) for M, N in zip(Ms, Ns)]
    biases = [torch.empty(M, dtype=torch.float32, device=dev) for M in Ms] if want_bias else None
    scratch = torch.empty(int(lib().mi_nerf_wgrad_scratch_bytes()), dtype=torch.uint8, device=dev)
    PP, II = C.c_void_p * n, C.c_int * n
    ms = C.c_float(0.0)
    with _guard(dev):
        check((lib().mi_nerf_wgrad_products_f16s if f16s else lib().mi_nerf_wgrad_products)(n, PP(*[dev_ptr(d, "delta") for d in deltas]), II(*[d.stride(0) for d in deltas]), II(*Ms),
                                           PP(*[dev_ptr(x, "x") for x in xs]), II(*[x.stride(0) for x in xs]), II(*Ns), int(P),
                                           PP(*[dev_ptr(o) for o in outs]), II(*Ns), PP(*[dev_ptr(b) for b in biases]) if want_bias else None,
                                           dev_ptr(scratch, "scratch", torch.uint8, 16), scratch.numel(), int(iters),
                                           C.byref(ms) if timed else None, stream_ptr(dev)), "mi_nerf_wgrad_products")
    return outs, biases, (float(ms.value) if timed else None)


def backward_range(net: Net, n_rays: int, S: int, work: torch.Tensor):
    lay = train_layout(net, n_rays, S)
    words = work[lay.work_bytes - 256:lay.work_bytes - 248].view(torch.float32).cpu()
    return float(words[0]), float(words[1])


def backward_range_words(net: Net, n_rays: int, S: int, work: torch.Tensor) -> torch.Tensor:
    lay = train_layout(net, n_rays, S)
    return work[lay.work_bytes - 256:lay.work_bytes - 248].view(torch.float32)


def train_views(net: Net, n_rays: int, S: int, stash: Optional[torch.Tensor] = None, work: Optional[torch.Tensor] = None):
    lay = train_layout(net, n_rays, S)
    n_pts = n_rays * S
    W, D = net.W, net.D
    out = {}
    def view(buf, off, shape):
        cnt = int(np.prod(shape))
        return buf[off:off + 4 * cnt].view(torch.float32).reshape(shape)
    if stash is not None:
        out["stash_h"] = view(stash, lay.stash_h, (D, n_pts, W))
        out["stash_f"] = view(stash, lay.stash_f, (n_pts, W))
        out["stash_g"] = view(stash, lay.stash_g, (n_pts, W // 2))
    if work is not None:
        out["delta_h"] = view(work, lay.delta_h, (D, n_pts, W))
        out["delta_f"] = view(work, lay.delta_f, (n_pts, W))
        out["delta_d"] = view(work, lay.delta_d, (n_pts, W // 2))
    return out


REDUCE_SCRATCH_BYTES = 8192


def image_metrics(pred: torch.Tensor, target: torch.Tensor) -> torch.Tensor:
    if pred.shape != target.shape or pred.numel() == 0:
        raise MiNerfError(f"pred {tuple(pred.shape)} and target {tuple(target.shape)} must match and be non-empty")
    dev = pred.device
    out = torch.empty(2, dtype=torch.float32, device=dev)
    scratch = torch.empty(REDUCE_SCRATCH_BYTES, dtype=torch.uint8, device=dev)
    with _guard(dev):
        check(lib().mi_nerf_image_metrics(dev_ptr(pred, "pred"), dev_ptr(target, "target"), pred.numel(), dev_ptr(out),
                                          dev_ptr(scratch, "scratch", torch.uint8), scratch.numel(), stream_ptr(dev)), "mi_nerf_image_metrics")
    return out


def ssim(pred: torch.Tensor, target: torch.Tensor, *, hw=None, downsample: int = 1, clamp_cs: bool = False, return_map: bool = False):
    from . import _iqa
    if pred.shape != target.shape or pred.numel() == 0:
        raise MiNerfError(f"pred {tuple(pred.shape)} and target {tuple(target.shape)} must match and be non-empty")
    shape = tuple(pred.shape)
    if len(shape) == 2 and shape[1] == 3 and hw is not None and int(hw[0]) * int(hw[1]) == shape[0]:
        n, H, W = 1, int(hw[0]), int(hw[1])
    elif len(shape) == 3 and shape[2] == 3 and hw is None:
        n, H, W = 1, shape[0], shape[1]
    elif len(shape) == 4 and shape[3] == 3 and hw is None:
        n, H, W = shape[0], shape[1], shape[2]
    else:
        raise MiNerfError(f"ssim takes [H,W,3], [H*W,3] with hw=(H,W), or [N,H,W,3]; got {shape} with hw={hw}")
    dev = pred.device
    with _guard(dev):
        L = _iqa.lib()
        ds = int(downsample)
        nbytes = L.mi_iqa_ssim_scratch_bytes(n, H, W, ds)
        f = L.mi_iqa_ssim_downsample_factor(H, W, ds)
        if nbytes == 0 or f == 0:
            raise MiNerfError(f"mi_iqa_ssim refused: {_iqa.last_error()}")
        out = torch.empty(n, dtype=torch.float32, device=dev)
        smap = torch.empty(n, H // f - 10, W // f - 10, 3, dtype=torch.float32, device=dev) if return_map else None
        scratch = torch.empty(nbytes // 8, dtype=torch.float64, device=dev)
        _iqa.check(L.mi_iqa_ssim(dev_ptr(pred, "pred"), dev_ptr(target, "target"), n, H, W, ds, _iqa.SSIM_CLAMP_CS if clamp_cs else 0,
                                 dev_ptr(out), dev_ptr(smap, "map"), dev_ptr(scratch, "scratch", torch.float64, 8), nbytes, stream_ptr(dev)),
                   "mi_iqa_ssim")
    return (out, smap) if return_map else out


def lpips(pred: torch.Tensor, target: torch.Tensor, hw=None, model=None, per_tap: bool = False):
    if model is None:
        raise MiNerfError("lpips needs model=perceptual.Lpips(...): the weights are the caller's, there is no default network")
    return model(pred, target, hw=hw, per_tap=per_tap)


def nanmax(x: torch.Tensor) -> torch.Tensor:
    if x.numel() == 0:
        raise MiNerfError("nanmax of an empty tensor")
    dev = x.device
    out = torch.empty(1, dtype=torch.float32, device=dev)
    scratch = torch.empty(REDUCE_SCRATCH_BYTES, dtype=torch.uint8, device=dev)
    with _guard(dev):
        check(lib().mi_nerf_nanmax(dev_ptr(x, "x"), x.numel(), dev_ptr(out), dev_ptr(scratch, "scratch", torch.uint8), scratch.numel(),
                                   stream_ptr(dev)), "mi_nerf_nanmax")
    return out


def to8b(x: torch.Tensor, divisor: Optional[torch.Tensor] = None) -> torch.Tensor:
    dev = x.device
    out = torch.empty(x.shape, dtype=torch.uint8, device=dev)
    with _guard(dev):
        check(lib().mi_nerf_to8b(dev_ptr(x, "x"), x.numel(), dev_ptr(divisor, "divisor"), dev_ptr(out, "out", torch.uint8, 1), stream_ptr(dev)),
              "mi_nerf_to8b")
    return out


def rays_rgb(W: int, H: int, K, poses: torch.Tensor, images: torch.Tensor) -> torch.Tensor:
    n_img = poses.shape[0]
    if tuple(poses.shape[1:]) != (3, 4) or tuple(images.shape) != (n_img, H, W, 3):
        raise MiNerfError(f"poses must be [n,3,4] and images [n,{H},{W},3]; got {tuple(poses.shape)} / {tuple(images.shape)}")
    dev = images.device
    k = K.detach().cpu().numpy() if isinstance(K, torch.Tensor) else np.asarray(K)
    k4 = (C.c_float * 4)(float(np.float32(k[0][0])), float(np.float32(k[1][1])), float(np.float32(k[0][2])), float(np.float32(k[1][2])))
    out = torch.empty(n_img * H * W, 3, 3, dtype=torch.float32, device=dev)
    with _guard(dev):
        check(lib().mi_nerf_rays_rgb(int(W), int(H), k4, dev_ptr(poses, "poses"), dev_ptr(images, "images"), n_img, dev_ptr(out),
                                     stream_ptr(dev)), "mi_nerf_rays_rgb")
    return out


def gather_rows(src: torch.Tensor, idx: torch.Tensor) -> torch.Tensor:
    if idx.dim() != 1 or idx.dtype != torch.int64:
        raise MiNerfError(f"idx must be a 1-d int64 tensor, got {tuple(idx.shape)} {idx.dtype}")
    n_src = src.shape[0]
    row = src.numel() // max(n_src, 1)
    n = int(idx.shape[0])
    dst = torch.empty((n, *src.shape[1:]), dtype=torch.float32, device=src.device)
    if n == 0:
        return dst
    with _guard(src.device):
        check(lib().mi_nerf_permute_rows(dev_ptr(src, "src"), dev_ptr(idx, "idx", torch.int64, 8), n, int(row), dev_ptr(dst), stream_ptr(src.device)),
              "mi_nerf_permute_rows")
    return dst


def permute_rows(src: torch.Tensor, perm: torch.Tensor) -> torch.Tensor:
    n = src.shape[0]
    if perm.shape != (n,):
        raise MiNerfError(f"perm must be [{n}], got {tuple(perm.shape)}")
    return gather_rows(src, perm)


MODE_F32, MODE_BF16, MODE_BF16_64, MODE_BF16_32, MODE_F16S, MODE_F16S_BF16, MODE_F16, MODE_F16_BF16 = 0, 1, 2, 3, 5, 6, 8, 9
PRECISION_FLAGS = ("bf16", "f16s", "coarse_f16s", "f16", "coarse_f16")
_FAMILIES = {(): ("fp32", "fp32"), ("bf16",): ("bf16", "bf16"), ("f16s",): ("f16s", "f16s"), ("bf16", "coarse_f16s"): ("f16s", "bf16"),
             ("f16",): ("f16", "f16"), ("bf16", "coarse_f16"): ("f16", "bf16")}
_MODES = {("fp32", "fp32", 0): MODE_F32, ("bf16", "bf16", 0): MODE_BF16, ("bf16", "bf16", 64): MODE_BF16_64, ("bf16", "bf16", 32): MODE_BF16_32,
          ("f16s", "f16s", 0): MODE_F16S, ("f16s", "bf16", 0): MODE_F16S_BF16, ("f16", "f16", 0): MODE_F16, ("f16", "bf16", 0): MODE_F16_BF16}


class Precision(NamedTuple):
    coarse: str
    fine: str
    points_per_wave: int = 0

    @property
    def mode(self) -> int:
        return _MODES[self]

    @property
    def reads_f16s(self) -> bool:
        return bool({self.coarse, self.fine} & {"f16s", "f16"})


def precision(bf16: bool = False, f16s: bool = False, coarse_f16s: bool = False, f16: bool = False, coarse_f16: bool = False,
              points_per_wave: int = 0) -> Precision:
    on = tuple(k for k, v in zip(PRECISION_FLAGS, (bf16, f16s, coarse_f16s, f16, coarse_f16)) if v)
    if on not in _FAMILIES:
        raise MiNerfError(f"no precision mode sets {' + '.join(on)}: none (fp32), bf16, f16s, f16, or bf16 with one of coarse_f16s / coarse_f16")
    coarse, fine = _FAMILIES[on]
    p = Precision(coarse, fine, 0 if fine in ("fp32", "f16s") else int(points_per_wave))
    if p not in _MODES:
        raise MiNerfError(f"points_per_wave={points_per_wave}: 0 (chosen per launch), or 64 / 32 with bf16 alone")
    return p


def render_cfg(near: float, far: float, Sc: int, Nf: int, det: bool, bf16: bool = False, points_per_wave: int = 0, seed: int = 0,
               ray_offset: int = 0, f16s: bool = False, coarse_f16s: bool = False, f16: bool = False, coarse_f16: bool = False) -> RenderCfg:
    mode = precision(bf16, f16s, coarse_f16s, f16, coarse_f16, points_per_wave).mode
    return RenderCfg(float(near), float(far), int(Sc), int(Nf), int(bool(det)), mode, int(seed) & 0xFFFFFFFF, 0, int(ray_offset))


def workspace_layout(cfg: RenderCfg, n: int) -> WorkspaceLayout:
    wl = WorkspaceLayout()
    check(lib().mi_nerf_render_workspace_layout(C.byref(cfg), n, C.byref(wl)), "mi_nerf_render_workspace_layout")
    return wl


def render_rays(net: Net, packed_c: torch.Tensor, packed_f: Optional[torch.Tensor], cfg: RenderCfg, rays: torch.Tensor,
                t_rand: Optional[torch.Tensor], u: Optional[torch.Tensor], workspace: Optional[torch.Tensor] = None,
                out: Optional[Sequence[torch.Tensor]] = None):
    n = rays.shape[0]
    dev = rays.device
    if tuple(rays.shape) != (n, 6) or (t_rand is not None and tuple(t_rand.shape) != (n, cfg.Sc)):
        raise MiNerfError(f"rays [n,6] / t_rand [n,{cfg.Sc}] expected, got {tuple(rays.shape)} / {None if t_rand is None else tuple(t_rand.shape)}")
    if cfg.Nf > 0 and not cfg.det and u is not None and tuple(u.shape) != (n, cfg.Nf):
        raise MiNerfError(f"u [n,{cfg.Nf}] expected")
    wl = workspace_layout(cfg, n)
    if workspace is None or workspace.numel() < wl.total:
        workspace = torch.empty(max(wl.total, 256), dtype=torch.uint8, device=dev)
    if out is None:
        rgb_c = torch.empty(n, 3, dtype=torch.float32, device=dev)
        disp_c = torch.empty(n, dtype=torch.float32, device=dev)
        rgb_f = torch.empty(n, 3, dtype=torch.float32, device=dev) if cfg.Nf > 0 else None
        disp_f = torch.empty(n, dtype=torch.float32, device=dev) if cfg.Nf > 0 else None
    else:
        rgb_c, disp_c, rgb_f, disp_f = out
    with _guard(dev):
        check(lib().mi_nerf_render_rays(C.byref(net), dev_ptr(packed_c, "packed_coarse", torch.uint8, 16),
                                        dev_ptr(packed_f, "packed_fine", torch.uint8, 16), C.byref(cfg), dev_ptr(rays, "rays"), n,
                                        dev_ptr(t_rand, "t_rand"), dev_ptr(u, "u") if (cfg.Nf > 0 and not cfg.det) else None,
                                        dev_ptr(workspace, "workspace", torch.uint8, 256), workspace.numel(), dev_ptr(rgb_c), dev_ptr(disp_c),
                                        dev_ptr(rgb_f), dev_ptr(disp_f), stream_ptr(dev)), "mi_nerf_render_rays")
    return rgb_c, disp_c, rgb_f, disp_f, workspace


def workspace_views(cfg: RenderCfg, n: int, workspace: torch.Tensor) -> Dict[str, torch.Tensor]:
    wl = workspace_layout(cfg, n)
    Sc, St = cfg.Sc, cfg.Sc + cfg.Nf
    def view(off, shape):
        cnt = int(np.prod(shape))
        return workspace[off:off + cnt * 4].view(torch.float32).view(*shape)
    v = {"z_c": view(wl.z_c, (n, Sc)), "raw_c": view(wl.raw_c, (n, Sc, 4)), "weights_c": view(wl.weights_c, (n, Sc))}
    if cfg.Nf > 0:
        v["z_f"] = view(wl.z_f, (n, St))
        v["raw_f"] = view(wl.raw_f, (n, St, 4))
    return v


def time_mlp_rays(net: Net, packed: torch.Tensor, rays: torch.Tensor, z: torch.Tensor, raw: torch.Tensor, iters: int, bf16: bool = False,
                  points_per_wave: int = 0, f16s: bool = False, f16: bool = False) -> float:
    mode = precision(bf16, f16s, f16=f16, points_per_wave=points_per_wave).mode
    n, S = z.shape
    ms = C.c_float(0.0)
    with _guard(z.device):
        check(lib().mi_nerf_time_mlp_rays(C.byref(net), dev_ptr(packed, "packed", torch.uint8, 16), dev_ptr(rays, "rays"), dev_ptr(z, "z"), n, S,
                                          dev_ptr(raw, "raw", align=16), iters, mode, C.byref(ms),
                                          stream_ptr(z.device)), "mi_nerf_time_mlp_rays")
    return float(ms.value)


def selftest_mfma(device) -> None:
    device = torch.device(device)
    with _guard(device):
        check(lib().mi_nerf_selftest_mfma(stream_ptr(device)), "mi_nerf_selftest_mfma")
```

Before: 493,400.

## Add density-only coarse pass that skips coarse color when only fine image is needed

When the caller does not need the coarse image (inference with a fine pass), the coarse MLP runs a density-only kernel variant. It stops after the trunk and density head, skipping the feature, direction and color layers, and streams only the trunk weights. Coarse compositing skips the sigmoid color and the weighted-sum reductions and writes only weights for fine sampling. This cuts coarse-pass arithmetic and weight traffic, but the coarse rgb/disp outputs are no longer produced, and the path only applies in F32 mode at kernel width 256 or less.

```diff
diff --git a/nerf_pytorch_paeng_amd/csrc/api.hip b/nerf_pytorch_paeng_amd/csrc/api.hip
--- a/nerf_pytorch_paeng_amd/csrc/api.hip
+++ b/nerf_pytorch_paeng_amd/csrc/api.hip
@@ -30,6 +30,7 @@
 }
 
 int mlp_rays_fp32(const mi_nerf_net*, const void*, const float*, const float*, int64_t, int, float*, hipStream_t);
+int mlp_rays_fp32_density(const mi_nerf_net*, const void*, const float*, const float*, int64_t, int, float*, hipStream_t);
 int mlp_embedded_fp32(const mi_nerf_net*, const void*, const float*, int64_t, float*, hipStream_t);
 int mlp_rays_bf16(const mi_nerf_net*, const void*, const float*, const float*, int64_t, int, float*, hipStream_t, int points_per_wave, const StratDraw* strat,
                   FineDraw* fine = nullptr);
@@ -402,7 +403,15 @@
     if (int rc = workspace_layout(cfg, n, &L)) return rc;
     if (n == 0) return MI_NERF_OK;
     MN_CHECK_ARG(ws_bytes >= L.total, "workspace too small: %zu < %zu", ws_bytes, L.total);
-    MN_CHECK_ARG(rays && rgb_c && disp_c && packed_c && (ws || L.total == 0), "NULL pointer");
+    MN_CHECK_ARG(rays && packed_c && (ws || L.total == 0), "NULL pointer");
+    const bool coarse_image = rgb_c || disp_c;
+    if (!coarse_image) {
+        if (int rc = check_net_basic(net)) return rc;
+        MN_CHECK_ARG(cfg->Nf > 0, "the coarse outputs are NULL and Nf == 0: without a fine pass the coarse image is the result");
+        MN_CHECK_ARG(cfg->mode == MI_NERF_MODE_F32 && !wide_kernel_width(kernel_width(net->W)),
+                     "the coarse outputs may be NULL (no coarse image) in MI_NERF_MODE_F32 at kernel width <= 256 only (mode %d, W = %d)", cfg->mode, net->W);
+    }
+    MN_CHECK_ARG(!coarse_image || (rgb_c && disp_c), "one of the coarse outputs is NULL: pass both, or neither (no coarse image)");
     MN_CHECK_ARG(cfg->Nf == 0 || (packed_f && rgb_f && disp_f), "fine pass needs packed_fine and outputs");
     MN_CHECK_ARG(cfg->reserved == 0, "mi_nerf_render_cfg.reserved must be 0");
     char* w = (char*)ws;
@@ -425,7 +434,9 @@
             return rc;
     } else {
         if (int rc = stage_stratified(n, Sc, cfg->near_, cfg->far_, t_rand, cfg->seed, cfg->ray_offset, z_c, st)) return rc;
-        if (int rc = mlp_rays_family(p.coarse, net, packed_c, rays, z_c, n, Sc, raw_c, st, p.points_per_wave)) return rc;
+        if (int rc = coarse_image ? mlp_rays_family(p.coarse, net, packed_c, rays, z_c, n, Sc, raw_c, st, p.points_per_wave)
+                                  : mlp_rays_fp32_density(net, packed_c, rays, z_c, n, Sc, raw_c, st))
+            return rc;
     }
     if (cfg->Nf == 0) return stage_composite(raw_c, z_c, rays, 6, n, Sc, rgb_c, disp_c, nullptr, wts_c, nullptr, st);
     {
diff --git a/nerf_pytorch_paeng_amd/csrc/layout.h b/nerf_pytorch_paeng_amd/csrc/layout.h
--- a/nerf_pytorch_paeng_amd/csrc/layout.h
+++ b/nerf_pytorch_paeng_amd/csrc/layout.h
@@ -70,6 +70,15 @@
     return b;
 }
 
+inline uint32_t trunk_stream_bytes(int D, int W_net, int skip) {
+    const int W = kernel_width(W_net);
+    const uint32_t NT = (uint32_t)W / 32;
+    const uint32_t pe_quads = (uint32_t)(pe_ksteps(KERNEL_LX) / 4) * NT;
+    const uint32_t h_quads = (uint32_t)(W / 2 / 4) * NT;
+    const bool has_skip_layer = skip >= 0 && skip + 1 < D;
+    return (pe_quads * (has_skip_layer ? 2u : 1u) + (uint32_t)(D - 1) * h_quads) * QUAD_BYTES;
+}
+
 struct SideTables {
     const char* stream;
     const float* side;
diff --git a/nerf_pytorch_paeng_amd/csrc/mlp_fp32.hip b/nerf_pytorch_paeng_amd/csrc/mlp_fp32.hip
--- a/nerf_pytorch_paeng_amd/csrc/mlp_fp32.hip
+++ b/nerf_pytorch_paeng_amd/csrc/mlp_fp32.hip
@@ -59,7 +59,7 @@
     }
 }
 
-template <int W, int MODE, int LX, int LD, bool STASH>
+template <int W, int MODE, int LX, int LD, bool STASH, bool DENS = false>
 __global__ __launch_bounds__(256) __attribute__((amdgpu_waves_per_eu(1, 1)))
 void mlp_fp32_kernel(const MlpArgs a) {
     constexpr int NT = W / 32;
@@ -124,7 +124,7 @@
             sample_point(p, o, d, zv);
             if (__builtin_expect(point_is_fast<LX>(p), 1)) encode_regs<LX, false>(pe, p, hh);
             else encode_regs<LX, true>(pe, p, hh);
-            if (ray != bias_ray) {
+            if (!DENS && ray != bias_ray) {
                 bias_ray = ray;
                 hoisted_dir_bias<W, LD>(scratch, d[0], d[1], d[2], side + a.o_wdir_t, side + a.o_bias_d, lane);
             }
@@ -155,6 +155,10 @@
         acc_to_b<NT, true>(acc, h);
         MN_STAMP(2);
         const float dens = xhalf_sum(dot_half<HN>(h, side + a.o_dens_w, hh)) + side[a.o_dens_b];
+        if constexpr (DENS) {
+            if (valid && hh == 0) a.out[out_idx * 4 + 3] = dens;
+            continue;
+        }
         acc_init<NT>(acc, side + a.o_bias_feat, hh);
         hidden_gemm<W, STASH, NT / 2, AL>(a, a.D - 1, out_idx, wt, wave_active, acc, h, aq, smem, ring, lane, hh);
         acc_to_b<NT, false>(acc, h);
@@ -217,10 +221,11 @@
 int mlp_rays_fp32_wide(const mi_nerf_net*, const void*, const float*, const float*, int64_t, int, float*, hipStream_t);
 int mlp_embedded_fp32_wide(const mi_nerf_net*, const void*, const float*, int64_t, float*, hipStream_t);
 
-template <int W, int MODE, bool STASH = false>
+template <int W, int MODE, bool STASH = false, bool DENS = false>
 static int launch(const MlpArgs& args_in, hipStream_t st) {
+    static_assert(!DENS || (MODE == 0 && !STASH), "the density-only pass is a MODE 0 inference kernel");
     MlpArgs args = args_in;
-    auto kern = mlp_fp32_kernel<W, MODE, 10, 4, STASH>;
+    auto kern = mlp_fp32_kernel<W, MODE, 10, 4, STASH, DENS>;
     static LdsOptIn opt_in = {};
     size_t lds;
     int grid;
@@ -278,6 +283,21 @@
     return kernel_width(net->W) == 256 ? launch<256, 0>(a, st) : launch<128, 0>(a, st);
 }
 
+int mlp_rays_fp32_density(const mi_nerf_net* net, const void* packed_dev, const float* rays_dev, const float* z_dev,
+                          int64_t n_rays, int S, float* raw_dev, hipStream_t st) {
+    if (int rc = check_net(net)) return rc;
+    MN_CHECK_ARG(!wide_kernel_width(kernel_width(net->W)), "the density-only pass exists for kernel widths 128 and 256 (W = %d runs at %d)", net->W,
+                 kernel_width(net->W));
+    MN_CHECK_ARG(n_rays >= 0 && S >= 1, "bad sizes n_rays=%lld S=%d", (long long)n_rays, S);
+    if (n_rays == 0) return MI_NERF_OK;
+    MN_CHECK_ARG(packed_dev && rays_dev && z_dev && raw_dev, "NULL device pointer");
+    MlpArgs a{};
+    fill_common(a, net, packed_dev, false);
+    a.stream_bytes = trunk_stream_bytes(net->D, net->W, net->skip);
+    fill_rays<32>(a, rays_dev, z_dev, n_rays, S, raw_dev);
+    return kernel_width(net->W) == 256 ? launch<256, 0, false, true>(a, st) : launch<128, 0, false, true>(a, st);
+}
+
 int mlp_rays_fp32_stash(const mi_nerf_net* net, const void* packed_dev, const float* rays_dev, const float* z_dev,
                         int64_t n_rays, int S, float* raw_dev, float* stash_h, float* stash_f, float* stash_g, unsigned* mask_h,
                         unsigned* mask_g, hipStream_t st) {
diff --git a/nerf_pytorch_paeng_amd/csrc/stage_dev.h b/nerf_pytorch_paeng_amd/csrc/stage_dev.h
--- a/nerf_pytorch_paeng_amd/csrc/stage_dev.h
+++ b/nerf_pytorch_paeng_amd/csrc/stage_dev.h
@@ -39,7 +39,7 @@
     return lane == 63 ? 0.0f : e;
 }
 
-template <int C>
+template <int C, bool IMAGE = true>
 __device__ __forceinline__ void composite_ray(const float* __restrict__ raw, const float* __restrict__ z, const float* __restrict__ rays,
                                               int ray_stride, long long ray, int S, int lane, float* __restrict__ rgb_o,
                                               float* __restrict__ disp_o, float* __restrict__ acc_o, float* __restrict__ w_o,
@@ -50,7 +50,8 @@
     const float* zr = z + ray * S;
     const f32x4* rr = (const f32x4*)(raw + ray * S * 4);
 
-    float alpha[C], zv[C], cr[C], cg[C], cb[C];
+    float alpha[C], zv[C];
+    [[maybe_unused]] float cr[C], cg[C], cb[C];
     float local = 1.0f;
 #pragma unroll
     for (int c = 0; c < C; ++c) {
@@ -65,13 +66,15 @@
         float a = 1.0f - expf(-sig * dist);
         if (!in || S == 1) a = 0.0f;
         alpha[c] = a;
-        cr[c] = 1.0f / (1.0f + expf(-v[0]));
-        cg[c] = 1.0f / (1.0f + expf(-v[1]));
-        cb[c] = 1.0f / (1.0f + expf(-v[2]));
+        if constexpr (IMAGE) {
+            cr[c] = 1.0f / (1.0f + expf(-v[0]));
+            cg[c] = 1.0f / (1.0f + expf(-v[1]));
+            cb[c] = 1.0f / (1.0f + expf(-v[2]));
+        }
         local *= in ? (1.0f - a + 1e-10f) : 1.0f;
     }
     float T = wave_excl_prod(local, lane);
-    float sw = 0.f, sr = 0.f, sg = 0.f, sb = 0.f, sd = 0.f;
+    [[maybe_unused]] float sw = 0.f, sr = 0.f, sg = 0.f, sb = 0.f, sd = 0.f;
 #pragma unroll
     for (int c = 0; c < C; ++c) {
         const int s = lane * C + c;
@@ -79,10 +82,11 @@
         if (s < S) {
             if (w_o) w_o[ray * S + s] = w;
             if (w_lds) w_lds[s] = w;
-            sw += w; sr += w * cr[c]; sg += w * cg[c]; sb += w * cb[c]; sd += w * zv[c];
+            if constexpr (IMAGE) { sw += w; sr += w * cr[c]; sg += w * cg[c]; sb += w * cb[c]; sd += w * zv[c]; }
         }
         T *= (1.0f - alpha[c] + 1e-10f);
     }
+    if constexpr (!IMAGE) return;
     sw = wave_sum(sw); sr = wave_sum(sr); sg = wave_sum(sg); sb = wave_sum(sb); sd = wave_sum(sd);
     if (lane == 0) {
         const float q = sd / sw;
diff --git a/nerf_pytorch_paeng_amd/csrc/stages.hip b/nerf_pytorch_paeng_amd/csrc/stages.hip
--- a/nerf_pytorch_paeng_amd/csrc/stages.hip
+++ b/nerf_pytorch_paeng_amd/csrc/stages.hip
@@ -260,7 +260,7 @@
     fine_z_ray(z_c, w_c + ray * Sc, ray, Sc, Nf, n2, det, u, z_f, z_samp, lds + wv * (2 * (Sc - 1) + n2), lane);
 }
 
-template <int C>
+template <int C, bool IMAGE = true>
 __global__ __launch_bounds__(256) void composite_fine_z_kernel(const float* __restrict__ raw, const float* __restrict__ z_c,
                                                                 const float* __restrict__ rays, long long n, int Sc, int Nf, int n2, int det,
                                                                 Jitter u, float* __restrict__ rgb_o, float* __restrict__ disp_o,
@@ -270,7 +270,7 @@
     const long long ray = (long long)blockIdx.x * 4 + wv;
     if (ray >= n) return;
     float* mine = lds + wv * (Sc + 2 * (Sc - 1) + n2);
-    composite_ray<C>(raw, z_c, rays, 6, ray, Sc, lane, rgb_o, disp_o, nullptr, w_o, nullptr, mine);
+    composite_ray<C, IMAGE>(raw, z_c, rays, 6, ray, Sc, lane, rgb_o, disp_o, nullptr, w_o, nullptr, mine);
     __builtin_amdgcn_wave_barrier();
     __builtin_amdgcn_fence(__ATOMIC_ACQ_REL, "wavefront");
     fine_z_ray(z_c, mine, ray, Sc, Nf, n2, det, u, z_f, nullptr, mine + Sc, lane);
@@ -423,15 +423,19 @@
     MN_CHECK_ARG(Sc + 2 * (Sc - 1) + n2 <= MAX_LDS_FLOATS_PER_RAY, "bad sizes (Sc=%d Nf=%d: 3 Sc - 2 + %d must not exceed %d)", Sc, Nf, n2,
                  MAX_LDS_FLOATS_PER_RAY);
     if (n == 0) return MI_NERF_OK;
-    MN_CHECK_ARG(raw_c && z_c && rays && rgb_c && disp_c && w_c && z_f, "NULL pointer");
+    MN_CHECK_ARG(raw_c && z_c && rays && w_c && z_f, "NULL pointer");
+    MN_CHECK_ARG((rgb_c != nullptr) == (disp_c != nullptr), "rgb_c and disp_c: both, or neither (no coarse image)");
+    const bool image = rgb_c != nullptr;
     const size_t lds = (size_t)4 * (Sc + 2 * (Sc - 1) + n2) * sizeof(float);
     const dim3 grid(blocks_for(n, 4)), block(256);
     const Jitter j{u, seed, 1u, (long long)ray0};
     const int C = (Sc + 63) / 64;
-#define MN_CFZ(CC) hipLaunchKernelGGL(composite_fine_z_kernel<CC>, grid, block, lds, st, raw_c, z_c, rays, (long long)n, Sc, Nf, n2, det, j, rgb_c, disp_c, w_c, z_f)
+#define MN_CFZ_(CC, IM) hipLaunchKernelGGL((composite_fine_z_kernel<CC, IM>), grid, block, lds, st, raw_c, z_c, rays, (long long)n, Sc, Nf, n2, det, j, rgb_c, disp_c, w_c, z_f)
+#define MN_CFZ(CC) do { if (image) MN_CFZ_(CC, true); else MN_CFZ_(CC, false); } while (0)
     if (C == 1) MN_CFZ(1); else if (C == 2) MN_CFZ(2); else if (C == 3) MN_CFZ(3); else if (C == 4) MN_CFZ(4);
     else if (C <= 8) MN_CFZ(8); else MN_CFZ(16);
 #undef MN_CFZ
+#undef MN_CFZ_
     MN_LAUNCH_CHECK("composite_fine_z_kernel");
     return MI_NERF_OK;
 }
diff --git a/nerf_pytorch_paeng_amd/dist.py b/nerf_pytorch_paeng_amd/dist.py
--- a/nerf_pytorch_paeng_amd/dist.py
+++ b/nerf_pytorch_paeng_amd/dist.py
@@ -173,9 +173,10 @@
     _, d = ops.make_o_d(W, H, K, pose, packed.device, row0=r0, n_rows=nr, want_origins=False)
     p = pose if isinstance(pose, torch.Tensor) else torch.as_tensor(pose)
     o = p[:3, -1].to(packed.device, torch.float32).expand(d.shape)
+    fine = int(opts.N_samples_f) > 0
     rc, dc, rf, df = NP.batchify_rays_and_render_by_chunk(o, d, packed, None, H, W, K, opts, seed=seed, ray_offset=r0 * W, bf16=bf16, f16s=f16s,
-                                                          coarse_f16s=coarse_f16s)
-    rgb, disp = (rc, dc) if int(opts.N_samples_f) == 0 else (rf, df)
+                                                          coarse_f16s=coarse_f16s, **({"coarse_image": False} if fine else {}))
+    rgb, disp = (rf, df) if fine else (rc, dc)
     return torch.cat([rgb, disp[:, None]], -1)
 
 
diff --git a/nerf_pytorch_paeng_amd/harness.py b/nerf_pytorch_paeng_amd/harness.py
--- a/nerf_pytorch_paeng_amd/harness.py
+++ b/nerf_pytorch_paeng_amd/harness.py
@@ -187,9 +187,11 @@
         rays = torch.cat([rays_o.reshape(-1, 3), rays_d.reshape(-1, 3)], -1)
         rgb, disp, _, _ = grid.render(rays, step=getattr(opts, "baked_step", None), T_min=float(getattr(opts, "baked_T_min", 0.0) or 0.0))
         return rgb, disp
+    fine = int(opts.N_samples_f) > 0
+    lean = {"coarse_image": False} if fine and not NP.train_path.wants_grad(model) else {}
     rgb_c, disp_c, rgb_f, disp_f = NP.batchify_rays_and_render_by_chunk(rays_o, rays_d, model, posenc, img_h, img_w, K, opts, **_precision(opts),
-                                                                        occupancy=getattr(opts, "occupancy", None))
-    return (rgb_c, disp_c) if int(opts.N_samples_f) == 0 else (rgb_f, disp_f)
+                                                                        occupancy=getattr(opts, "occupancy", None), **lean)
+    return (rgb_f, disp_f) if fine else (rgb_c, disp_c)
 
 
 def test(idx, i_test, posenc, model, test_imgs, gt_intrinsic, gt_extrinsic, hw, opts, *, log_dir: Optional[str] = None,
diff --git a/nerf_pytorch_paeng_amd/nerf_process.py b/nerf_pytorch_paeng_amd/nerf_process.py
--- a/nerf_pytorch_paeng_amd/nerf_process.py
+++ b/nerf_pytorch_paeng_amd/nerf_process.py
@@ -114,7 +114,7 @@
 
 
 def _render(rays: torch.Tensor, packed: PackedNeRF, opts, t_rand, u, seed: int, ray_offset: int, prec: ops.Precision,
-            intermediates: bool, occupancy=None, geometry: bool = False) -> Dict[str, torch.Tensor]:
+            intermediates: bool, occupancy=None, geometry: bool = False, coarse_image: bool = True) -> Dict[str, torch.Tensor]:
     n = rays.shape[0]
     dev = rays.device
     Sc, Nf = int(opts.N_samples_c), int(opts.N_samples_f)
@@ -135,12 +135,15 @@
     net, blob_c, blob_f = packed.kernel_blobs(prec)
     stats = None
     if occupancy is None:
-        rgb_c, disp_c, rgb_f, disp_f, ws = ops.render_rays(net, blob_c, blob_f if Nf > 0 else None, cfg, rays, t_rand, u)
+        rgb_c, disp_c, rgb_f, disp_f, ws = ops.render_rays(net, blob_c, blob_f if Nf > 0 else None, cfg, rays, t_rand, u,
+                                                           **({} if coarse_image else {"coarse_image": False}))
         views = ops.workspace_views
     else:
         rgb_c, disp_c, rgb_f, disp_f, ws, stats = occ.render_rays(net, blob_c, blob_f if Nf > 0 else None, cfg, occupancy, rays, t_rand, u)
         occupancy.last_stats = occ.add_stats(occupancy.last_stats, stats)
         views = occ.workspace_views
+        if not coarse_image:
+            rgb_c = disp_c = None
     out = {"rgb_c": rgb_c, "disp_c": disp_c}
     if Nf > 0:
         out["rgb_f"], out["disp_f"] = rgb_f, disp_f
@@ -194,6 +197,20 @@
     return {**({"geometry": True} if geometry else {}), **({"ray_grad": True} if ray_grad else {})}
 
 
+def _coarse_image_arg(coarse_image, opts, training: bool, geometry, intermediates: bool = False) -> Dict[str, bool]:
+    if coarse_image:
+        return {}
+    if int(opts.N_samples_f) == 0:
+        raise MiNerfError("coarse_image=False needs a fine pass (N_samples_f > 0): without one the coarse image is the result")
+    if training:
+        raise MiNerfError("coarse_image=False is an inference feature: the training loss reads rgb_c (call under torch.no_grad(), or freeze the model)")
+    if geometry:
+        raise MiNerfError("coarse_image=False with geometry=True: the coarse geometry outputs are composited from the whole of raw_c")
+    if intermediates:
+        raise MiNerfError("coarse_image=False with return_intermediates=True: the intermediates include the whole of raw_c")
+    return {"coarse_image": False}
+
+
 def _render_train(rays, model, opts, train_occupancy, t_rand, u, seed: int, ray_offset: int, f16s: bool, geometry, ray_grad):
     grid = {} if train_occupancy is None else {"grid": train_occupancy}
     return train_path.render_train(rays, model, opts, t_rand=t_rand, u=u, seed=seed, ray_offset=ray_offset, f16s=f16s,
@@ -208,10 +225,11 @@
 
 def render_rays(rays, model, posenc, opts, *, t_rand=None, u=None, seed=None, ray_offset: int = 0, bf16: bool = False,
                 return_intermediates: bool = False, f16s: bool = False, coarse_f16s: bool = False, f16: bool = False, coarse_f16: bool = False,
-                occupancy=None, train_occupancy=None, geometry: bool = False, ray_grad: bool = False):
+                occupancy=None, train_occupancy=None, geometry: bool = False, ray_grad: bool = False, coarse_image: bool = True):
     prec = ops.precision(bf16, f16s, coarse_f16s, f16, coarse_f16)
     ray_grad = _ray_grad_arg(ray_grad, train_occupancy)
     training = train_path.wants_grad(model) or train_path.wants_ray_grad(model, ray_grad, rays)
+    lean_kw = _coarse_image_arg(coarse_image, opts, training, geometry, return_intermediates)
     occupancy = _occupancy_arg(occupancy, training, prec)
     train_occupancy = _train_occupancy_arg(train_occupancy, training, prec)
     if training:
@@ -225,16 +243,18 @@
         raise MiNerfError(f"rays must be [n, 6] (o, d), got {tuple(rays.shape)}")
     if occupancy is not None and rays.shape[0] > occ.MAX_RAYS_PER_LAUNCH:
         raise MiNerfError(f"render_rays with a grid takes at most {occ.MAX_RAYS_PER_LAUNCH} rays per call (batchify_rays_and_render_by_chunk slabs them)")
-    return _render(rays, packed, opts, t_rand, u, _next_seed(seed), int(ray_offset), prec, return_intermediates, occupancy, **_geometry_kw(geometry))
+    return _render(rays, packed, opts, t_rand, u, _next_seed(seed), int(ray_offset), prec, return_intermediates, occupancy, **_geometry_kw(geometry),
+                   **lean_kw)
 
 
 def batchify_rays_and_render_by_chunk(ray_o, ray_d, model, posenc, H, W, K, opts, *, t_rand=None, u=None, seed=None,
                                       ray_offset: int = 0, bf16: bool = False, f16s: bool = False, coarse_f16s: bool = False, f16: bool = False,
                                       coarse_f16: bool = False, occupancy=None, train_occupancy=None, geometry: bool = False,
-                                      ray_grad: bool = False):
+                                      ray_grad: bool = False, coarse_image: bool = True):
     prec = ops.precision(bf16, f16s, coarse_f16s, f16, coarse_f16)
     ray_grad = _ray_grad_arg(ray_grad, train_occupancy)
     training = train_path.wants_grad(model) or train_path.wants_ray_grad(model, ray_grad, ray_o, ray_d)
+    lean_kw = _coarse_image_arg(coarse_image, opts, training, geometry)
     occupancy = _occupancy_arg(occupancy, training, prec)
     train_occupancy = _train_occupancy_arg(train_occupancy, training, prec)
     train_f16s = _train_f16s(prec) if training else False
@@ -268,10 +288,13 @@
             if train_occupancy is not None:
                 train_stats = occ.add_stats(train_stats, train_occupancy.last_stats)
         else:
-            parts.append(_render(rays[i:j], packed, opts, tr, uu, seed, int(ray_offset) + i, prec, False, occupancy, **_geometry_kw(geometry)))
+            parts.append(_render(rays[i:j], packed, opts, tr, uu, seed, int(ray_offset) + i, prec, False, occupancy, **_geometry_kw(geometry),
+                                 **lean_kw))
     if train_occupancy is not None:
         train_occupancy.last_stats = train_stats
     def cat(key):
+        if parts[0][key] is None:
+            return None
         return parts[0][key] if len(parts) == 1 else torch.cat([p[key] for p in parts], dim=0)
     res = (cat("rgb_c"), cat("disp_c"), cat("rgb_f"), cat("disp_f")) if Nf > 0 else (cat("rgb_c"), cat("disp_c"), None, None)
     if geometry:
diff --git a/nerf_pytorch_paeng_amd/ops.py b/nerf_pytorch_paeng_amd/ops.py
--- a/nerf_pytorch_paeng_amd/ops.py
+++ b/nerf_pytorch_paeng_amd/ops.py
@@ -643,9 +643,15 @@
     return wl
 
 
+def density_only_coarse(net: Net, cfg: RenderCfg) -> bool:
+    return cfg.Nf > 0 and cfg.mode == MODE_F32 and net.W <= 256
+
+
 def render_rays(net: Net, packed_c: torch.Tensor, packed_f: Optional[torch.Tensor], cfg: RenderCfg, rays: torch.Tensor,
                 t_rand: Optional[torch.Tensor], u: Optional[torch.Tensor], workspace: Optional[torch.Tensor] = None,
-                out: Optional[Sequence[torch.Tensor]] = None):
+                out: Optional[Sequence[torch.Tensor]] = None, coarse_image: bool = True):
+    if not coarse_image and cfg.Nf <= 0:
+        raise MiNerfError("coarse_image=False needs a fine pass (Nf > 0): without one the coarse image is the result")
     n = rays.shape[0]
     dev = rays.device
     if tuple(rays.shape) != (n, 6) or (t_rand is not None and tuple(t_rand.shape) != (n, cfg.Sc)):
@@ -655,19 +661,24 @@
     wl = workspace_layout(cfg, n)
     if workspace is None or workspace.numel() < wl.total:
         workspace = torch.empty(max(wl.total, 256), dtype=torch.uint8, device=dev)
+    lean = not coarse_image and density_only_coarse(net, cfg)
     if out is None:
-        rgb_c = torch.empty(n, 3, dtype=torch.float32, device=dev)
-        disp_c = torch.empty(n, dtype=torch.float32, device=dev)
+        rgb_c = None if lean else torch.empty(n, 3, dtype=torch.float32, device=dev)
+        disp_c = None if lean else torch.empty(n, dtype=torch.float32, device=dev)
         rgb_f = torch.empty(n, 3, dtype=torch.float32, device=dev) if cfg.Nf > 0 else None
         disp_f = torch.empty(n, dtype=torch.float32, device=dev) if cfg.Nf > 0 else None
     else:
         rgb_c, disp_c, rgb_f, disp_f = out
+        if lean:
+            rgb_c = disp_c = None
     with _guard(dev):
         check(lib().mi_nerf_render_rays(C.byref(net), dev_ptr(packed_c, "packed_coarse", torch.uint8, 16),
                                         dev_ptr(packed_f, "packed_fine", torch.uint8, 16), C.byref(cfg), dev_ptr(rays, "rays"), n,
                                         dev_ptr(t_rand, "t_rand"), dev_ptr(u, "u") if (cfg.Nf > 0 and not cfg.det) else None,
                                         dev_ptr(workspace, "workspace", torch.uint8, 256), workspace.numel(), dev_ptr(rgb_c), dev_ptr(disp_c),
                                         dev_ptr(rgb_f), dev_ptr(disp_f), stream_ptr(dev)), "mi_nerf_render_rays")
+    if not coarse_image:
+        rgb_c = disp_c = None
     return rgb_c, disp_c, rgb_f, disp_f, workspace
 
 
```

Result: no change. 493,500 (median of 2 runs) (+0.0%).
